# neevparikh/rpt

Hardware: AMD Instinct MI355X
Metric: Msamples/sec (higher is better)
Workload: dtype f32; 1 GPU; C3 lampshade-in-fog path trace 1024x1024x256spp; scene=examples/volumetric_pathtrace_lampshade.rs, parallelism=tile-shard x1, streams=2

## Files before the change

### include/rpt_hip.h

```cpp
#ifndef RPT_HIP_H
#define RPT_HIP_H

#include <stdint.h>

#ifdef __cplusplus
extern "C" {
#endif

#define RPT_OK 0
#define RPT_ERR_INVALID (-1)
#define RPT_ERR_STATE (-2)
#define RPT_ERR_DEVICE (-3)
#define RPT_ERR_UNSUPPORTED (-4)

typedef struct rpt_scene rpt_scene;

enum { RPT_SHAPE_SPHERE = 0, RPT_SHAPE_CUBE = 1, RPT_SHAPE_PLANE = 2, RPT_SHAPE_MESH = 3,
       RPT_SHAPE_GROUP = 4,
       RPT_SHAPE_MONOMIAL = 5  };

typedef struct rpt_shape_desc {
    int32_t kind;
    int32_t has_transform;
    double transform[16];
// ... 105 lines not shown
int rpt_denoise_device(rpt_denoiser*, const rpt_denoise_params*, const void* d_rgb, const void* d_var, const void* d_albedo,
                       const void* d_normal, const void* d_depth, void* d_out, void* d_out_var, void* hip_stream);
int rpt_denoise(rpt_denoiser*, const rpt_denoise_params*, const double* rgb, const double* var, const double* albedo,
                const double* normal, const double* depth, double* out, double* out_var);
int rpt_buffer_mean_device(rpt_buffer*, void* d_rgb, void* d_var, void* hip_stream);
int rpt_buffer_denoised_image(rpt_buffer*, rpt_denoiser*, const rpt_denoise_params*, const void* d_albedo, const void* d_normal,
                              const void* d_depth, uint8_t* out_rgb8);

int rpt_buffer_add_samples_tiles_device(rpt_buffer*, const void* d_rgb, const void* d_tiles, uint32_t n_tiles, void* hip_stream);
int rpt_buffer_tile_batches(rpt_buffer*, uint32_t* out , uint64_t capacity);
typedef struct rpt_adaptive_params {
    uint32_t spp_per_batch, min_batches, max_batches, _pad;
    double threshold;
    double floor;
} rpt_adaptive_params;
int rpt_buffer_tile_errors_device(rpt_buffer*, double floor, void* d_err , void* hip_stream);
int rpt_buffer_refine_tiles(rpt_buffer*, const rpt_adaptive_params*, void* d_tiles_out ,
                            uint32_t* n_out , void* d_err , void* hip_stream);
int rpt_render_adaptive(rpt_scene*, const rpt_camera*, const rpt_render_params*, const rpt_adaptive_params*,
                        uint64_t seed, rpt_buffer*, uint64_t stats[4] );

enum { RPT_PHOTON_MAP = 0, RPT_PHOTON_POINT_BEAM = 1, RPT_PHOTON_BEAM_BEAM = 2 };
int rpt_photon_map_build(rpt_scene*, uint64_t photon_count, int32_t kind, double watts, uint64_t seed);
#define RPT_PHOTON_RECORD_BYTES 48
int rpt_photon_shoot(rpt_scene*, uint64_t photon_count, int32_t kind, double watts, uint64_t seed,
                     uint32_t shard_rank, uint32_t shard_count, uint64_t n_out[2]);
int rpt_photon_records(rpt_scene*, int32_t which , void** d_records, uint64_t* n);
int rpt_photon_map_from_records(rpt_scene*, uint64_t photon_count, int32_t kind, const void* d_surface,
                                uint64_t n_surface, const void* d_volume, uint64_t n_volume);
int rpt_photon_map_stats(rpt_scene*, uint64_t out[8]);
int rpt_photon_map_download(rpt_scene*, int32_t which, float* out, uint64_t capacity_photons);
int rpt_photon_render_sample(rpt_scene*, const rpt_camera*, const rpt_render_params*, uint64_t gather_size,
                             uint64_t gather_size_volume, uint32_t num_samples, uint64_t seed,
                             uint32_t sample_offset, double* out_rgb);
int rpt_photon_render_sample_device(rpt_scene*, const rpt_camera*, const rpt_render_params*, uint64_t gather_size,
                                    uint64_t gather_size_volume, uint32_t num_samples, uint64_t seed,
                                    uint32_t sample_offset, void* d_out_rgb, void* hip_stream);

typedef struct rpt_comm rpt_comm;
#define RPT_COMM_ID_BYTES 128
int rpt_comm_unique_id(void* id_out);
int rpt_comm_create(const void* id, int rank, int n_ranks, int device, rpt_comm** out);
void rpt_comm_destroy(rpt_comm*);
int rpt_comm_rank(const rpt_comm*, int* rank, int* n_ranks);
#define RPT_GATHER_LOOPBACK 1u
int rpt_gather_frame_device(rpt_comm*, uint32_t width, uint32_t height, const void* d_shard, void* d_frame,
                            uint32_t flags, void* hip_stream);
int rpt_allgather_records_device(rpt_comm*, const void* d_local, uint64_t n_local, void* d_out, uint64_t capacity,
                                 uint64_t* n_per_rank, uint64_t* n_total, void* hip_stream);
int rpt_frame_pack_layout(uint32_t width, uint32_t height, uint32_t n_ranks, uint64_t* tile_offsets);
int rpt_frame_pack_device(uint32_t width, uint32_t height, uint32_t rank, uint32_t n_ranks, const void* d_frame,
                          void* d_packed, void* hip_stream);
int rpt_frame_unpack_device(uint32_t width, uint32_t height, uint32_t rank, uint32_t n_ranks, const void* d_packed,
                            void* d_frame, void* hip_stream);

int rpt_debug_epsilon_counters(rpt_scene*, uint64_t out[12]);
int rpt_f64_mesh_tree_info(rpt_scene*, uint64_t out[8]);

int rpt_debug_rng_u32(uint64_t seed, uint32_t pixel, uint32_t sample, uint32_t n, uint32_t* out);
int rpt_debug_material_sample_f(const rpt_material*, uint64_t n, const float* normals, const float* wos,
                                uint64_t seed, float* wi, float* pdf, int32_t* some);
int rpt_debug_material_bsdf(const rpt_material*, uint64_t n, const float* normals, const float* wos,
                            const float* wis, float* out_rgb);
int rpt_debug_radix_sort(uint64_t n, const uint64_t* keys, uint64_t* keys_out, uint32_t* order_out);
int rpt_debug_exclusive_scan2(uint64_t n, const uint32_t* a, const uint32_t* b, uint32_t* out_a, uint32_t* out_b, uint64_t totals[2]);
int rpt_debug_photon_positions64(rpt_scene*, double* out, uint64_t capacity);
int rpt_debug_photon_selections(rpt_scene*, uint32_t* out, uint64_t capacity_words, uint64_t dims[3]);
int rpt_debug_camera_rays(const rpt_camera*, const rpt_render_params*, uint64_t seed, uint32_t sample,
                          float* origins, float* dirs);
int rpt_debug_camera_sample(const rpt_camera*, const rpt_render_params*, uint64_t seed, uint32_t sample,
                            float* origins, float* dirs, uint32_t* next_word);
int rpt_debug_camera_sample_f64(const rpt_camera*, const rpt_render_params*, uint64_t seed, uint32_t sample,
                                double* origins, double* dirs, uint32_t* next_word);
int rpt_debug_light_sample(rpt_scene*, uint32_t light, uint64_t n, const float* positions, uint64_t seed, float* v, float* nrm,
                           float* pdf, float* intensity, float* wi, float* dist, uint32_t* next_word);
int rpt_debug_light_sample_f64(rpt_scene*, uint32_t light, uint64_t n, const double* positions, uint64_t seed, double* v, double* nrm,
                               double* pdf, double* intensity, double* wi, double* dist, uint32_t* next_word);
int rpt_debug_env_color(rpt_scene*, uint64_t n, const float* dirs, float* rgb);
int rpt_debug_env_color_f64(rpt_scene*, uint64_t n, const double* dirs, double* rgb);
int rpt_debug_medium_distance(rpt_scene*, uint64_t n, uint64_t seed, float* dmed, float* t_limit);
int rpt_debug_shadow_test(rpt_scene*, uint32_t light, uint64_t n, const float* origins, const float* dirs, const float* dist,
                          int32_t* out_flag, float* out_t);
int rpt_shadow_scan_info(rpt_scene*, uint32_t light, uint32_t out[4]);
int rpt_debug_distance_pair(float sigma_t, uint32_t k0, uint32_t n, float* out_new, float* out_guarded);
int rpt_debug_draw_forms(uint64_t seed, uint32_t n, uint32_t* out_new, uint32_t* out_ref);

int rpt_debug_bounce(const rpt_material* m, uint32_t max_bounces, uint32_t depth, int32_t in_medium, int32_t medium_event,
                     float albedo_med, const float* medium_color, uint64_t n, const float* normals, const float* rds, uint64_t seed,
                     int32_t* flag, float* wi, float* k, uint32_t* next_word);
int rpt_debug_material_f64(const rpt_material* m, uint64_t n, const double* normals, const double* wos, uint64_t seed, int32_t* some,
                           double* wi, double* pdf, double* f, uint32_t* next_word);
int rpt_debug_material_bsdf_f64(const rpt_material* m, uint64_t n, const double* normals, const double* wos, const double* wis,
                                double* f);
#ifdef __cplusplus
}
#endif
#endif
```

### rpt_amd/_lib.py

```python
import ctypes as C
import os
import sys

_HERE = os.path.dirname(os.path.abspath(__file__))
LIB_PATH = os.environ.get("RPT_LIB", os.path.join(_HERE, "librpt_hip.so"))


class RptError(RuntimeError):
    """Raised for every non-zero return code of the C ABI (message from rpt_last_error)."""


class ShapeDesc(C.Structure):
    pass


ShapeDesc._fields_ = [
    ("kind", C.c_int32),
    ("has_transform", C.c_int32),
    ("transform", C.c_double * 16),
    ("plane_normal", C.c_double * 3),
    ("plane_value", C.c_double),
    ("tris", C.POINTER(C.c_double)),
    ("n_tris", C.c_uint64),
    ("children", C.POINTER(ShapeDesc)),
# ... 86 lines not shown
     [_P, C.POINTER(CameraDesc), C.POINTER(RenderParams), C.c_uint32, C.c_uint64, C.c_uint32, _P, _P, _P, _P]),
    ("rpt_intersect_batch", C.c_int, [_P, C.c_uint64, _P, _P, _P, _P, _P]),
    ("rpt_intersect_batch_f64", C.c_int, [_P, C.c_uint64, _P, _P, _P, _P, _P]),
    ("rpt_intersect_segments", C.c_int, [_P, C.c_uint64, _P, _P, _P, _P, _P]),
    ("rpt_scan_cull_counters", C.c_int, [_P, C.POINTER(C.c_uint64)]),
    ("rpt_scan_cull_groups", C.c_int, [_P, C.POINTER(C.c_float), C.POINTER(C.c_uint64), C.POINTER(C.c_uint32), C.POINTER(C.c_uint32)]),
    ("rpt_scene_stats", C.c_int, [_P, C.POINTER(C.c_uint64)]),
    ("rpt_get_counters", C.c_int, [_P, C.POINTER(C.c_uint64)]),
    ("rpt_debug_section_counters", C.c_int, [_P, C.POINTER(C.c_uint64)]),
    ("rpt_get_timing", C.c_int, [_P, C.POINTER(C.c_double), C.POINTER(C.c_double), C.POINTER(C.c_int32)]),
    ("rpt_get_timing_mean", C.c_int, [_P, C.POINTER(C.c_double), C.POINTER(C.c_double), C.POINTER(C.c_int32)]),
    ("rpt_render_chunking", C.c_int, [C.c_uint32, C.POINTER(C.c_uint32), C.POINTER(C.c_uint32)]),
    ("rpt_scene_render_chunking", C.c_int, [_P, C.c_uint32, C.POINTER(C.c_uint32), C.POINTER(C.c_uint32)]),
    ("rpt_set_option", C.c_int, [C.c_char_p, C.c_int64]),
    ("rpt_scene_set_option", C.c_int, [_P, C.c_char_p, C.c_int64]),
    ("rpt_buffer_create", _P, [C.c_int, C.c_uint32, C.c_uint32, C.c_uint32]),
    ("rpt_buffer_destroy", None, [_P]),
    ("rpt_buffer_add_samples", C.c_int, [_P, _P]),
    ("rpt_buffer_add_samples_device", C.c_int, [_P, _P, _P]),
    ("rpt_buffer_image", C.c_int, [_P, _P]),
    ("rpt_buffer_variance", C.c_int, [_P, C.POINTER(C.c_double)]),
    ("rpt_buffer_batches", C.c_int, [_P, C.POINTER(C.c_uint32)]),
    ("rpt_render_into_buffer", C.c_int,
     [_P, C.POINTER(CameraDesc), C.POINTER(RenderParams), C.c_uint32, C.c_uint64, C.c_uint32, _P]),
    ("rpt_denoiser_create", _P, [C.c_int, C.c_uint32, C.c_uint32]),
    ("rpt_denoiser_destroy", None, [_P]),
    ("rpt_denoise_device", C.c_int, [_P, C.POINTER(DenoiseParams), _P, _P, _P, _P, _P, _P, _P, _P]),
    ("rpt_denoise", C.c_int, [_P, C.POINTER(DenoiseParams), _P, _P, _P, _P, _P, _P, _P]),
    ("rpt_buffer_mean_device", C.c_int, [_P, _P, _P, _P]),
    ("rpt_buffer_denoised_image", C.c_int, [_P, _P, C.POINTER(DenoiseParams), _P, _P, _P, _P]),
    ("rpt_buffer_add_samples_tiles_device", C.c_int, [_P, _P, _P, C.c_uint32, _P]),
    ("rpt_buffer_tile_batches", C.c_int, [_P, _P, C.c_uint64]),
    ("rpt_buffer_tile_errors_device", C.c_int, [_P, C.c_double, _P, _P]),
    ("rpt_buffer_refine_tiles", C.c_int, [_P, C.POINTER(AdaptiveParams), _P, C.POINTER(C.c_uint32), _P, _P]),
    ("rpt_render_adaptive", C.c_int,
     [_P, C.POINTER(CameraDesc), C.POINTER(RenderParams), C.POINTER(AdaptiveParams), C.c_uint64, _P, C.POINTER(C.c_uint64)]),
    ("rpt_photon_map_build", C.c_int, [_P, C.c_uint64, C.c_int32, C.c_double, C.c_uint64]),
    ("rpt_photon_shoot", C.c_int,
     [_P, C.c_uint64, C.c_int32, C.c_double, C.c_uint64, C.c_uint32, C.c_uint32, C.POINTER(C.c_uint64)]),
    ("rpt_photon_records", C.c_int, [_P, C.c_int32, C.POINTER(C.c_void_p), C.POINTER(C.c_uint64)]),
    ("rpt_photon_map_from_records", C.c_int, [_P, C.c_uint64, C.c_int32, _P, C.c_uint64, _P, C.c_uint64]),
    ("rpt_photon_map_stats", C.c_int, [_P, C.POINTER(C.c_uint64)]),
    ("rpt_photon_map_download", C.c_int, [_P, C.c_int32, _P, C.c_uint64]),
    ("rpt_photon_render_sample", C.c_int,
     [_P, C.POINTER(CameraDesc), C.POINTER(RenderParams), C.c_uint64, C.c_uint64, C.c_uint32, C.c_uint64, C.c_uint32, _P]),
    ("rpt_photon_render_sample_device", C.c_int,
     [_P, C.POINTER(CameraDesc), C.POINTER(RenderParams), C.c_uint64, C.c_uint64, C.c_uint32, C.c_uint64, C.c_uint32, _P, _P]),
    ("rpt_comm_unique_id", C.c_int, [_P]),
    ("rpt_comm_create", C.c_int, [_P, C.c_int, C.c_int, C.c_int, C.POINTER(C.c_void_p)]),
    ("rpt_comm_destroy", None, [_P]),
    ("rpt_comm_rank", C.c_int, [_P, C.POINTER(C.c_int), C.POINTER(C.c_int)]),
    ("rpt_gather_frame_device", C.c_int, [_P, C.c_uint32, C.c_uint32, _P, _P, C.c_uint32, _P]),
    ("rpt_allgather_records_device", C.c_int, [_P, _P, C.c_uint64, _P, C.c_uint64, C.POINTER(C.c_uint64), C.POINTER(C.c_uint64), _P]),
    ("rpt_frame_pack_layout", C.c_int, [C.c_uint32, C.c_uint32, C.c_uint32, C.POINTER(C.c_uint64)]),
    ("rpt_frame_pack_device", C.c_int, [C.c_uint32, C.c_uint32, C.c_uint32, C.c_uint32, _P, _P, _P]),
    ("rpt_frame_unpack_device", C.c_int, [C.c_uint32, C.c_uint32, C.c_uint32, C.c_uint32, _P, _P, _P]),
    ("rpt_debug_epsilon_counters", C.c_int, [_P, C.POINTER(C.c_uint64)]),
    ("rpt_f64_mesh_tree_info", C.c_int, [_P, C.POINTER(C.c_uint64)]),
    ("rpt_debug_rng_u32", C.c_int, [C.c_uint64, C.c_uint32, C.c_uint32, C.c_uint32, _P]),
    ("rpt_debug_material_sample_f", C.c_int,
     [C.POINTER(MaterialDesc), C.c_uint64, _P, _P, C.c_uint64, _P, _P, _P]),
    ("rpt_debug_material_bsdf", C.c_int, [C.POINTER(MaterialDesc), C.c_uint64, _P, _P, _P, _P]),
    ("rpt_debug_radix_sort", C.c_int, [C.c_uint64, _P, _P, _P]),
    ("rpt_debug_exclusive_scan2", C.c_int, [C.c_uint64, _P, _P, _P, _P, C.POINTER(C.c_uint64)]),
    ("rpt_debug_photon_positions64", C.c_int, [_P, _P, C.c_uint64]),
    ("rpt_debug_photon_selections", C.c_int, [_P, _P, C.c_uint64, C.POINTER(C.c_uint64)]),
    ("rpt_debug_camera_rays", C.c_int,
     [C.POINTER(CameraDesc), C.POINTER(RenderParams), C.c_uint64, C.c_uint32, _P, _P]),
    ("rpt_debug_light_sample", C.c_int, [_P, C.c_uint32, C.c_uint64, _P, C.c_uint64, _P, _P, _P, _P, _P, _P, _P]),
    ("rpt_debug_light_sample_f64", C.c_int, [_P, C.c_uint32, C.c_uint64, _P, C.c_uint64, _P, _P, _P, _P, _P, _P, _P]),
    ("rpt_debug_env_color", C.c_int, [_P, C.c_uint64, _P, _P]),
    ("rpt_debug_env_color_f64", C.c_int, [_P, C.c_uint64, _P, _P]),
    ("rpt_debug_medium_distance", C.c_int, [_P, C.c_uint64, C.c_uint64, _P, _P]),
    ("rpt_debug_camera_sample", C.c_int,
     [C.POINTER(CameraDesc), C.POINTER(RenderParams), C.c_uint64, C.c_uint32, _P, _P, _P]),
    ("rpt_debug_camera_sample_f64", C.c_int,
     [C.POINTER(CameraDesc), C.POINTER(RenderParams), C.c_uint64, C.c_uint32, _P, _P, _P]),
    ("rpt_debug_bounce", C.c_int, [C.POINTER(MaterialDesc), C.c_uint32, C.c_uint32, C.c_int32, C.c_int32, C.c_float, _P,
                                   C.c_uint64, _P, _P, C.c_uint64, _P, _P, _P, _P]),
    ("rpt_debug_shadow_test", C.c_int, [_P, C.c_uint32, C.c_uint64, _P, _P, _P, _P, _P]),
    ("rpt_debug_distance_pair", C.c_int, [C.c_float, C.c_uint32, C.c_uint32, _P, _P]),
    ("rpt_debug_draw_forms", C.c_int, [C.c_uint64, C.c_uint32, _P, _P]),
    ("rpt_shadow_scan_info", C.c_int, [_P, C.c_uint32, C.POINTER(C.c_uint32)]),
    ("rpt_debug_material_f64", C.c_int, [C.POINTER(MaterialDesc), C.c_uint64, _P, _P, C.c_uint64, _P, _P, _P, _P, _P]),
    ("rpt_debug_material_bsdf_f64", C.c_int, [C.POINTER(MaterialDesc), C.c_uint64, _P, _P, _P, _P]),
]

_lib = None


def vp(a):
    return a.ctypes.data_as(C.c_void_p)


def load():
    global _lib
    if _lib is not None:
        return _lib
    if not os.path.exists(LIB_PATH):
        raise RptError(
            f"{LIB_PATH} is missing: build it with `python -c 'import __graft_entry__ as g; g.build()'` "
            "(hipcc --offload-arch=gfx950).  There is no CPU fallback.")
    if "torch" not in sys.modules and os.environ.get("RPT_IMPORT_TORCH", "0") == "1":
        import torch
    lib = C.CDLL(LIB_PATH, mode=C.RTLD_GLOBAL)
    for name, res, args in SYMBOLS:
        fn = getattr(lib, name)
        fn.restype = res
        fn.argtypes = args
    _lib = lib
    return lib


def check(rc):
    if rc < 0:
        msg = load().rpt_last_error()
        raise RptError(f"rpt error {rc}: {msg.decode() if msg else ''}")
    return rc
```

### rpt_amd/api.py

```python
import ctypes as C
import math
import weakref

import numpy as np

from . import _lib
from ._lib import RptError, vp as _vp

def shard_pixels(width, height, rank, count):
    lib = _lib.load()
    n = _lib.check(lib.rpt_shard_tiles(width, height, rank, count, None, 0))
    tiles = np.zeros(max(n, 1), dtype=np.uint32)
    _lib.check(lib.rpt_shard_tiles(width, height, rank, count, tiles.ctypes.data_as(C.c_void_p), n))
    tiles_x = (width + 31) // 32
    ys, xs = np.mgrid[0:32, 0:32]
    out = []
    for t in tiles[:n]:
        x = (int(t) % tiles_x) * 32 + xs
        y = (int(t) // tiles_x) * 32 + ys
        m = (x < width) & (y < height)
        out.append((y[m] * width + x[m]).astype(np.uint32))
    return np.sort(np.concatenate(out)) if out else np.zeros(0, dtype=np.uint32)


# ... 1133 lines not shown
        return dict(zip(names, [int(v) for v in out]))

    def get_closest_hit(self, origins, dirs):
        lib = _lib.load()
        h = self.scene._commit(self.device_)
        o = np.ascontiguousarray(origins, dtype=np.float32).reshape(-1, 3)
        d = np.ascontiguousarray(dirs, dtype=np.float32).reshape(-1, 3)
        n = o.shape[0]
        t = np.empty(n, dtype=np.float32)
        obj = np.empty(n, dtype=np.int32)
        nrm = np.empty((n, 3), dtype=np.float32)
        _lib.check(lib.rpt_intersect_batch(h, n, o.ctypes.data_as(C.c_void_p), d.ctypes.data_as(C.c_void_p),
                                           t.ctypes.data_as(C.c_void_p), obj.ctypes.data_as(C.c_void_p),
                                           nrm.ctypes.data_as(C.c_void_p)))
        return t, obj, nrm

    def get_closest_hit_f64(self, origins, dirs):
        lib = _lib.load()
        h = self.scene._commit(self.device_)
        o = np.ascontiguousarray(origins, dtype=np.float64).reshape(-1, 3)
        d = np.ascontiguousarray(dirs, dtype=np.float64).reshape(-1, 3)
        n = o.shape[0]
        t = np.empty(n, dtype=np.float64)
        obj = np.empty(n, dtype=np.int32)
        nrm = np.empty((n, 3), dtype=np.float64)
        _lib.check(lib.rpt_intersect_batch_f64(h, n, o.ctypes.data_as(C.c_void_p), d.ctypes.data_as(C.c_void_p),
                                               t.ctypes.data_as(C.c_void_p), obj.ctypes.data_as(C.c_void_p),
                                               nrm.ctypes.data_as(C.c_void_p)))
        return t, obj, nrm

    def f64_mesh_tree_info(self):
        out = (C.c_uint64 * 8)()
        _lib.check(_lib.load().rpt_f64_mesh_tree_info(self.scene._commit(self.device_), out))
        keys = ("meshes", "triangles", "nodes", "depth", "bytes", "render_uses_trees", "photon_uses_trees", "tree_min")
        return {k: int(v) for k, v in zip(keys, out)}

    def debug_light_sample(self, light_index, positions, seed=0, f64=False):
        lib = _lib.load()
        h = self.scene._commit(self.device_)
        ft = np.float64 if f64 else np.float32
        pos = np.ascontiguousarray(positions, dtype=ft).reshape(-1, 3)
        n = pos.shape[0]
        out = {"v": np.empty((n, 3), ft), "nrm": np.empty((n, 3), ft), "p": np.empty(n, ft), "intensity": np.empty((n, 3), ft),
               "wi": np.empty((n, 3), ft), "dist": np.empty(n, ft), "next_word": np.empty(n, np.uint32)}
        fn = lib.rpt_debug_light_sample_f64 if f64 else lib.rpt_debug_light_sample
        _lib.check(fn(h, light_index, n, pos.ctypes.data_as(C.c_void_p), seed,
                      *[out[k].ctypes.data_as(C.c_void_p) for k in ("v", "nrm", "p", "intensity", "wi", "dist", "next_word")]))
        return out

    def debug_env_color(self, dirs, f64=False):
        lib = _lib.load()
        h = self.scene._commit(self.device_)
        d = np.ascontiguousarray(dirs, dtype=np.float64 if f64 else np.float32).reshape(-1, 3)
        out = np.empty_like(d)
        fn = lib.rpt_debug_env_color_f64 if f64 else lib.rpt_debug_env_color
        _lib.check(fn(h, d.shape[0], d.ctypes.data_as(C.c_void_p), out.ctypes.data_as(C.c_void_p)))
        return out

    def debug_medium_distance(self, n, seed=0):
        lib = _lib.load()
        h = self.scene._commit(self.device_)
        dmed, lim = np.empty(n, np.float32), np.empty(n, np.float32)
        _lib.check(lib.rpt_debug_medium_distance(h, n, seed, dmed.ctypes.data_as(C.c_void_p), lim.ctypes.data_as(C.c_void_p)))
        return dmed, lim

    def debug_shadow_test(self, light_index, origins, dirs, dist):
        lib = _lib.load()
        h = self.scene._commit(self.device_)
        o = np.ascontiguousarray(origins, dtype=np.float32).reshape(-1, 3)
        d = np.ascontiguousarray(dirs, dtype=np.float32).reshape(-1, 3)
        ds = np.ascontiguousarray(dist, dtype=np.float32).reshape(-1)
        n = o.shape[0]
        if d.shape[0] != n or ds.shape[0] != n:
            raise ValueError("origins, dirs and dist differ in length")
        flag, t = np.empty(n, np.int32), np.empty(n, np.float32)
        _lib.check(lib.rpt_debug_shadow_test(h, light_index, n, _vp(o), _vp(d), _vp(ds), _vp(flag), _vp(t)))
        return flag, t

    def shadow_scan_info(self, light_index):
        out = (C.c_uint32 * 4)()
        _lib.check(_lib.load().rpt_shadow_scan_info(self.scene._commit(self.device_), light_index, out))
        return {"twin_lo": int(out[0]), "twin_hi": int(out[1]), "shadow_form": int(out[2]), "twin_object": int(np.int32(np.uint32(out[3])))}


def debug_distance_pair(sigma_t, k0, n):
    new, guarded = np.empty(n, np.float32), np.empty(n, np.float32)
    _lib.check(_lib.load().rpt_debug_distance_pair(float(sigma_t), int(k0), int(n), _vp(new), _vp(guarded)))
    return new, guarded


DRAW_FORM_WORDS = 274


def debug_draw_forms(seed, n):
    new, ref = np.empty((DRAW_FORM_WORDS, n), np.uint32), np.empty((DRAW_FORM_WORDS, n), np.uint32)
    _lib.check(_lib.load().rpt_debug_draw_forms(C.c_uint64(int(seed)), int(n), _vp(new), _vp(ref)))
    return new, ref


def debug_bounce(material, normals, rds, max_bounces=3, depth=0, seed=0, in_medium=False, medium_event=False, albedo_med=0.0,
                 medium_color=(0.0, 0.0, 0.0)):
    nrm = np.ascontiguousarray(normals, dtype=np.float32).reshape(-1, 3)
    rd = np.ascontiguousarray(rds, dtype=np.float32).reshape(-1, 3)
    n = nrm.shape[0]
    if rd.shape[0] != n:
        raise ValueError("normals and rds differ in length")
    mcol = np.ascontiguousarray(medium_color, dtype=np.float32).reshape(3)
    out = {"flag": np.empty(n, np.int32), "wi": np.empty((n, 3), np.float32), "k": np.empty((n, 3), np.float32),
           "next_word": np.empty(n, np.uint32)}
    md = material_desc(material, _lib.MaterialDesc)
    _lib.check(_lib.load().rpt_debug_bounce(C.byref(md), max_bounces, depth, int(bool(in_medium)), int(bool(medium_event)),
                                            float(albedo_med), _vp(mcol), n, _vp(nrm), _vp(rd), seed,
                                            *[_vp(out[k]) for k in ("flag", "wi", "k", "next_word")]))
    return out


def debug_material_f64(material, normals, wos, seed=0):
    nrm = np.ascontiguousarray(normals, dtype=np.float64).reshape(-1, 3)
    wo = np.ascontiguousarray(wos, dtype=np.float64).reshape(-1, 3)
    n = nrm.shape[0]
    if wo.shape[0] != n:
        raise ValueError("normals and wos differ in length")
    out = {"some": np.empty(n, np.int32), "wi": np.empty((n, 3)), "pdf": np.empty(n), "f": np.empty((n, 3)),
           "next_word": np.empty(n, np.uint32)}
    md = material_desc(material, _lib.MaterialDesc)
    _lib.check(_lib.load().rpt_debug_material_f64(C.byref(md), n, _vp(nrm), _vp(wo), seed,
                                                  *[_vp(out[k]) for k in ("some", "wi", "pdf", "f", "next_word")]))
    return out


def debug_material_bsdf_f64(material, normals, wos, wis):
    arrs = [np.ascontiguousarray(a, dtype=np.float64).reshape(-1, 3) for a in (normals, wos, wis)]
    n = arrs[0].shape[0]
    if any(a.shape[0] != n for a in arrs):
        raise ValueError("normals, wos and wis differ in length")
    f = np.empty((n, 3))
    md = material_desc(material, _lib.MaterialDesc)
    _lib.check(_lib.load().rpt_debug_material_bsdf_f64(C.byref(md), n, *[_vp(a) for a in arrs], _vp(f)))
    return f


def debug_camera_sample(camera, width, height, sample=0, seed=0, f64=False):
    ft = np.float64 if f64 else np.float32
    n = width * height
    out = {"o": np.empty((n, 3), ft), "d": np.empty((n, 3), ft), "next_word": np.empty(n, np.uint32)}
    prm = _lib.RenderParams(width, height, 0.0, 0, 0, 1)
    lib = _lib.load()
    fn = lib.rpt_debug_camera_sample_f64 if f64 else lib.rpt_debug_camera_sample
    _lib.check(fn(C.byref(camera_desc(camera, _lib.CameraDesc)), C.byref(prm), seed, sample,
                  *[_vp(out[k]) for k in ("o", "d", "next_word")]))
    return out
```

### rpt_amd/csrc/device_core.h

```cpp
#pragma once
#include <hip/hip_runtime.h>
#include <type_traits>
#include "gpu_layout.h"

namespace rptg {

#define RPT_DEV __device__ __forceinline__

static constexpr float kPi = 3.14159265358979323846f;
static constexpr float kInvPi = 0.31830988618379067154f;
static constexpr float kInf = __builtin_huge_valf();

struct V {
    float x, y, z;
};
RPT_DEV V mk(float x, float y, float z) { return V{x, y, z}; }
RPT_DEV V operator+(V a, V b) { return V{a.x + b.x, a.y + b.y, a.z + b.z}; }
RPT_DEV V operator-(V a, V b) { return V{a.x - b.x, a.y - b.y, a.z - b.z}; }
RPT_DEV V operator-(V a) { return V{-a.x, -a.y, -a.z}; }
RPT_DEV V operator*(float s, V a) { return V{s * a.x, s * a.y, s * a.z}; }
RPT_DEV V operator*(V a, float s) { return V{s * a.x, s * a.y, s * a.z}; }
RPT_DEV V operator*(V a, V b) { return V{a.x * b.x, a.y * b.y, a.z * b.z}; }
RPT_DEV float dot(V a, V b) { return fmaf(a.x, b.x, fmaf(a.y, b.y, a.z * b.z)); }
RPT_DEV V cross(V a, V b) {
    return V{a.y * b.z - a.z * b.y, a.z * b.x - a.x * b.z, a.x * b.y - a.y * b.x};
}
RPT_DEV V fma3(float s, V a, V b) { return V{fmaf(s, a.x, b.x), fmaf(s, a.y, b.y), fmaf(s, a.z, b.z)}; }
RPT_DEV V fma3(V s, V a, V b) { return V{fmaf(s.x, a.x, b.x), fmaf(s.y, a.y, b.y), fmaf(s.z, a.z, b.z)}; }
RPT_DEV float rsq(float x) { return __builtin_amdgcn_rsqf(x); }
RPT_DEV float rcp(float x) { return __builtin_amdgcn_rcpf(x); }
RPT_DEV float sqrt1(float x) { return __builtin_amdgcn_sqrtf(x); }
RPT_DEV V normalize(V a) { return rsq(dot(a, a)) * a; }
RPT_DEV V vmin(V a, V b) { return V{fminf(a.x, b.x), fminf(a.y, b.y), fminf(a.z, b.z)}; }
RPT_DEV float max3(float a, float b, float c) { return fmaxf(fmaxf(a, b), c); }
RPT_DEV float min3(float a, float b, float c) { return fminf(fminf(a, b), c); }
RPT_DEV V xyz(const F4& f) { return V{f.x, f.y, f.z}; }
RPT_DEV float dot3w(const F4& r, V p) { return fmaf(r.x, p.x, fmaf(r.y, p.y, fmaf(r.z, p.z, r.w))); }
RPT_DEV float dot3(const F4& r, V p) { return fmaf(r.x, p.x, fmaf(r.y, p.y, r.z * p.z)); }
RPT_DEV bool is_zero(V a) { return a.x == 0.f && a.y == 0.f && a.z == 0.f; }

template <class T>
RPT_DEV T uload(const T* p) {
    static_assert(sizeof(T) % 16 == 0, "scene records are 16-byte multiples");
    typedef uint32_t u4v __attribute__((ext_vector_type(4)));
    typedef const __attribute__((address_space(4))) u4v* CP;
    CP q = (CP)(uintptr_t)p;
    u4v raw[sizeof(T) / 16];
#pragma unroll
    for (unsigned i = 0; i < sizeof(T) / 16; i++) raw[i] = q[i];
    T out;
    __builtin_memcpy(&out, raw, sizeof(T));
    return out;
}

typedef const __attribute__((address_space(4))) SceneView* KernargView;
RPT_DEV KernargView kernarg_scene() {
    KernargView kv = (KernargView)__builtin_amdgcn_kernarg_segment_ptr();
    asm volatile("" : "+s"(kv));
    return kv;
}
template <class T>
RPT_DEV T kernarg_load(const __attribute__((address_space(4))) T* p) {
    static_assert(sizeof(T) % 4 == 0, "kernel-argument structs are dword multiples");
    typedef const __attribute__((address_space(4))) uint32_t* Q;
    Q q = (Q)p;
    uint32_t raw[sizeof(T) / 4];
#pragma unroll
    for (unsigned i = 0; i < sizeof(T) / 4; i++) raw[i] = q[i];
    T out;
    __builtin_memcpy(&out, raw, sizeof(T));
    return out;
}
template <class T>
RPT_DEV const __attribute__((address_space(4))) T* kernarg_args() {
    typedef const __attribute__((address_space(4))) T* P;
    P p = (P)__builtin_amdgcn_kernarg_segment_ptr();
    asm volatile("" : "+s"(p));
    return p;
}

RPT_DEV uint64_t mix64(uint64_t x) {
    x ^= x >> 30;
    x *= 0xBF58476D1CE4E5B9ULL;
    x ^= x >> 27;
    x *= 0x94D049BB133111EBULL;
    x ^= x >> 31;
    return x;
}
// ... 344 lines not shown

template <bool COUNT, bool PRIMS, bool ANY, bool MONO>
RPT_DEV void bvh_traverse(const SceneView& scene_, uint32_t root, V o, V d, float tmin, float& tbest, uint32_t& code,
                          uint32_t& inst, uint32_t* stk, uint32_t stride, uint32_t cap, uint32_t& c_nodes,
                          uint32_t& c_tris, AnyHit any) {
    const auto& sc = *kernarg_scene();
    const BvhNode* nodes = sc.nodes;
    const V inv = mk(rcp(d.x), rcp(d.y), rcp(d.z));
    const uint32_t kDone = 0xFFFFFFFFu;
    uint32_t sp = 0;
    uint32_t cur = root;
    while (cur != kDone) {
        while (!(cur & BVH_LEAF)) {
            const BvhNode nd = nodes[cur];
            if (COUNT) c_nodes++;
            float n0, f0, n1, f1;
            slab2(nd.lo0, nd.hi0, o, inv, n0, f0);
            slab2(nd.lo1, nd.hi1, o, inv, n1, f1);
            const bool h0 = fmaxf(n0, tmin) <= fminf(f0, tbest);
            const bool h1 = fmaxf(n1, tmin) <= fminf(f1, tbest);
            if (h0 && h1) {
                const bool first0 = n0 <= n1;
                if (sp < cap) { stk[sp * stride] = first0 ? nd.e1 : nd.e0; sp++; }
                else if (COUNT && sc.stack_overflows) atomicAdd(sc.stack_overflows, 1ull);
                cur = first0 ? nd.e0 : nd.e1;
            } else if (h0 || h1) {
                cur = h0 ? nd.e0 : nd.e1;
            } else if (sp) {
                sp--;
                cur = stk[sp * stride];
            } else {
                cur = kDone;
            }
        }
        if (cur != kDone) {
            const uint32_t first = cur & BVH_INDEX_MASK;
            const uint32_t count = ((cur >> 26) & 31u) + 1u;
            if (PRIMS && (cur & BVH_PRIMS)) {
                for (uint32_t i = 0; i < count; i++) {
                    if (COUNT) c_tris++;
                    hit_prim<COUNT, MONO>(scene_, sc.pleaf[first + i], o, d, inv, tmin, tbest, code, inst, stk + sp * stride, stride,
                                    cap - sp, c_nodes, c_tris);
                }
            } else {
                for (uint32_t i = 0; i < count; i++) {
                    const TriScan tr = sc.btri[first + i];
                    if (COUNT) c_tris++;
                    float t = hit_tri(tr.pn, tr.A, tr.B, o, d, tmin, tbest);
                    if (t >= 0.f) { tbest = t; code = (K_BVHTRI << 28) | (first + i); }
                }
            }
            if (ANY && code != CODE_MISS && any.blocks(tbest, code)) sp = 0;
            if (sp) {
                sp--;
                cur = stk[sp * stride];
            } else {
                cur = kDone;
            }
        }
    }
}

template <bool SHELL>
RPT_DEV bool interval_meets_box(const SceneView::ScanBox& b, V o, V inv, float tmin, float tbest) {
#pragma clang fp contract(off)
    const float x1 = (b.lo[0] - o.x) * inv.x, x2 = (b.hi[0] - o.x) * inv.x;
    const float y1 = (b.lo[1] - o.y) * inv.y, y2 = (b.hi[1] - o.y) * inv.y;
    const float z1 = (b.lo[2] - o.z) * inv.z, z2 = (b.hi[2] - o.z) * inv.z;
    float start, end;
    if (SHELL) {
        const bool sx = x1 > x2, sy = y1 > y2, sz = z1 > z2;
        start = max3(sx ? x2 : x1, sy ? y2 : y1, sz ? z2 : z1);
        end = min3(sx ? x1 : x2, sy ? y1 : y2, sz ? z1 : z2);
    } else {
        start = max3(fminf(x1, x2), fminf(y1, y2), fminf(z1, z2));
        end = min3(fmaxf(x1, x2), fmaxf(y1, y2), fmaxf(z1, z2));
    }
    return !(fmaxf(start, tmin) > fminf(end, tbest));
}
struct ShadowTwin {
    uint32_t kind, lo, span;
    RPT_DEV bool has(uint32_t i) const { return i - lo <= span; }
};
template <bool MASKED = false, bool MONO = false, bool TAIL = false, bool SHADOW = false>
RPT_DEV void scan_prims(const SceneView& scene, V o, V d, float tmin, float& tbest, uint32_t& code, uint64_t mask = ~0ull,
                        bool* tail_skipped = nullptr, ShadowTwin twin = ShadowTwin{0u, 1u, 0u}, bool* best_is_twin = nullptr) {
    static_assert(!(TAIL && MASKED), "one cull at a time");
    static_assert(!(SHADOW && (MASKED || TAIL)), "the shadow form is a plain scan");
    const auto& sc = *kernarg_scene();
    (void)scene;
    bool flag = false;
    float t_twin = __builtin_nanf("");
    auto acc = [&](bool ok, float t, uint32_t c, auto is_twin) {
        if (ok) tbest = t;
        asm volatile("" : "+v"(tbest));
        if constexpr (!SHADOW) { if (ok) code = c; }
        else if constexpr (std::is_same_v<decltype(is_twin), std::false_type>) flag = flag && !ok;
        else if (ok && is_twin) t_twin = t;
    };
    auto twin_at = [&](auto tw, uint32_t i) {
        if constexpr (decltype(tw)::value) return twin.has(i);
        else return std::false_type{};
    };
    auto kind_loop = [&](uint32_t kind, auto&& loop) {
        if constexpr (SHADOW) {
            if (twin.kind == kind) {
                loop(std::true_type{});
                flag = t_twin == tbest;
                return;
            }
        }
        loop(std::false_type{});
    };
    uint32_t bit = 0;
    auto on = [&](uint32_t i) { return !MASKED || ((mask >> ((bit + i) & 63u)) & 1ull) != 0ull; };
    const uint64_t sph_yrot = MASKED ? 0ull : sc.sph_yrot, cub_yrot = MASKED ? 0ull : sc.cub_yrot;
    kind_loop(K_SPHERE, [&](auto tw) {
        for (uint32_t i = 0; i < sc.n_sph; i++) {
            if (!on(i)) continue;
            const XfScan x = uload(&sc.sph[i]);
            V ol, dl;
            if (!MASKED && ((sph_yrot >> (i & 63u)) & 1ull)) to_local_y(x, o, d, ol, dl);
            else to_local(x, o, d, ol, dl);
            float t;
            acc(sphere_closer(ol, dl, tmin, tbest, t), t, (K_SPHERE << 28) | i, twin_at(tw, i));
        }
    });
    bit += sc.n_sph;
    kind_loop(K_CUBE, [&](auto tw) {
        uint32_t i = 0;
        if (!MASKED)
            for (; i + 1u < sc.n_cub; i += 2u) {
                const XfScan x0 = uload(&sc.cub[i]), x1 = uload(&sc.cub[i + 1u]);
                V ol0, dl0, ol1, dl1;
                float t0, t1;
                if (((cub_yrot >> (i & 63u)) & 3ull) == 3ull) {
                    to_local_y(x0, o, d, ol0, dl0);
                    to_local_y(x1, o, d, ol1, dl1);
                } else {
                    to_local(x0, o, d, ol0, dl0);
                    to_local(x1, o, d, ol1, dl1);
                }
                acc(cube_closer(ol0, dl0, tmin, tbest, t0), t0, (K_CUBE << 28) | i, twin_at(tw, i));
                acc(cube_closer(ol1, dl1, tmin, tbest, t1), t1, (K_CUBE << 28) | (i + 1u), twin_at(tw, i + 1u));
            }
        for (; i < sc.n_cub; i++) {
            if (!on(i)) continue;
            const XfScan x = uload(&sc.cub[i]);
            V ol, dl;
            if (!MASKED && ((cub_yrot >> (i & 63u)) & 1ull)) to_local_y(x, o, d, ol, dl);
            else to_local(x, o, d, ol, dl);
            float t;
            acc(cube_closer(ol, dl, tmin, tbest, t), t, (K_CUBE << 28) | i, twin_at(tw, i));
        }
    });
    bit += sc.n_cub;
    for (uint32_t i = 0; i < sc.n_pln; i++) {
        const F4 nv = uload(&sc.pln[i]).nv;
        float t;
        acc(plane_closer(nv, o, d, tmin, tbest, t), t, (K_PLANE << 28) | i, std::false_type{});
    }
    const uint32_t n_rect = sc.n_rect_x + sc.n_rect_y + sc.n_rect_z;
    if (sc.n_aabb + n_rect + sc.has_shell != 0) {
        const V inv = mk(rcp(d.x), rcp(d.y), rcp(d.z));
        if (sc.has_shell)
            shell_closer(uload(sc.shell), o, inv, tmin, tbest, [&](bool ok, float t, auto code_of) {
                if constexpr (SHADOW) acc(ok, t, 0u, std::false_type{});
                else { if (ok) { tbest = t; code = code_of(); } }
            });
        if constexpr (TAIL) {
            if (sc.scan_cull) {
                const SceneView::ScanBox tb = kernarg_load(&sc.scan_tail);
                if (__ballot(interval_meets_box<false>(tb, o, inv, tmin, tbest)) == 0ull) {
                    if (tail_skipped) *tail_skipped = true;
                    return;
                }
            }
        }
        kind_loop(K_AABB, [&](auto tw) {
            uint32_t i = 0;
            if (!MASKED)
                for (; i + 1u < sc.n_aabb; i += 2u) {
                    const AabbScan b0 = uload(&sc.aabb[i]), b1 = uload(&sc.aabb[i + 1u]);
                    aabb_pair_closer(b0, b1, __float_as_uint(b0.hi.w), o, inv, tmin, tbest, i,
                                     [&](bool ok, float t, uint32_t k) { acc(ok, t, (K_AABB << 28) | k, twin_at(tw, k)); });
                }
            for (; i < sc.n_aabb; i++) {
                if (!on(i)) continue;
                const AabbScan b = uload(&sc.aabb[i]);
                float t;
                acc(aabb_closer(b.lo, b.hi, o, inv, tmin, tbest, t), t, (K_AABB << 28) | i, twin_at(tw, i));
            }
        });
        bit += sc.n_aabb;
        kind_loop(K_RECT, [&](auto tw) {
            uint32_t i = 0;
            for (uint32_t e = sc.n_rect_x; i < e; i++) {
                if (!on(i)) continue;
                const RectScan r = uload(&sc.rect[i]);
                float t;
                acc(rect_closer(r.a, r.b.x, o.x, inv.x, o.y, d.y, o.z, d.z, tmin, tbest, t), t, (K_RECT << 28) | i, twin_at(tw, i));
            }
            for (uint32_t e = sc.n_rect_x + sc.n_rect_y; i < e; i++) {
                if (!on(i)) continue;
                const RectScan r = uload(&sc.rect[i]);
                float t;
                acc(rect_closer(r.a, r.b.x, o.y, inv.y, o.z, d.z, o.x, d.x, tmin, tbest, t), t, (K_RECT << 28) | i, twin_at(tw, i));
            }
            for (uint32_t e = n_rect; i < e; i++) {
                if (!on(i)) continue;
                const RectScan r = uload(&sc.rect[i]);
                float t;
                acc(rect_closer(r.a, r.b.x, o.z, inv.z, o.x, d.x, o.y, d.y, tmin, tbest, t), t, (K_RECT << 28) | i, twin_at(tw, i));
            }
        });
        bit += n_rect;
    } else {
        bit += sc.n_aabb + n_rect;
    }
    kind_loop(K_TRI, [&](auto tw) {
        for (uint32_t i = 0; i < sc.n_tri; i++) {
            if (!on(i)) continue;
            const TriScan tr = uload(&sc.tri[i]);
            float t;
            acc(tri_closer(tr.pn, tr.A, tr.B, o, d, tmin, tbest, t), t, (K_TRI << 28) | i, twin_at(tw, i));
        }
    });
    if constexpr (MONO) {
        static_assert(!MASKED && !TAIL, "scan_mask_for_ball and the tail cull do not cover the monomial surfaces");
        for (uint32_t i = 0; i < sc.n_mono; i++) {
            const MonoScan m = uload(&sc.mono[i]);
            V ol, dl;
            to_local(XfScan{m.r0, m.r1, m.r2}, o, d, ol, dl);
            float t;
            acc(mono_closer(ol, dl, m.h, tmin, tbest, t), t, (K_MONO << 28) | i, std::false_type{});
        }
    }
    if constexpr (SHADOW) *best_is_twin = flag;
}
RPT_DEV uint64_t scan_mask_for_ball(const SceneView& scene_, bool live, V c, float r, bool* touched = nullptr) {
    const auto& sc = *kernarg_scene();
    const uint32_t n = sc.n_sph + sc.n_cub + sc.n_aabb + sc.n_rect_x + sc.n_rect_y + sc.n_rect_z + sc.n_tri;
    if (touched) *touched = n != 0u;
    if (n > 64u) return ~0ull;
    bool mine = false;
    const float r2 = r * r;
    uint64_t mask = 0ull;
    auto reaches = [&](const AabbScan& b) {
        const float dx = fmaxf(fmaxf(b.lo.x - c.x, c.x - b.hi.x), 0.f);
        const float dy = fmaxf(fmaxf(b.lo.y - c.y, c.y - b.hi.y), 0.f);
        const float dz = fmaxf(fmaxf(b.lo.z - c.z, c.z - b.hi.z), 0.f);
        const bool t = live && fmaf(dx, dx, fmaf(dy, dy, dz * dz)) <= r2;
        mine = mine || t;
        return __any(t);
    };
    uint32_t i = 0;
    for (; i + 4u <= n; i += 4u) {
        const AabbScan b0 = uload(&sc.pbox[i]), b1 = uload(&sc.pbox[i + 1u]), b2 = uload(&sc.pbox[i + 2u]), b3 = uload(&sc.pbox[i + 3u]);
        if (reaches(b0)) mask |= 1ull << i;
        if (reaches(b1)) mask |= 2ull << i;
        if (reaches(b2)) mask |= 4ull << i;
        if (reaches(b3)) mask |= 8ull << i;
    }
    for (; i < n; i++)
        if (reaches(uload(&sc.pbox[i]))) mask |= 1ull << i;
    if (touched) *touched = mine;
    return mask;
}
template <bool COUNT>
RPT_DEV void scan_primary(const SceneView& scene, V o, V d, float tmin, float& tbest, uint32_t& code, unsigned long long* cnt) {
    if constexpr (COUNT) {
        const auto& sc = *kernarg_scene();
        const SceneView::ScanBox bound = kernarg_load(&sc.scan_bound);
        const bool first = cnt && uint32_t(__builtin_ctzll(__ballot(true))) == (threadIdx.x & 63u);
        if (!(bound.lo[0] > bound.hi[0])) {
            const V inv = mk(rcp(d.x), rcp(d.y), rcp(d.z));
            const bool need = interval_meets_box<true>(bound, o, inv, tmin, tbest);
            const uint32_t n_need = uint32_t(__popcll(__ballot(need)));
            if (first) atomicAdd(&cnt[n_need == 0u ? 0 : n_need <= 2u ? 1 : n_need <= 4u ? 2 : n_need <= 8u ? 3 : 4], 1ull);
            if (n_need != 0u)
                for (uint32_t g = 0; g < sc.n_scan_groups; g++) {
                    const SceneView::ScanGroup grp = kernarg_load(&sc.scan_groups[g]);
                    const bool reach = need && interval_meets_box<false>(grp.box, o, inv, tmin, tbest);
                    if (__ballot(reach) == 0ull && first) atomicAdd(&cnt[5u + g], 1ull);
                }
        }
        bool skipped = false;
        scan_prims<false, false, true>(scene, o, d, tmin, tbest, code, ~0ull, &skipped);
        if (skipped && first) atomicAdd(&cnt[9], 1ull);
    } else {
        scan_prims<false, false, true>(scene, o, d, tmin, tbest, code);
    }
}

RPT_DEV bool mesh_roots_hit(const SceneView& scene_, V o, V d, float tmin, float tbest) {
    const auto& sc = *kernarg_scene();
    const V inv = mk(rcp(d.x), rcp(d.y), rcp(d.z));
    bool need = false;
    for (uint32_t i = 0; i < sc.n_mesh; i++) {
        const MeshRef m = uload(&sc.meshes[i]);
        const BvhNode nd = uload(&sc.nodes[m.root]);
        float n0, f0, n1, f1;
        slab2(nd.lo0, nd.hi0, o, inv, n0, f0);
        slab2(nd.lo1, nd.hi1, o, inv, n1, f1);
        need = need || fmaxf(n0, tmin) <= fminf(f0, tbest) || fmaxf(n1, tmin) <= fminf(f1, tbest);
    }
    return need;
}
template <bool COUNT, bool ANY>
RPT_DEV void walk_meshes(const SceneView& scene_, V o, V d, float tmin, float& tbest, uint32_t& code, uint32_t& inst,
                         uint32_t* stk, uint32_t stride, uint32_t& c_nodes, uint32_t& c_tris, AnyHit any, uint32_t cap = 32u) {
    const auto& sc = *kernarg_scene();
    for (uint32_t i = 0; i < sc.n_mesh; i++) {
        const MeshRef m = uload(&sc.meshes[i]);
        if (ANY && code != CODE_MISS && any.blocks(tbest, code)) break;
        bvh_traverse<COUNT, false, ANY>(scene_, m.root, o, d, tmin, tbest, code, inst, stk, stride, cap, c_nodes, c_tris, any);
    }
}
static const uint32_t kWalkDone = 0xFFFFFFFFu;
struct WalkState {
    uint32_t cur, sp, mesh;
};
RPT_DEV WalkState walk_begin(const SceneView&) { return WalkState{uload(&kernarg_scene()->meshes[0]).root, 0u, 0u}; }
template <bool COUNT>
RPT_DEV void walk_meshes_resumable(const SceneView& scene_, V o, V d, float tmin, float& tbest, uint32_t& code, uint32_t* stk,
                                   uint32_t stride, WalkState& w, uint32_t min_active, AnyHit any, uint32_t& c_nodes,
                                   uint32_t& c_tris, uint32_t cap = 32u, uint32_t leaf_quarters = 0u, uint32_t* c_wave = nullptr) {
    const auto& sc = *kernarg_scene();
    const BvhNode* nodes = sc.nodes;
    const V inv = mk(rcp(d.x), rcp(d.y), rcp(d.z));
    uint32_t cur = w.cur, sp = w.sp, mesh = w.mesh;
    while (uint32_t(__popcll(__ballot(cur != kWalkDone))) >= min_active) {
        for (;;) {
            const bool inner = !(cur & BVH_LEAF);
            const uint32_t n_inner = uint32_t(__popcll(__ballot(inner)));
            if (n_inner == 0u) break;
            if (leaf_quarters != 0u && 4u * uint32_t(__popcll(__ballot(!inner && cur != kWalkDone))) >= leaf_quarters * n_inner) break;
            if (COUNT && c_wave) c_wave[0]++;
            if (!inner) continue;
            const BvhNode nd = nodes[cur];
            if (COUNT) c_nodes++;
            float n0, f0, n1, f1;
            slab2(nd.lo0, nd.hi0, o, inv, n0, f0);
            slab2(nd.lo1, nd.hi1, o, inv, n1, f1);
            const bool h0 = fmaxf(n0, tmin) <= fminf(f0, tbest);
            const bool h1 = fmaxf(n1, tmin) <= fminf(f1, tbest);
            if (h0 && h1) {
                const bool first0 = n0 <= n1;
                if (sp < cap) { stk[sp * stride] = first0 ? nd.e1 : nd.e0; sp++; }
                else if (COUNT && sc.stack_overflows) atomicAdd(sc.stack_overflows, 1ull);
                cur = first0 ? nd.e0 : nd.e1;
            } else if (h0 || h1) {
                cur = h0 ? nd.e0 : nd.e1;
            } else if (sp) {
                sp--;
                cur = stk[sp * stride];
            } else {
                cur = kWalkDone;
            }
        }
        if (COUNT && c_wave) {
            uint32_t mx = 0;
            for (uint32_t k = 1; k <= 4u; k++)
                if (__ballot((cur & BVH_LEAF) && cur != kWalkDone && ((cur >> 26) & 31u) + 1u >= k) != 0ull) mx = k;
            c_wave[1] += mx;
        }
        if ((cur & BVH_LEAF) && cur != kWalkDone) {
            const uint32_t first = cur & BVH_INDEX_MASK;
            const uint32_t count = ((cur >> 26) & 31u) + 1u;
            TriScan nxt = sc.btri[first];
            for (uint32_t i = 0; i < count; i++) {
                const TriScan tr = nxt;
                if (i + 1u < count) nxt = sc.btri[first + i + 1u];
                if (COUNT) c_tris++;
                float t = hit_tri(tr.pn, tr.A, tr.B, o, d, tmin, tbest);
                if (t >= 0.f) { tbest = t; code = (K_BVHTRI << 28) | (first + i); }
            }
            if (code != CODE_MISS && any.blocks(tbest, code)) { sp = 0; mesh = sc.n_mesh; }
            if (sp) {
                sp--;
                cur = stk[sp * stride];
            } else {
                cur = kWalkDone;
            }
        }
        if (cur == kWalkDone && mesh + 1u < sc.n_mesh) {
            mesh++;
            cur = sc.meshes[mesh].root;
        }
    }
    w.cur = cur;
    w.sp = sp;
    w.mesh = mesh;
}

template <int BVH, bool COUNT, bool ANY = false, bool MONO = false>
RPT_DEV void closest_hit(const SceneView& scene_, V o, V d, float tmin, float& tbest, uint32_t& code, uint32_t& inst,
                         uint32_t* stk, uint32_t stride, uint32_t& c_nodes, uint32_t& c_tris,
                         AnyHit any = AnyHit{-kInf, 1u, 0u}) {
    const auto& sc = *kernarg_scene();
    if (BVH == 2 && sc.scene_bvh) {
        for (uint32_t i = 0; i < sc.n_pln; i++) {
            const F4 nv = uload(&sc.pln[i]).nv;
            float t = hit_plane(nv, o, d, tmin);
            if (t >= 0.f && t < tbest) { tbest = t; code = (K_PLANE << 28) | i; }
        }
        bvh_traverse<COUNT, true, ANY, MONO>(scene_, sc.top_root, o, d, tmin, tbest, code, inst, stk, stride, 32u, c_nodes, c_tris, any);
        if (sc.mesh_deferred) walk_meshes<COUNT, ANY>(scene_, o, d, tmin, tbest, code, inst, stk, stride, c_nodes, c_tris, any);
        return;
    }
    scan_prims<false, MONO>(scene_, o, d, tmin, tbest, code);
    if (BVH) walk_meshes<COUNT, ANY>(scene_, o, d, tmin, tbest, code, inst, stk, stride, c_nodes, c_tris, any);
}

template <int BVH, bool COUNT, bool MONO = false>
RPT_DEV void scan_or_tree(const SceneView& scene_, V o, V d, float tmin, float& tbest, uint32_t& code, uint32_t& inst, uint32_t* stk,
                          uint32_t stride, uint32_t& c_nodes, uint32_t& c_tris) {
    if constexpr (BVH == 3) {
        const auto& sc = *kernarg_scene();
        for (uint32_t i = 0; i < sc.n_pln; i++) {
            const F4 nv = uload(&sc.pln[i]).nv;
            float t = hit_plane(nv, o, d, tmin);
            if (t >= 0.f && t < tbest) { tbest = t; code = (K_PLANE << 28) | i; }
        }
        bvh_traverse<COUNT, true, false, MONO>(scene_, sc.top_root, o, d, tmin, tbest, code, inst, stk, stride, 32u, c_nodes, c_tris);
    } else {
        scan_prims<false, MONO>(scene_, o, d, tmin, tbest, code);
    }
}

RPT_DEV V box_face_normal(V p, V lo, V hi) {
    const float xl = fabsf(p.x - lo.x), xh = fabsf(p.x - hi.x), yl = fabsf(p.y - lo.y), yh = fabsf(p.y - hi.y);
    const float zl = fabsf(p.z - lo.z), zh = fabsf(p.z - hi.z);
    const float ex = fminf(xl, xh), ey = fminf(yl, yh), ez = fminf(zl, zh);
    const bool ax0 = ex <= ey && ex <= ez, ax1 = !ax0 && ey <= ez;
    return mk(ax0 ? (xh < xl ? 1.f : -1.f) : 0.f, ax1 ? (yh < yl ? 1.f : -1.f) : 0.f, (!ax0 && !ax1) ? (zh < zl ? 1.f : -1.f) : 0.f);
}
template <bool MONO = false>
RPT_DEV void finalize_hit(const SceneView& scene_, V o, V d, float tmin, float t, uint32_t code, uint32_t inst, V& n,
                          uint32_t& obj) {
    const auto& sc = *kernarg_scene();
    uint32_t kind = code >> 28, idx = code & 0x0FFFFFFFu;
    if (MONO && kind == K_MONO) {
        const MonoScan m = sc.mono[idx];
        const XfShade s = sc.mono_sh[idx];
        V ol, dl;
        to_local(XfScan{m.r0, m.r1, m.r2}, o, d, ol, dl);
        const V p = fma3(t, dl, ol);
        const float k = m.h.x * 4.f * fmaf(p.x, p.x, p.z * p.z);
        V nl = normalize(mk(k * p.x, -1.f, k * p.z));
        if (dot(nl, dl) > 0.f) nl = -nl;
        n = (s.r1.w != 0.f) ? normalize(mk(dot3(s.r0, nl), dot3(s.r1, nl), dot3(s.r2, nl))) : nl;
        obj = __float_as_uint(s.r0.w);
        return;
    }
    if (kind == K_INSTTRI) {
        const InstRec r = sc.inst[inst];
        const TriShade s = sc.btri_sh[idx];
        V nl;
        if (s.n2.w != 0.f) {
            nl = xyz(s.n1);
        } else {
            const TriScan tr = sc.btri[idx];
            const V ol = mk(dot3w(r.r0, o), dot3w(r.r1, o), dot3w(r.r2, o));
            const V dl = mk(dot3(r.r0, d), dot3(r.r1, d), dot3(r.r2, d));
            V p = fma3(t, dl, ol);
            float v = dot3w(tr.A, p), w = dot3w(tr.B, p);
            float u = 1.f - v - w;
            nl = normalize(u * xyz(s.n1) + v * xyz(s.n2) + w * xyz(s.n3));
        }
        n = normalize(mk(dot3(r.n0, nl), dot3(r.n1, nl), dot3(r.n2, nl)));
        obj = __float_as_uint(r.n0.w);
        return;
    }
    if (kind == K_SPHERE) {
        const XfScan x = sc.sph[idx];
        const XfShade s = sc.sph_sh[idx];
        V ol, dl;
        to_local(x, o, d, ol, dl);
        V nl = normalize(fma3(t, dl, ol));
        n = (s.r1.w != 0.f) ? normalize(mk(dot3(s.r0, nl), dot3(s.r1, nl), dot3(s.r2, nl))) : nl;
        obj = __float_as_uint(s.r0.w);
    } else if (kind == K_CUBE) {
        const XfScan x = sc.cub[idx];
        const XfShade s = sc.cub_sh[idx];
        V ol, dl;
        to_local(x, o, d, ol, dl);
        const V nl = box_face_normal(fma3(t, dl, ol), mk(-0.5f, -0.5f, -0.5f), mk(0.5f, 0.5f, 0.5f));
        n = (s.r1.w != 0.f) ? normalize(mk(dot3(s.r0, nl), dot3(s.r1, nl), dot3(s.r2, nl))) : nl;
        obj = __float_as_uint(s.r0.w);
    } else if (kind == K_AABB) {
        const AabbScan b = sc.aabb[idx];
        n = box_face_normal(fma3(t, d, o), xyz(b.lo), xyz(b.hi));
        obj = __float_as_uint(b.lo.w);
// ... 298 lines not shown
```

### rpt_amd/csrc/gpu_layout.h

```cpp
#pragma once
#include <stdint.h>

namespace rptg {

struct alignas(16) F4 {
    float x, y, z, w;
};

enum : uint32_t { K_SPHERE = 0, K_CUBE = 1, K_PLANE = 2, K_TRI = 3, K_BVHTRI = 4, K_AABB = 5, K_RECT = 6,
                  K_INST = 7,
                  K_INSTTRI = 8,
                  K_MONO = 9 };
static const uint32_t CODE_MISS = 0xFFFFFFFFu;

struct alignas(16) XfScan {
    F4 r0, r1, r2;
};
struct alignas(16) XfShade {
    F4 r0, r1, r2;
};
struct alignas(16) PlaneScan {
    F4 nv;
};
struct alignas(16) MonoScan {
    F4 r0, r1, r2;
    F4 h;
};
struct alignas(16) PlaneShade {
    F4 unit_n_obj;
};
struct alignas(16) TriScan {
    F4 pn, A, B;
};
struct alignas(16) TriShade {
    F4 n1, n2, n3;
};
struct alignas(16) AabbScan {
    F4 lo, hi;
};
struct alignas(16) RectScan {
    F4 a;
    F4 b;
};
struct alignas(16) ShellScan {
    F4 lo, hi;
    uint32_t face[8];
};
struct alignas(16) RectShade {
    F4 n_obj;
};
struct alignas(16) BvhNode {
    float lo0[3];
    uint32_t e0;
    float hi0[3];
    uint32_t pad0;
    float lo1[3];
    uint32_t e1;
    float hi1[3];
    uint32_t pad1;
};
static const uint32_t BVH_LEAF = 0x80000000u;
static const uint32_t BVH_PRIMS = 0x02000000u;
static const uint32_t BVH_INDEX_MASK = 0x01FFFFFFu;
enum : uint32_t { M_LAMBERTIAN = 0, M_PHONG = 1, M_MIRROR = 2, M_TRANSMISSIVE = 3 };
struct alignas(16) Material {
    F4 albedo_emit;
    F4 params;
};
enum : uint32_t { L_POINT = 0, L_AMBIENT = 1, L_DIRECTIONAL = 2, L_OBJECT = 3 };
enum : uint32_t { LS_SPHERE = 0, LS_CUBE = 1, LS_GROUP = 2, LS_MESH = 3 };
struct alignas(16) Light {
    uint32_t kind;
    uint32_t shape;
    int32_t twin_object;
    uint32_t first;
    uint32_t count;
    uint32_t xf;
    uint32_t twin_lo, twin_hi;
    F4 color;
    F4 albedo;
};
struct alignas(16) LightPart {
    uint32_t shape;
    uint32_t first;
// ... 72 lines not shown
```

### rpt_amd/csrc/host_internal.h

```cpp
#pragma once
#include <hip/hip_runtime_api.h>

#include <functional>
#include <string>
#include <utility>

#include "../../include/rpt_hip.h"
#include "kernels.h"

namespace rpt64 { struct Args; struct Camera; }

namespace rpti {
class DevMem {
  public:
    DevMem() = default;
    DevMem(DevMem&& o) noexcept : p_(std::exchange(o.p_, nullptr)), cap_(std::exchange(o.cap_, 0)) {}
    DevMem& operator=(DevMem&& o) noexcept {
        if (this != &o) {
            reset();
            p_ = std::exchange(o.p_, nullptr);
            cap_ = std::exchange(o.cap_, 0);
        }
        return *this;
    }
    ~DevMem() { reset(); }
    hipError_t reserve(size_t bytes) {
        if (bytes <= cap_) return hipSuccess;
        hipError_t e = p_ ? hipFree(p_) : hipSuccess;
        p_ = nullptr;
        cap_ = 0;
        if (e == hipSuccess) e = hipMalloc(&p_, bytes);
        if (e != hipSuccess) { p_ = nullptr; return e; }
        cap_ = bytes;
        return hipSuccess;
    }
    void reset() {
        if (p_) (void)hipFree(p_);
        p_ = nullptr;
        cap_ = 0;
    }
    template <class T = void>
    T* get() const { return static_cast<T*>(p_); }
    size_t capacity() const { return cap_; }
    explicit operator bool() const { return p_ != nullptr; }

  private:
    void* p_ = nullptr;
    size_t cap_ = 0;
};
class Event {
  public:
    Event() = default;
    Event(Event&& o) noexcept : e_(std::exchange(o.e_, nullptr)) {}
    Event& operator=(Event&& o) noexcept {
        if (this != &o) {
            reset();
            e_ = std::exchange(o.e_, nullptr);
        }
        return *this;
    }
    ~Event() { reset(); }
    hipError_t create(unsigned flags = hipEventDefault) {
        reset();
        hipError_t e = hipEventCreateWithFlags(&e_, flags);
        if (e != hipSuccess) e_ = nullptr;
        return e;
    }
    void reset() {
        if (e_) (void)hipEventDestroy(e_);
        e_ = nullptr;
    }
    hipEvent_t get() const { return e_; }

  private:
    hipEvent_t e_ = nullptr;
};
inline float elapsed_ms(const Event& a, const Event& b) {
    float ms = 0.f;
    (void)hipEventElapsedTime(&ms, a.get(), b.get());
    return ms;
}

int fail(int code, const std::string& msg);
uint64_t seed_mix(uint64_t seed);
struct SceneDev {
    bool committed;
    int device, n_cus;
    rptg::SceneView view;
    int first_object_light;
    bool epsilon64;
    bool has_monomial;
};
SceneDev scene_dev(rpt_scene* s);
void fill_camera64(const rpt_camera* cam, rpt64::Camera& q);
int light_kind(rpt_scene* s, uint32_t light);
void*& photon_slot(rpt_scene* s);
void photon_release(void* p);
int prepare_render(rpt_scene* s, hipStream_t st, const rpt_camera* cam, const rpt_render_params* prm, uint32_t iterations, uint64_t seed,
                   uint32_t sample_offset, rptg::RenderArgs& a, uint32_t min_chunk = 0, uint32_t fixed_chunk = 0,
                   uint32_t slab_item_bytes = 16,
                   bool launch_set = true);
int run_persistent(rpt_scene* s, const rpt_render_params* prm, const rptg::RenderArgs& a, double* d_out, hipStream_t st,
                   int blocks_per_cu, const std::function<hipError_t(const rptg::RenderArgs&, int, hipStream_t)>& launch,
                   bool indexed_start = false, bool wave_items = false,
                   const std::function<hipError_t(double, double*, hipStream_t)>& resolve = nullptr,
                   bool clear_sharded = true);
int serialize_with_other_streams(rpt_scene* s, hipStream_t st);
int fetch_counters(rpt_scene* s, const rptg::RenderArgs& a);
void fill_args64(rpt_scene* s, const rpt_camera* cam, const rpt_render_params* prm, const rptg::RenderArgs* a, rpt64::Args& q);
double* scratch_out(rpt_scene* s, size_t bytes);
int64_t option_photon_skip(rpt_scene* s);
int64_t option_max_blocks(rpt_scene* s);
int64_t option_f64_photon_slice(rpt_scene* s);
int64_t option_photon_parts(rpt_scene* s);
int64_t option_photon_coop_gather(rpt_scene* s);
int64_t option_photon_split(rpt_scene* s);
int64_t option_photon_block_lists(rpt_scene* s);
}

#define RPTI_HIP_TRY(expr)                                                                          \
    do {                                                                                            \
        hipError_t e__ = (expr);                                                                    \
        if (e__ != hipSuccess)                                                                      \
            return rpti::fail(RPT_ERR_DEVICE, std::string(#expr) + ": " + hipGetErrorString(e__));  \
    } while (0)
```

### rpt_amd/csrc/kernels.h

```cpp
#pragma once
#include <hip/hip_runtime_api.h>
#include <stddef.h>
#include <stdint.h>
#include "gpu_layout.h"

namespace rptg {

struct RenderArgs {
    SceneView sc;
    CameraG cam;
    uint32_t width, height;
    float inv_dim;
    uint32_t max_bounces;
    uint32_t iterations;
    uint32_t sample_offset;
    uint32_t chunk_spp;
    uint32_t n_chunks;
    uint64_t seed_mixed;
    const uint32_t* tiles;
    uint32_t n_tiles, tiles_x;
    uint32_t n_owned;
    uint32_t n_items;
    float* slab;
    float* slab2;
    unsigned long long* queue;
    unsigned long long* counters;
    uint32_t lds_stack;
    uint32_t defer_lanes;
    uint32_t defer_stop;
    uint32_t walk_leaf_quarters;
    uint32_t detach;
    uint32_t pull_batch;
    uint32_t detach_trigger;
    uint32_t stream_backlog;
    uint32_t stream_contexts;
    uint32_t n_twin_lights;
    uint32_t* stream_scratch;
};

static_assert(offsetof(RenderArgs, sc) == 0, "RenderArgs must begin with the SceneView");

struct KernelInfo {
    int vgprs, sgprs, lds, max_blocks_per_cu;
};

hipError_t launch_render(const RenderArgs& a, int n_blocks, hipStream_t stream);
hipError_t render_occupancy(bool medium, int bvh, int* blocks_per_cu, int detach = 0);
size_t stream_scratch_bytes_per_block();
int bvh_mode(const SceneView& sc);
hipError_t launch_buffer_add(uint32_t n_pixels, const double* d_batch, double* d_sum, double* d_sumsq, hipStream_t st);
hipError_t launch_buffer_image(uint32_t w, uint32_t h, uint32_t radius, uint32_t n_batches, const double* d_sum, uint8_t* d_out,
                               hipStream_t st);
hipError_t launch_buffer_variance(uint32_t n_pixels, uint32_t n_batches, const double* d_sum, const double* d_sumsq, double* d_out,
                                  hipStream_t st);
hipError_t launch_resolve(const RenderArgs& a, double scale, double* d_out, hipStream_t stream);
hipError_t launch_frame_pack(const double* d_frame, double* d_packed, const uint32_t* d_tiles, uint32_t n_tiles, uint32_t tiles_x,
                             uint32_t width, uint32_t height, hipStream_t st);
hipError_t launch_frame_unpack(const double* d_packed, double* d_frame, const uint32_t* d_tiles, uint32_t n_tiles, uint32_t tiles_x,
                               uint32_t width, uint32_t height, hipStream_t st);
__attribute__((weak)) hipError_t launch_intersect_segments(const SceneView& sc, uint64_t n, const float* d_o, const float* d_d, const float* d_tmax,
                                                           float* d_t, uint32_t* d_code, hipStream_t stream);
hipError_t launch_intersect(const SceneView& sc, uint64_t n, const float* d_o, const float* d_d, float* d_t,
                            int32_t* d_obj, float* d_n, bool bvh, hipStream_t stream);
struct FeatureArgs {
    RenderArgs r;
    double* slab;
    uint32_t* ids;
};
static_assert(offsetof(FeatureArgs, r) == 0, "FeatureArgs must begin with the SceneView");
struct FeatureResolveArgs {
    const uint32_t* tiles;
    uint32_t tiles_x, n_owned, n_chunks, n_items;
    uint32_t width, height, iterations, pad_;
    const double* slab;
    const uint32_t* ids;
    double *albedo, *normal, *depth;
};
__attribute__((weak)) hipError_t launch_features(const FeatureArgs& a, hipStream_t stream);
__attribute__((weak)) hipError_t launch_feature_resolve(const FeatureResolveArgs& a, hipStream_t stream);
struct DenoisePrepareArgs {
    uint32_t n_pixels, flags;
    const double *rgb, *var, *albedo, *normal, *depth;
    double* rec;
    double* ids;
};
struct DenoisePassArgs {
    uint32_t width, height, step, flags;
    uint32_t terms, pad_;
    double sigma_color2, a_n, a_z;
    const double* rec_in;
    const double* ids;
    const double* albedo;
    double* rec_out;
    double *out, *out_var;
};
__attribute__((weak)) hipError_t launch_denoise_prepare(const DenoisePrepareArgs& a, hipStream_t stream);
__attribute__((weak)) hipError_t launch_denoise_pass(const DenoisePassArgs& a, bool staged , hipStream_t stream);
static constexpr uint32_t kDenoiseMaxStagedStep = 2;
__attribute__((weak)) hipError_t launch_buffer_mean(uint32_t n_pixels, uint32_t n_batches, const double* d_sum, const double* d_sumsq,
                                                    double* d_rgb, double* d_var , hipStream_t st);
__attribute__((weak)) hipError_t launch_color_bytes(uint64_t n_values, const double* d_rgb, uint8_t* d_out, hipStream_t st);
struct TileBufferView {
    uint32_t width, height, tiles_x, tiles_y;
    uint32_t n_batches, pad_;
    const uint32_t* extra;
};
__attribute__((weak)) hipError_t launch_buffer_add_tiles(const TileBufferView& b, const double* d_batch, double* d_sum, double* d_sumsq,
                                                         uint32_t* d_extra, const uint32_t* d_tiles, uint32_t n_tiles, hipStream_t st);
__attribute__((weak)) hipError_t launch_buffer_image_tiles(const TileBufferView& b, uint32_t radius, const double* d_sum, uint8_t* d_out,
                                                           hipStream_t st);
__attribute__((weak)) hipError_t launch_buffer_variance_tiles(const TileBufferView& b, const double* d_sum, const double* d_sumsq, double* d_out,
                                                              hipStream_t st);
__attribute__((weak)) hipError_t launch_buffer_mean_tiles(const TileBufferView& b, const double* d_sum, const double* d_sumsq, double* d_rgb,
                                                          double* d_var , hipStream_t st);
__attribute__((weak)) hipError_t launch_tile_errors(const TileBufferView& b, double floor, const double* d_sum, const double* d_sumsq,
                                                    double* d_err, hipStream_t st);
__attribute__((weak)) hipError_t launch_tile_select(const TileBufferView& b, double threshold2, uint32_t max_batches, const double* d_err,
                                                    uint32_t* d_tiles_out, uint32_t* d_n_out, hipStream_t st);
hipError_t launch_debug_rng(uint64_t seed_mixed, uint32_t pixel, uint32_t sample, uint32_t n, uint32_t* d_out,
                            hipStream_t stream);
hipError_t launch_debug_sample_f(const Material& m, uint64_t n, const float* d_n, const float* d_wo,
                                 uint64_t seed_mixed, float* d_wi, float* d_pdf, int32_t* d_some, hipStream_t s);
hipError_t launch_debug_bsdf(const Material& m, uint64_t n, const float* d_n, const float* d_wo, const float* d_wi,
                             float* d_out, hipStream_t s);
__attribute__((weak)) hipError_t launch_debug_camera_sample(const CameraG& cam, uint32_t w, uint32_t h, float inv_dim, uint64_t seed_mixed,
                                                            uint32_t sample, float* d_o, float* d_d, uint32_t* d_next_word ,
                                                            hipStream_t s);
struct LightSampleArgs {
    uint32_t light;
    uint32_t pad_;
    uint64_t n;
    uint64_t seed_mixed;
    const float* pos;
    float *v, *nrm, *pdf;
    float *intensity, *wi, *dist;
    uint32_t* next_word;
};
__attribute__((weak)) hipError_t launch_debug_light_sample(const SceneView& sc, const LightSampleArgs& q, hipStream_t s);
__attribute__((weak)) hipError_t launch_debug_env_color(const SceneView& sc, uint64_t n, const float* d_dirs, float* d_rgb, hipStream_t s);
__attribute__((weak)) hipError_t launch_debug_medium_distance(const SceneView& sc, uint64_t n, uint64_t seed_mixed, float* d_dmed,
                                                              float* d_limit, hipStream_t s);
struct ShadowTestArgs {
    uint32_t light;
    uint32_t pad_;
    uint64_t n;
    const float *o, *d;
    const float* dist;
    int32_t* flag;
    float* t;
};
__attribute__((weak)) hipError_t launch_debug_shadow_test(const SceneView& sc, const ShadowTestArgs& q, hipStream_t s);
__attribute__((weak)) hipError_t launch_debug_distance_pair(float sigma_t, uint32_t k0, uint32_t n, float* d_new, float* d_guarded, hipStream_t s);
static constexpr uint32_t kDrawFormWords = 274;
__attribute__((weak)) hipError_t launch_debug_draw_forms(uint64_t seed_mixed, uint32_t n, const float inv[3], uint32_t* d_new, uint32_t* d_ref,
                                                         hipStream_t s);
struct BounceArgs {
    Material m;
    uint32_t max_bounces, depth;
    uint32_t in_medium;
    uint32_t medium_event;
    float albedo_med;
    float mcol[3];
    uint64_t n;
    uint64_t seed_mixed;
    const float *nrm, *rd;
    int32_t* flag;
    float *wi, *k;
    uint32_t* next_word;
};
__attribute__((weak)) hipError_t launch_debug_bounce(const BounceArgs& q, hipStream_t s);

}
namespace rpt64 { struct Args; struct ShootArgs64; struct SurfArgs64; struct FeatureArgs64; }
namespace rptg {
hipError_t launch_render_f64(const rpt64::Args& a, int n_blocks, hipStream_t stream);
hipError_t launch_resolve_f64(const rpt64::Args& a, double scale, double* d_out, hipStream_t stream);
hipError_t render_f64_occupancy(bool medium, int* blocks_per_cu);
hipError_t launch_photon_shoot_f64(const rpt64::ShootArgs64& a, int n_blocks, hipStream_t stream);
hipError_t launch_photon_surface_f64(const rpt64::SurfArgs64& a, int n_blocks, hipStream_t stream);
hipError_t launch_resolve_photon_f64(const rpt64::Args& a, const void* slab32, uint32_t n_chunks32, double scale_over_total, bool accumulate,
                                     double* d_out, hipStream_t stream);
__attribute__((weak)) hipError_t launch_features_f64(const rpt64::FeatureArgs64& a, hipStream_t stream);
}
```

### rpt_amd/csrc/kernels.hip

```cpp
#include "device_core.h"
#include "kernels.h"

namespace rptg {

RPT_DEV uint32_t mbcnt64(uint64_t m) {
    return __builtin_amdgcn_mbcnt_hi(uint32_t(m >> 32), __builtin_amdgcn_mbcnt_lo(uint32_t(m), 0u));
}
template <bool MONO = false>
RPT_DEV uint32_t code_object(const SceneView& sc, uint32_t code, uint32_t inst) {
    uint32_t kind = code >> 28, idx = code & 0x0FFFFFFFu;
    float w;
    if (MONO && kind == K_MONO) w = sc.mono_sh[idx].r0.w;
    else if (kind == K_INSTTRI) w = sc.inst[inst].n0.w;
    else if (kind == K_SPHERE) w = sc.sph_sh[idx].r0.w;
    else if (kind == K_CUBE) w = sc.cub_sh[idx].r0.w;
    else if (kind == K_PLANE) w = sc.pln_sh[idx].unit_n_obj.w;
    else if (kind == K_TRI) w = sc.tri_sh[idx].n1.w;
    else if (kind == K_AABB) w = sc.aabb[idx].lo.w;
    else if (kind == K_RECT) w = sc.rect_sh[idx].n_obj.w;
    else w = sc.btri_sh[idx].n1.w;
    return __float_as_uint(w);
}
RPT_DEV float ray_tmin(V o) { return 2e-5f * (1.f + max3(fabsf(o.x), fabsf(o.y), fabsf(o.z))); }

// ... 67 lines not shown
        RPT_MARK(k);                                                                             \
        if (COUNT) {                                                                             \
            const uint64_t m_ = __ballot(true);                                                  \
            if (mbcnt64(m_) == 0) {                                                              \
                atomicAdd(&a.counters[8 + 2 * (k)], 1ull);                                       \
                atomicAdd(&a.counters[9 + 2 * (k)], (unsigned long long)__popcll(m_));           \
            }                                                                                    \
        }                                                                                        \
    } while (0)
#endif
#ifdef RPT_SECT_CLOCKS
#define SECTK(k)                                                                                 \
    do {                                                                                         \
        if (COUNT) {                                                                             \
            const uint64_t now_ = __builtin_amdgcn_s_memtime();                                  \
            if (mbcnt64(__ballot(true)) == 0) {                                                  \
                sect_lds_[threadIdx.x >> 6][2 * (k)] += 1ull;                                    \
                sect_lds_[threadIdx.x >> 6][2 * sect_prev_ + 1] += now_ - sect_clk_;             \
            }                                                                                    \
            sect_prev_ = (k);                                                                    \
            sect_clk_ = now_;                                                                    \
        }                                                                                        \
    } while (0)
#else
#define SECTK(k) SECT(k)
#endif
RPT_DEV float medium_distance_guarded(float xi, float inv_sigma_t) { return -__logf(xi) * inv_sigma_t; }
RPT_DEV float medium_distance(float xi, float inv_sigma_t) {
#pragma clang fp contract(off)
    const float ln2_hi = 0x1.62e42ep-1f, ln2_lo = 0x1.efa39ep-25f;
    const float y = __builtin_amdgcn_logf(xi);
    const float r = y * ln2_hi;
    const float e = __builtin_fmaf(y, ln2_hi, -r);
    const float lo = __builtin_fmaf(y, ln2_lo, e);
    const float ln = __builtin_fmaf(ln2_hi, y, lo);
    return -ln * inv_sigma_t;
}
template <bool MEDIUM>
RPT_DEV void stage_distance(Rng& rng, float inv_sigma_t, float& dmed, float& t) {
    dmed = kInf;
    if (MEDIUM) {
        float xi = rng.range(0.f, 1.f);
        dmed = medium_distance(xi, inv_sigma_t);
    }
    t = (MEDIUM && dmed < 400.f) ? dmed * (1.f + 1e-6f) : kInf;
}
template <bool COUNT, bool MONO = false>
RPT_DEV void stage_event(const RenderArgs& a, const LdsTables& tab, V ro, V rd, uint32_t depth, bool medium, float dmed, float t,
                         uint32_t code, uint32_t inst, V& x, V& n, V& mcol, Mat& mat, V& E) {
    const SceneView& sc = a.sc;
    if (medium) {
        SECT(5);
        x = fma3(dmed, rd, ro);
        bool hi = sc.medium_kind == 1u && x.y > 250.f;
        mcol = hi ? mk(sc.medium_color_hi[0], sc.medium_color_hi[1], sc.medium_color_hi[2])
                  : mk(sc.medium_color[0], sc.medium_color[1], sc.medium_color[2]);
        E = (depth == 0) ? sc.medium_emission * mcol : mk(0, 0, 0);
    } else {
        uint32_t obj;
        SECT(6);
        finalize_hit<MONO>(sc, ro, rd, ray_tmin(ro), t, code, inst, n, obj);
        mat = load_mat(sc, obj, tab);
        x = fma3(t, rd, ro);
        E = (depth == 0) ? mat_emit(mat) * mat_color(mat) : mk(0, 0, 0);
    }
}
template <bool PIN_RD = false>
RPT_DEV void stage_light_add(const SceneView& sc, float albedo_med, V rd, bool medium, V I, V wi, V n, V mcol, const Mat& mat, V& E) {
    if (medium) {
        E = fma3(albedo_med * sc.medium_phase, I * mcol, E);
    } else {
        if constexpr (PIN_RD) asm volatile("" : "+v"(rd.x), "+v"(rd.y), "+v"(rd.z));
        V f = bsdf(mat, n, -normalize(rd), wi);
        E = fma3(dot(wi, n), f * I, E);
    }
}
template <bool MONO = false>
RPT_DEV void stage_light_term(const SceneView& sc, const Light& L, float albedo_med, V rd, bool medium, float ts, uint32_t cs,
                              uint32_t is, float dist, V I, V wi, V n, V mcol, const Mat& mat, V& E) {
    const bool twin = (L.twin_lo <= L.twin_hi) ? (cs >= L.twin_lo && cs <= L.twin_hi)
                                               : (cs != CODE_MISS && code_object<MONO>(sc, cs, is) == uint32_t(L.twin_object));
    if (cs != CODE_MISS && ts >= dist * (1.f - 1e-3f) && twin) stage_light_add(sc, albedo_med, rd, medium, I, wi, n, mcol, mat, E);
}
template <bool MONO = false>
RPT_DEV bool scan_light_visible(const SceneView& sc, const Light& L, V x, V wi, float dist, float& ts) {
    ts = dist * (1.f + 1e-3f);
    uint32_t cs = CODE_MISS;
    if (__float_as_uint(L.color.w) != 0u) {
        bool twin = false;
        scan_prims<false, MONO, false, true>(sc, x, wi, ray_tmin(x), ts, cs, ~0ull, nullptr,
                                             ShadowTwin{L.twin_lo >> 28, L.twin_lo & 0x0FFFFFFFu, L.twin_hi - L.twin_lo}, &twin);
        return twin && ts >= dist * (1.f - 1e-3f);
    }
    scan_prims<false, MONO>(sc, x, wi, ray_tmin(x), ts, cs);
    const bool twin = (L.twin_lo <= L.twin_hi) ? (cs >= L.twin_lo && cs <= L.twin_hi)
                                               : (cs != CODE_MISS && code_object<MONO>(sc, cs, 0u) == uint32_t(L.twin_object));
    return cs != CODE_MISS && ts >= dist * (1.f - 1e-3f) && twin;
}
template <bool MEDIUM, bool COUNT>
RPT_DEV bool stage_bounce(const RenderArgs& a, float albedo_med, V rd, uint32_t depth, bool medium, V n, V mcol, const Mat& mat,
                          Rng& rng, V& wi, V& k) {
    bool bounce;
    SECT(10);
    if (medium) {
        SECT(11);
        bounce = rng.below<kRoulette08>(0.8f);
        if (bounce) {
            float ax = rng.range(-1.f, 1.f), ay = rng.range(-1.f, 1.f), az = rng.range(-1.f, 1.f);
            wi = normalize(mk(ax, ay, az));
            k = (albedo_med * 1.25f) * mcol;
        }
    } else {
        SECT(12);
        bounce = MEDIUM ? rng.below<kRoulette08>(0.8f) : (depth < a.max_bounces);
        if (bounce) {
            float pdf;
            SECT(13);
            const V wo = -normalize(rd);
            bounce = sample_f(mat, n, wo, rng, wi, pdf);
            if (bounce) {
                V f = bsdf(mat, n, wo, wi);
                float wgt = fabsf(dot(wi, n)) * rcp(MEDIUM ? pdf * 0.8f : pdf);
                k = wgt * f;
            }
        }
    }
    return bounce && !is_zero(k);
}

template <bool MEDIUM, int BVH, bool COUNT, bool GROUPS = false, int DETACH = 0, bool MONO = false>
__global__ __launch_bounds__(256, BVH == 0 ? ((GROUPS || COUNT || MONO) ? RPT_MIN_WAVES_SCAN_GROUPS : RPT_MIN_WAVES_SCAN) : BVH == 3 ? RPT_MIN_WAVES_SCENE_MESH : BVH == 1 ? (DETACH == 2 ? RPT_MIN_WAVES_STREAM : RPT_MIN_WAVES_MESH) : RPT_MIN_WAVES)
void render_kernel(const RenderArgs a) {
#ifdef RPT_SECT_CLOCKS
    __shared__ unsigned long long sect_lds_[4][56];
    if ((threadIdx.x & 63u) < 56u) sect_lds_[threadIdx.x >> 6][threadIdx.x & 63u] = 0ull;
    uint64_t sect_clk_ = __builtin_amdgcn_s_memtime();
    uint32_t sect_prev_ = 27u;
#endif
    static_assert(DETACH == 0 || (MEDIUM && BVH == 1 && !GROUPS), "detached tree walks: per-mesh-tree kernels in a medium only");
    static_assert(DETACH == 0 || !MONO, "no detached tree walks in scenes with monomial surfaces");
    extern __shared__ uint32_t dyn_lds[];
    const SceneView& sc = a.sc;
    uint32_t* stk = BVH ? (dyn_lds + threadIdx.x) : nullptr;
    const uint32_t stride = 256;

    const float sigma_t = sc.sigma_a + sc.sigma_s;
    const float inv_sigma_t = MEDIUM ? 1.f / sigma_t : 0.f;
    const float albedo_med = MEDIUM ? sc.sigma_s / sigma_t : 0.f;

    Rng rng;
    rng.s0 = rng.s1 = rng.s2 = rng.s3 = 0;
    V ro = mk(0, 0, 0), rd = mk(0, 0, 1);
    V P = mk(0, 0, 0), Q = mk(1, 1, 1), Rc = mk(kInf, kInf, kInf);
    constexpr uint32_t kStackRows = BVH == 1 ? (DETACH ? kDetachStackRows : 21u) : 32u;
    constexpr uint32_t kStateBase = BVH ? kStackRows * 256u : 0u;
    uint32_t* const ls = dyn_lds + kStateBase + threadIdx.x;
    enum { S_SLAB = 0, S_END = 1, S_PIX = 2, S_XN = 3, S_YN = 4, S_S = 5, S_ACC = 6, S_P = 9, S_Q = 12, S_RC = 15, S_ROWS = 18 };
    static_assert(S_RC + 3 == S_ROWS, "the staged tables begin right behind the state rows");
    constexpr uint32_t kTabBase = kStateBase + (BVH == 0 ? uint32_t(S_ROWS) : 5u) * 256u;
    LdsTables tab;
    {
        const F4* const t4 = reinterpret_cast<const F4*>(dyn_lds + kTabBase);
        F4* const w4 = reinterpret_cast<F4*>(dyn_lds + kTabBase);
        const uint32_t nm = sc.n_obj <= kLdsMats ? sc.n_obj : 0u, nl = sc.n_ltris <= kLdsLtris ? sc.n_ltris : 0u;
        for (uint32_t i = threadIdx.x; i < 2u * nm; i += 256u) w4[i] = reinterpret_cast<const F4*>(sc.mats)[i];
        for (uint32_t i = threadIdx.x; i < 6u * nl; i += 256u) w4[2u * kLdsMats + i] = reinterpret_cast<const F4*>(sc.ltris)[i];
        __syncthreads();
        tab.mats = t4; tab.n_mats = nm;
        tab.ltris = t4 + 2u * kLdsMats; tab.n_ltris = nl;
    }
    auto in_lds = [](int k) { return BVH == 0 || k <= S_YN; };
    V acc_r = mk(0, 0, 0);
    uint32_t slab_idx_r = 0, s_r = 0, s_end_r = 0, pix_r = 0;
    float xn_r = 0.f, yn_r = 0.f;
    auto ldu = [&](int k, uint32_t reg) { return in_lds(k) ? ls[k * 256] : reg; };
    auto ldf = [&](int k, float reg) { return in_lds(k) ? __uint_as_float(ls[k * 256]) : reg; };
    auto stu = [&](int k, uint32_t& reg, uint32_t v) { if (in_lds(k)) ls[k * 256] = v; else reg = v; };
    auto stf = [&](int k, float& reg, float v) { if (in_lds(k)) ls[k * 256] = __float_as_uint(v); else reg = v; };
    volatile uint32_t* const ls_pend = dyn_lds + (DETACH ? kDetachPendBase : 0u);
    unsigned long long* const acc64 = reinterpret_cast<unsigned long long*>(dyn_lds + (DETACH ? kDetachAccBase : 0u));
    volatile uint32_t* const wq = dyn_lds + (DETACH ? kDetachQBase + (threadIdx.x >> 6) * kQWaveDwords : 0u);
    auto acc_add = [&](V v) {
        if constexpr (DETACH) {
            atomicAdd(&acc64[threadIdx.x], to_fixed(v.x));
            atomicAdd(&acc64[256u + threadIdx.x], to_fixed(v.y));
            atomicAdd(&acc64[512u + threadIdx.x], to_fixed(v.z));
        } else {
            stf(S_ACC + 0, acc_r.x, ldf(S_ACC + 0, acc_r.x) + v.x);
            stf(S_ACC + 1, acc_r.y, ldf(S_ACC + 1, acc_r.y) + v.y);
            stf(S_ACC + 2, acc_r.z, ldf(S_ACC + 2, acc_r.z) + v.z);
        }
    };
    if constexpr (DETACH) {
        if ((threadIdx.x & 63u) < 16u) wq[threadIdx.x & 63u] = 0u;
        ls_pend[threadIdx.x] = 0u;
    }
    auto ldv = [&](int k, V reg) { return BVH == 0 ? mk(__uint_as_float(ls[k * 256]), __uint_as_float(ls[(k + 1) * 256]), __uint_as_float(ls[(k + 2) * 256])) : reg; };
    auto stv = [&](int k, V& reg, V v) {
        if (BVH == 0) { ls[k * 256] = __float_as_uint(v.x); ls[(k + 1) * 256] = __float_as_uint(v.y); ls[(k + 2) * 256] = __float_as_uint(v.z); }
        else reg = v;
    };
    uint32_t depth = 0;
    bool alive = true, have_item = false, need_path = true;
    bool item_done = true;
    bool drained = false;
    bool first_batch = true;
    uint32_t pool_next = 0, pool_end = 0;
    uint32_t pool_chunk = 0, pool_x0 = 0, pool_y0 = 0;

    uint32_t c_samples = 0, c_rays = 0, c_vertices = 0, c_trips = 0, c_nodes = 0, c_btris = 0;
    uint32_t c_nodes_primary = 0;
    uint32_t c_wave[2] = {0, 0}, w_tot[2] = {0, 0};

    enum : uint32_t { PH_NEW = 0, PH_HAVEP = 1, PH_LIGHT = 2, PH_HAVES = 3, PH_WAITP = 4, PH_WAITS = 5 };
    uint32_t phase = PH_NEW, q_code = CODE_MISS, q_inst = 0, v_li = 0;
    float q_t = kInf, v_dmed = kInf, v_dist = 0.f;
    V v_x = mk(0, 0, 0), v_n = mk(0, 1, 0), v_mcol = mk(0, 0, 0), v_E = mk(0, 0, 0), v_I = mk(0, 0, 0), v_wi = mk(0, 0, 1);
    Mat v_mat = Mat{mk(0, 0, 0), 0.f, 0u, 0.f, 0.f};
    bool v_medium = false;
    WalkState walk{kWalkDone, 0u, 0u};
    uint32_t fuse = 0u;
    constexpr uint32_t kNoEntry = 0xFFFFFFFFu;
    uint32_t h_e = kNoEntry;
// ... 709 lines not shown
                        if (L.twin_object >= 0) {
                            SECTK(8);
                            const float tm = ray_tmin(v_x);
                            q_t = v_dist * (1.f + 1e-3f);
                            q_code = CODE_MISS;
                            q_inst = 0;
                            scan_or_tree<BVH, COUNT, MONO>(sc, v_x, v_wi, tm, q_t, q_code, q_inst, stk, stride, c_nodes, c_btris);
                            if (COUNT) c_rays++;
                            const AnyHit any{L.twin_lo <= L.twin_hi ? v_dist * (1.f - 1e-3f) : -kInf, L.twin_lo, L.twin_hi};
                            const bool blocked = q_code != CODE_MISS && any.blocks(q_t, q_code);
                            phase = (!blocked && mesh_roots_hit(sc, v_x, v_wi, tm, q_t)) ? PH_WAITS : PH_HAVES;
                            walk = walk_begin(sc);
                            next = false;
                        }
                    }
                    if (next) v_li = l + 1u;
                }
                if (alive && phase == PH_HAVES && v_li == l) {
                    SECTK(9);
                    stage_light_term<MONO>(sc, L, albedo_med, rd, v_medium, q_t, q_code, q_inst, v_dist, v_I, v_wi, v_n, v_mcol, v_mat, v_E);
                    v_li = l + 1u;
                    phase = PH_LIGHT;
                }
            }
            if (alive && phase == PH_LIGHT && v_li >= sc.n_lights) {
                V wi = mk(0, 0, 1), k = mk(0, 0, 0);
                const bool cont = stage_bounce<MEDIUM, COUNT>(a, albedo_med, rd, depth, v_medium, v_n, v_mcol, v_mat, rng, wi, k);
                SECTK(14);
                P = fma3(Q, v_E, P);
                if (cont) {
                    if (!MEDIUM) Rc = vmin(Rc, fma3(100.f, Q, P));
                    Q = Q * k;
                    ro = v_x;
                    rd = wi;
                    depth++;
                } else {
                    acc_add(vmin(P, Rc));
                    need_path = true;
                }
                phase = PH_NEW;
            }
            const bool waiting = alive && phase >= PH_WAITP;
            const uint64_t wm = __ballot(waiting);
            const bool idle = __ballot(alive && !waiting && !(need_path && item_done)) == 0;
            if (wm != 0 && (uint32_t(__popcll(wm)) >= a.defer_lanes || idle)) {
                if (COUNT) c_wave[0] = c_wave[1] = 0;
                if (waiting) {
                    SECTK(15);
                    const bool shadow = phase == PH_WAITS;
                    const V qo = shadow ? v_x : ro, qd = shadow ? v_wi : rd;
                    AnyHit any{-kInf, 1u, 0u};
                    if (shadow) {
                        const uint32_t lo = sc.lights[v_li].twin_lo, hi = sc.lights[v_li].twin_hi;
                        any = AnyHit{lo <= hi ? v_dist * (1.f - 1e-3f) : -kInf, lo, hi};
                    }
                    walk_meshes_resumable<COUNT>(sc, qo, qd, ray_tmin(qo), q_t, q_code, stk, stride, walk,
                                                 idle ? 1u : a.defer_stop, any, c_nodes, c_btris, kStackRows, a.walk_leaf_quarters, c_wave);
                    if (walk.cur == kWalkDone) {
                        phase = shadow ? PH_HAVES : PH_HAVEP;
                        SECTK(16);
                        if ((q_code >> 28) == K_BVHTRI) { SECTK(17); }
                        if (shadow) { SECTK(18); }
                    }
                }
                if (COUNT) {
                    for (int k = 0; k < 2; k++) {
                        uint32_t v = c_wave[k];
                        for (int off = 32; off; off >>= 1) v = max(v, uint32_t(__shfl_xor(int(v), off)));
                        w_tot[k] += v;
                    }
                }
            }
            continue;
        }
        if (!alive || need_path) continue;

        if (COUNT) c_vertices++;
        SECTK(2);
        float dmed, t;
        stage_distance<MEDIUM>(rng, inv_sigma_t, dmed, t);
        const float tmin = ray_tmin(ro);
        uint32_t code = CODE_MISS, inst = 0;
        if constexpr (MEDIUM && BVH == 0 && !MONO)
            scan_primary<COUNT>(sc, ro, rd, tmin, t, code, COUNT ? a.counters + kCullCounters : nullptr);
        else
            closest_hit<BVH, COUNT, false, MONO>(sc, ro, rd, tmin, t, code, inst, stk, stride, c_nodes, c_btris);
        if (COUNT) c_rays++;
        SECTK(3);
        const bool hit = code != CODE_MISS;

        const bool ev_medium = MEDIUM && (dmed < (hit ? t : 400.f));
        const bool ev_surface = !ev_medium && hit;
        if (!ev_medium && !ev_surface) {
            SECTK(4);
            if constexpr (BVH == 0) {
                const V v = fma3(ldv(S_Q, Q), env_color(sc, rd), ldv(S_P, P));
                acc_add(MEDIUM ? v : vmin(v, ldv(S_RC, Rc)));
            } else {
                acc_add(vmin(fma3(Q, env_color(sc, rd), P), Rc));
            }
            need_path = true;
            continue;
        }

        V x, n = mk(0, 1, 0), mcol = mk(0, 0, 0), E;
        Mat mat = Mat{mk(0, 0, 0), 0.f, 0u, 0.f, 0.f};
        stage_event<COUNT, MONO>(a, tab, ro, rd, depth, ev_medium, dmed, t, code, inst, x, n, mcol, mat, E);

        for (uint32_t li = 0; li < sc.n_lights; li++) {
            const Light L = uload(&sc.lights[li]);
            if (L.kind == L_AMBIENT) {
                E = fma3(xyz(L.color), ev_medium ? mcol : mat_color(mat), E);
            } else if (L.kind == L_OBJECT) {
                V I, wi;
                float dist;
                SECTK(7);
                illuminate_object<GROUPS>(sc, L, x, rng, I, wi, dist, tab);
                if (L.twin_object >= 0) {
                    SECTK(8);
                    if constexpr (BVH == 0) {
                        float ts;
                        const bool visible = scan_light_visible<MONO>(sc, L, x, wi, dist, ts);
                        if (COUNT) c_rays++;
                        SECTK(9);
                        if (visible) stage_light_add<true>(sc, albedo_med, rd, ev_medium, I, wi, n, mcol, mat, E);
                    } else {
                        float ts = dist * (1.f + 1e-3f);
                        uint32_t cs = CODE_MISS, is = 0;
                        const bool range = L.twin_lo <= L.twin_hi;
                        closest_hit<BVH, COUNT, true, MONO>(sc, x, wi, ray_tmin(x), ts, cs, is, stk, stride, c_nodes, c_btris,
                                                            AnyHit{range ? dist * (1.f - 1e-3f) : -kInf, L.twin_lo, L.twin_hi});
                        if (COUNT) c_rays++;
                        SECTK(9);
                        stage_light_term<MONO>(sc, L, albedo_med, rd, ev_medium, ts, cs, is, dist, I, wi, n, mcol, mat, E);
                    }
                }
            }
        }

        V wi = mk(0, 0, 1), k = mk(0, 0, 0);
        const bool cont = stage_bounce<MEDIUM, COUNT>(a, albedo_med, rd, depth, ev_medium, n, mcol, mat, rng, wi, k);
        SECTK(14);
        if constexpr (BVH == 0) {
            const V q = ldv(S_Q, Q);
            const V pn = fma3(q, E, ldv(S_P, P));
            if (cont) {
                stv(S_P, P, pn);
                if (!MEDIUM) stv(S_RC, Rc, vmin(ldv(S_RC, Rc), fma3(100.f, q, pn)));
                stv(S_Q, Q, q * k);
                ro = x;
                rd = wi;
                depth++;
            } else {
                acc_add(MEDIUM ? pn : vmin(pn, ldv(S_RC, Rc)));
                need_path = true;
            }
        } else {
            P = fma3(Q, E, P);
            if (cont) {
                if (!MEDIUM) Rc = vmin(Rc, fma3(100.f, Q, P));
                Q = Q * k;
                ro = x;
                rd = wi;
                depth++;
            } else {
                acc_add(vmin(P, Rc));
                need_path = true;
            }
        }
    }

    if (COUNT) {
#ifdef RPT_SECT_CLOCKS
        if ((threadIdx.x & 63u) < 56u) atomicAdd(&a.counters[8 + (threadIdx.x & 63u)], sect_lds_[threadIdx.x >> 6][threadIdx.x & 63u]);
#endif
        atomicAdd(&a.counters[0], (unsigned long long)c_samples);
        atomicAdd(&a.counters[1], (unsigned long long)c_rays);
        atomicAdd(&a.counters[2], (unsigned long long)c_vertices);
        if ((threadIdx.x & 63u) == 0) atomicAdd(&a.counters[3], (unsigned long long)c_trips);
        if ((threadIdx.x & 63u) == 0) { atomicAdd(&a.counters[46], (unsigned long long)w_tot[0]); atomicAdd(&a.counters[47], (unsigned long long)w_tot[1]); }
        atomicAdd(&a.counters[5], (unsigned long long)c_nodes);
        if (c_nodes_primary) atomicAdd(&a.counters[61], (unsigned long long)c_nodes_primary);
        atomicAdd(&a.counters[6], (unsigned long long)c_btris);
    }
}

__global__ __launch_bounds__(256) void resolve_kernel(const RenderArgs a, double scale, double* __restrict__ out) {
    uint32_t p = blockIdx.x * 256u + threadIdx.x;
    if (p >= a.n_owned) return;
    uint32_t x, y;
    item_pixel(a, p, x, y);
    if (x >= a.width || y >= a.height) return;
    double r = 0.0, g = 0.0, b = 0.0;
    const float4* slab = reinterpret_cast<const float4*>(a.slab);
    for (uint32_t c = 0; c < a.n_chunks; c++) {
        float4 v = slab[size_t(c) * a.n_owned + p];
        r += double(v.x);
        g += double(v.y);
        b += double(v.z);
        if (a.slab2) {
            const float4 w = reinterpret_cast<const float4*>(a.slab2)[size_t(c) * a.n_owned + p];
            r += double(w.x);
            g += double(w.y);
            b += double(w.z);
        }
    }
    size_t o = (size_t(y) * a.width + x) * 3;
    double inv = scale / double(a.iterations);
    out[o] = r * inv;
    out[o + 1] = g * inv;
    out[o + 2] = b * inv;
}

__global__ __launch_bounds__(256) void buffer_add_kernel(uint32_t n_pixels, const double* __restrict__ batch,
                                                         double* __restrict__ sum, double* __restrict__ sumsq) {
    uint32_t p = blockIdx.x * 256u + threadIdx.x;
    if (p >= n_pixels) return;
    double r = batch[3 * size_t(p)], g = batch[3 * size_t(p) + 1], b = batch[3 * size_t(p) + 2];
    sum[3 * size_t(p)] += r;
    sum[3 * size_t(p) + 1] += g;
    sum[3 * size_t(p) + 2] += b;
    sumsq[p] += r * r + g * g + b * b;
}
__global__ __launch_bounds__(256) void buffer_image_kernel(uint32_t width, uint32_t height, uint32_t radius, uint32_t n_batches,
                                                           const double* __restrict__ sum, uint8_t* __restrict__ out) {
    uint32_t p = blockIdx.x * 256u + threadIdx.x;
    if (p >= width * height) return;
    uint32_t x = p % width, y = p / width;
    double r = 0.0, g = 0.0, b = 0.0;
    uint64_t count = 0;
    uint32_t x0 = x >= radius ? x - radius : 0u, y0 = y >= radius ? y - radius : 0u;
    for (uint32_t i = x0; i <= x + radius; i++)
        for (uint32_t j = y0; j <= y + radius; j++)
            if (i < width && j < height) {
                size_t q = size_t(j) * width + i;
                r += sum[3 * q];
                g += sum[3 * q + 1];
                b += sum[3 * q + 2];
                count += n_batches;
            }
    double c[3] = {r / double(count), g / double(count), b / double(count)};
    for (int k = 0; k < 3; k++) {
        double v = fmin(fmax(c[k], 0.0), 1.0);
        out[3 * size_t(p) + k] = uint8_t(pow(v, 1.0 / 2.2) * 255.0);
    }
}
__global__ __launch_bounds__(256) void buffer_variance_kernel(uint32_t n_pixels, uint32_t n_batches, const double* __restrict__ sum,
                                                              const double* __restrict__ sumsq, double* __restrict__ out) {
    uint32_t p = blockIdx.x * 256u + threadIdx.x;
    if (p >= n_pixels) return;
    double n = double(n_batches);
    double mr = sum[3 * size_t(p)] / n, mg = sum[3 * size_t(p) + 1] / n, mb = sum[3 * size_t(p) + 2] / n;
    double ss = sumsq[p] - n * (mr * mr + mg * mg + mb * mb);
    out[p] = fmax(ss, 0.0) / (n - 1.0);
}

template <bool PACK>
__global__ __launch_bounds__(256) void frame_tiles_kernel(const double* __restrict__ src, double* __restrict__ dst,
                                                          const uint32_t* __restrict__ tiles, uint32_t n_tiles, uint32_t tiles_x,
                                                          uint32_t width, uint32_t height) {
    const uint64_t e = uint64_t(blockIdx.x) * 256u + threadIdx.x;
    if (e >= uint64_t(n_tiles) * 3072u) return;
    const uint32_t t = uint32_t(e / 3072u), r = uint32_t(e % 3072u), p = r / 3u, c = r - 3u * p;
    const uint32_t tile = tiles[t], ty = tile / tiles_x, tx = tile - ty * tiles_x;
    const uint32_t x = tx * 32u + (p & 31u), y = ty * 32u + (p >> 5);
    const bool inside = x < width && y < height;
    const size_t f = (size_t(y) * width + x) * 3u + c;
    if (PACK) dst[e] = inside ? src[f] : 0.0;
    else if (inside) dst[f] = src[e];
// ... 244 lines not shown
        for (uint32_t j = 0; j < 32u; j++) bits |= uint32_t(REF ? r.below_ref(0.8f) : r.template below<kRoulette08>(0.8f)) << j;
        put(256u + h, bits);
    }
    r = start;
    for (uint32_t j = 0; j < 8u; j++) {
        uint32_t ku, kv;
        if (REF) triangle_pair_ref(r, ku, kv);
        else triangle_pair(r, ku, kv);
        put(258u + 2u * j, ku);
        put(259u + 2u * j, kv);
    }
}
__global__ __launch_bounds__(256) void debug_draw_forms_kernel(uint64_t seed_mixed, uint32_t n, float inv0, float inv1, float inv2,
                                                               uint32_t* __restrict__ out_new, uint32_t* __restrict__ out_ref) {
    const uint32_t i = blockIdx.x * 256u + threadIdx.x;
    if (i >= n) return;
    RngT<RPT_RNG_ALL> r;
    r.seed(seed_mixed, i, 0);
    draw_forms<false>(r, i, n, inv0, inv1, inv2, out_new);
    draw_forms<true>(r, i, n, inv0, inv1, inv2, out_ref);
}
template <bool MEDIUM>
__global__ __launch_bounds__(256) void debug_bounce_kernel(const RenderArgs a, const BounceArgs q) {
    const uint64_t i = uint64_t(blockIdx.x) * 256u + threadIdx.x;
    if (i >= q.n) return;
    Rng r;
    r.seed(q.seed_mixed, uint32_t(i), 0);
    V wi = mk(0.f, 0.f, 0.f), k = mk(0.f, 0.f, 0.f);
    const bool go = stage_bounce<MEDIUM, false>(a, q.albedo_med, mk(q.rd[3 * i], q.rd[3 * i + 1], q.rd[3 * i + 2]), q.depth,
                                                MEDIUM && q.medium_event != 0u, mk(q.nrm[3 * i], q.nrm[3 * i + 1], q.nrm[3 * i + 2]),
                                                mk(q.mcol[0], q.mcol[1], q.mcol[2]), mat_from(q.m), r, wi, k);
    q.flag[i] = go ? 1 : 0;
    q.wi[3 * i] = wi.x; q.wi[3 * i + 1] = wi.y; q.wi[3 * i + 2] = wi.z;
    q.k[3 * i] = k.x; q.k[3 * i + 1] = k.y; q.k[3 * i + 2] = k.z;
    q.next_word[i] = r.next();
}

static constexpr size_t kStackBytes = 32u * 256u * sizeof(uint32_t);
static constexpr size_t kTabBytes = (2u * 32u + 6u * 8u) * 16u;
static constexpr size_t kStateBytes = 18u * 256u * sizeof(uint32_t) + kTabBytes;
static constexpr size_t kStateBytesBvh = 5u * 256u * sizeof(uint32_t) + kTabBytes;
static constexpr size_t kMeshTreeBytes = (21u + 5u) * 256u * sizeof(uint32_t) + kTabBytes;
static constexpr size_t kDetachBytes = kDetachDwords * sizeof(uint32_t);
static_assert(kTabBytes == kTabDwords * 4u, "one table layout");

template <bool M, int B, bool C>
static hipError_t launch_render_t(const RenderArgs& a, int n_blocks, hipStream_t stream) {
    const size_t lds = B == 1 ? kMeshTreeBytes : B ? kStackBytes + kStateBytesBvh : kStateBytes;
    if (a.sc.n_mono) {
        if (a.sc.n_lparts) hipLaunchKernelGGL((render_kernel<M, B, false, true, 0, true>), dim3(n_blocks), dim3(256), lds, stream, a);
        else hipLaunchKernelGGL((render_kernel<M, B, false, false, 0, true>), dim3(n_blocks), dim3(256), lds, stream, a);
        return hipGetLastError();
    }
    if constexpr (M && B == 1) {
#ifdef RPT_EXPERIMENTS
        if (a.detach == 2 && !a.sc.n_lparts) {
            hipLaunchKernelGGL((render_kernel<true, 1, C, false, 2>), dim3(n_blocks), dim3(256), kDetachBytes, stream, a);
            return hipGetLastError();
        }
#endif
        if (a.detach && !a.sc.n_lparts) {
            hipLaunchKernelGGL((render_kernel<true, 1, C, false, 1>), dim3(n_blocks), dim3(256), kDetachBytes, stream, a);
            return hipGetLastError();
        }
    }
    if (a.sc.n_lparts) hipLaunchKernelGGL((render_kernel<M, B, false, true>), dim3(n_blocks), dim3(256), lds, stream, a);
    else hipLaunchKernelGGL((render_kernel<M, B, C>), dim3(n_blocks), dim3(256), lds, stream, a);
    return hipGetLastError();
}
template <bool M, bool C>
static hipError_t launch_render_b(const RenderArgs& a, int bvh, int n_blocks, hipStream_t stream) {
    if (bvh == 3) return launch_render_t<M, 3, C>(a, n_blocks, stream);
    if (bvh == 2) return launch_render_t<M, 2, C>(a, n_blocks, stream);
    if (bvh == 1) return launch_render_t<M, 1, C>(a, n_blocks, stream);
    return launch_render_t<M, 0, C>(a, n_blocks, stream);
}
int bvh_mode(const SceneView& sc) { return sc.scene_bvh ? ((sc.mesh_deferred && sc.n_mesh) ? 3 : 2) : (sc.n_nodes ? 1 : 0); }
hipError_t launch_render(const RenderArgs& a, int n_blocks, hipStream_t stream) {
    const bool m = a.sc.has_medium != 0, c = a.counters != nullptr;
    const int b = bvh_mode(a.sc);
    if (m) return c ? launch_render_b<true, true>(a, b, n_blocks, stream) : launch_render_b<true, false>(a, b, n_blocks, stream);
    return c ? launch_render_b<false, true>(a, b, n_blocks, stream) : launch_render_b<false, false>(a, b, n_blocks, stream);
}
size_t stream_scratch_bytes_per_block() { return size_t(kWaveScratchDwords) * 4u * 4u; }
hipError_t render_occupancy(bool medium, int bvh, int* blocks_per_cu, int detach) {
#ifdef RPT_EXPERIMENTS
    if (detach == 2 && medium && bvh == 1)
        return hipOccupancyMaxActiveBlocksPerMultiprocessor(blocks_per_cu, (const void*)render_kernel<true, 1, false, false, 2>, 256, kDetachBytes);
#endif
    if (detach && medium && bvh == 1)
        return hipOccupancyMaxActiveBlocksPerMultiprocessor(blocks_per_cu, (const void*)render_kernel<true, 1, false, false, 1>, 256, kDetachBytes);
    const void* f;
    if (bvh == 3) return hipOccupancyMaxActiveBlocksPerMultiprocessor(blocks_per_cu, medium ? (const void*)render_kernel<true, 3, false> : (const void*)render_kernel<false, 3, false>,
                                                                      256, kStackBytes + kStateBytesBvh);
    if (medium) f = bvh == 2 ? (const void*)render_kernel<true, 2, false> : bvh == 1 ? (const void*)render_kernel<true, 1, false> : (const void*)render_kernel<true, 0, false>;
    else f = bvh == 2 ? (const void*)render_kernel<false, 2, false> : bvh == 1 ? (const void*)render_kernel<false, 1, false> : (const void*)render_kernel<false, 0, false>;
    return hipOccupancyMaxActiveBlocksPerMultiprocessor(blocks_per_cu, f, 256, bvh == 1 ? kMeshTreeBytes : bvh ? kStackBytes + kStateBytesBvh : kStateBytes);
}
hipError_t launch_resolve(const RenderArgs& a, double scale, double* d_out, hipStream_t stream) {
    uint32_t blocks = (a.n_owned + 255u) / 256u;
    hipLaunchKernelGGL(resolve_kernel, dim3(blocks), dim3(256), 0, stream, a, scale, d_out);
    return hipGetLastError();
}
hipError_t launch_buffer_add(uint32_t n_pixels, const double* d_batch, double* d_sum, double* d_sumsq, hipStream_t st) {
    hipLaunchKernelGGL(buffer_add_kernel, dim3((n_pixels + 255) / 256), dim3(256), 0, st, n_pixels, d_batch, d_sum, d_sumsq);
    return hipGetLastError();
}
hipError_t launch_buffer_image(uint32_t w, uint32_t h, uint32_t radius, uint32_t n_batches, const double* d_sum, uint8_t* d_out,
                               hipStream_t st) {
    hipLaunchKernelGGL(buffer_image_kernel, dim3((w * h + 255) / 256), dim3(256), 0, st, w, h, radius, n_batches, d_sum, d_out);
    return hipGetLastError();
}
hipError_t launch_buffer_variance(uint32_t n_pixels, uint32_t n_batches, const double* d_sum, const double* d_sumsq, double* d_out,
                                  hipStream_t st) {
    hipLaunchKernelGGL(buffer_variance_kernel, dim3((n_pixels + 255) / 256), dim3(256), 0, st, n_pixels, n_batches, d_sum, d_sumsq,
                       d_out);
    return hipGetLastError();
}
hipError_t launch_frame_pack(const double* d_frame, double* d_packed, const uint32_t* d_tiles, uint32_t n_tiles, uint32_t tiles_x,
                             uint32_t width, uint32_t height, hipStream_t st) {
    if (!n_tiles) return hipSuccess;
    hipLaunchKernelGGL(frame_tiles_kernel<true>, dim3(n_tiles * 12u), dim3(256), 0, st, d_frame, d_packed, d_tiles, n_tiles, tiles_x, width, height);
    return hipGetLastError();
}
hipError_t launch_frame_unpack(const double* d_packed, double* d_frame, const uint32_t* d_tiles, uint32_t n_tiles, uint32_t tiles_x,
                               uint32_t width, uint32_t height, hipStream_t st) {
    if (!n_tiles) return hipSuccess;
    hipLaunchKernelGGL(frame_tiles_kernel<false>, dim3(n_tiles * 12u), dim3(256), 0, st, d_packed, d_frame, d_tiles, n_tiles, tiles_x, width, height);
    return hipGetLastError();
}
hipError_t launch_intersect(const SceneView& sc, uint64_t n, const float* d_o, const float* d_d, float* d_t,
                            int32_t* d_obj, float* d_n, bool bvh, hipStream_t stream) {
    uint32_t blocks = uint32_t((n + 255) / 256);
    if (sc.n_mono) {
        if (bvh) hipLaunchKernelGGL((intersect_kernel<2, true>), dim3(blocks), dim3(256), kStackBytes, stream, sc, n, d_o, d_d, d_t, d_obj, d_n);
        else hipLaunchKernelGGL((intersect_kernel<0, true>), dim3(blocks), dim3(256), 0, stream, sc, n, d_o, d_d, d_t, d_obj, d_n);
        return hipGetLastError();
    }
    if (bvh) hipLaunchKernelGGL(intersect_kernel<2>, dim3(blocks), dim3(256), kStackBytes, stream, sc, n, d_o, d_d, d_t, d_obj, d_n);
    else hipLaunchKernelGGL(intersect_kernel<0>, dim3(blocks), dim3(256), 0, stream, sc, n, d_o, d_d, d_t, d_obj, d_n);
    return hipGetLastError();
}
hipError_t launch_features(const FeatureArgs& a, hipStream_t stream) {
    if (!a.r.n_items) return hipSuccess;
    const dim3 grid((a.r.n_items + 255u) / 256u);
    const bool bvh = a.r.sc.n_nodes != 0;
    if (a.r.sc.n_mono) {
        if (bvh) hipLaunchKernelGGL((features_kernel<2, true>), grid, dim3(256), kStackBytes, stream, a);
        else hipLaunchKernelGGL((features_kernel<0, true>), grid, dim3(256), 0, stream, a);
        return hipGetLastError();
    }
    if (bvh) hipLaunchKernelGGL(features_kernel<2>, grid, dim3(256), kStackBytes, stream, a);
    else hipLaunchKernelGGL(features_kernel<0>, grid, dim3(256), 0, stream, a);
    return hipGetLastError();
}
hipError_t launch_feature_resolve(const FeatureResolveArgs& a, hipStream_t stream) {
    if (!a.n_owned) return hipSuccess;
    hipLaunchKernelGGL(feature_resolve_kernel, dim3((a.n_owned + 255u) / 256u), dim3(256), 0, stream, a);
    return hipGetLastError();
}
hipError_t launch_intersect_segments(const SceneView& sc, uint64_t n, const float* d_o, const float* d_d, const float* d_tmax, float* d_t,
                                     uint32_t* d_code, hipStream_t stream) {
    hipLaunchKernelGGL(intersect_segments_kernel, dim3(uint32_t((n + 255) / 256)), dim3(256), 0, stream, sc, n, d_o, d_d, d_tmax, d_t, d_code);
    return hipGetLastError();
}
hipError_t launch_debug_rng(uint64_t seed_mixed, uint32_t pixel, uint32_t sample, uint32_t n, uint32_t* d_out,
                            hipStream_t stream) {
    hipLaunchKernelGGL(debug_rng_kernel, dim3(1), dim3(64), 0, stream, seed_mixed, pixel, sample, n, d_out);
    return hipGetLastError();
}
hipError_t launch_debug_sample_f(const Material& m, uint64_t n, const float* d_n, const float* d_wo,
                                 uint64_t seed_mixed, float* d_wi, float* d_pdf, int32_t* d_some, hipStream_t s) {
    hipLaunchKernelGGL(debug_sample_f_kernel, dim3(uint32_t((n + 255) / 256)), dim3(256), 0, s, m, n, d_n, d_wo, seed_mixed,
                       d_wi, d_pdf, d_some);
    return hipGetLastError();
}
hipError_t launch_debug_bsdf(const Material& m, uint64_t n, const float* d_n, const float* d_wo, const float* d_wi,
                             float* d_out, hipStream_t s) {
    hipLaunchKernelGGL(debug_bsdf_kernel, dim3(uint32_t((n + 255) / 256)), dim3(256), 0, s, m, n, d_n, d_wo, d_wi, d_out);
    return hipGetLastError();
}
hipError_t launch_debug_camera_sample(const CameraG& cam, uint32_t w, uint32_t h, float inv_dim, uint64_t seed_mixed, uint32_t sample,
                                      float* d_o, float* d_d, uint32_t* d_next_word, hipStream_t s) {
    hipLaunchKernelGGL(debug_camera_kernel, dim3((w * h + 255) / 256), dim3(256), 0, s, cam, w, h, inv_dim, seed_mixed, sample, d_o, d_d,
                       d_next_word);
    return hipGetLastError();
}
hipError_t launch_debug_light_sample(const SceneView& sc, const LightSampleArgs& q, hipStream_t s) {
    const dim3 grid(uint32_t((q.n + 255) / 256));
    if (sc.n_lparts) hipLaunchKernelGGL(debug_light_sample_kernel<true>, grid, dim3(256), 0, s, sc, q);
    else hipLaunchKernelGGL(debug_light_sample_kernel<false>, grid, dim3(256), 0, s, sc, q);
    return hipGetLastError();
}
hipError_t launch_debug_env_color(const SceneView& sc, uint64_t n, const float* d_dirs, float* d_rgb, hipStream_t s) {
    hipLaunchKernelGGL(debug_env_color_kernel, dim3(uint32_t((n + 255) / 256)), dim3(256), 0, s, sc, n, d_dirs, d_rgb);
    return hipGetLastError();
}
hipError_t launch_debug_medium_distance(const SceneView& sc, uint64_t n, uint64_t seed_mixed, float* d_dmed, float* d_limit,
                                        hipStream_t s) {
    hipLaunchKernelGGL(debug_medium_distance_kernel, dim3(uint32_t((n + 255) / 256)), dim3(256), 0, s, sc, n, seed_mixed, d_dmed, d_limit);
    return hipGetLastError();
}
hipError_t launch_debug_shadow_test(const SceneView& sc, const ShadowTestArgs& q, hipStream_t s) {
    const dim3 grid(uint32_t((q.n + 255) / 256));
    if (sc.n_mono) hipLaunchKernelGGL(debug_shadow_test_kernel<true>, grid, dim3(256), 0, s, sc, q);
    else hipLaunchKernelGGL(debug_shadow_test_kernel<false>, grid, dim3(256), 0, s, sc, q);
    return hipGetLastError();
}
hipError_t launch_debug_distance_pair(float sigma_t, uint32_t k0, uint32_t n, float* d_new, float* d_guarded, hipStream_t s) {
    hipLaunchKernelGGL(debug_distance_pair_kernel, dim3((n + 255u) / 256u), dim3(256), 0, s, sigma_t, k0, n, d_new, d_guarded);
    return hipGetLastError();
}
hipError_t launch_debug_draw_forms(uint64_t seed_mixed, uint32_t n, const float inv[3], uint32_t* d_new, uint32_t* d_ref, hipStream_t s) {
    hipLaunchKernelGGL(debug_draw_forms_kernel, dim3((n + 255u) / 256u), dim3(256), 0, s, seed_mixed, n, inv[0], inv[1], inv[2], d_new, d_ref);
    return hipGetLastError();
}
hipError_t launch_debug_bounce(const BounceArgs& q, hipStream_t s) {
    RenderArgs a{};
    a.max_bounces = q.max_bounces;
    const dim3 grid(uint32_t((q.n + 255) / 256));
    if (q.in_medium) hipLaunchKernelGGL(debug_bounce_kernel<true>, grid, dim3(256), 0, s, a, q);
    else hipLaunchKernelGGL(debug_bounce_kernel<false>, grid, dim3(256), 0, s, a, q);
    return hipGetLastError();
}

}
```

### rpt_amd/csrc/rpt_capi.cpp

```cpp
#include <hip/hip_runtime_api.h>

#include <algorithm>
#include <cfloat>
#include <cmath>
#include <cstdio>
#include <cstring>
#include <functional>
#include <limits>
#include <memory>
#include <mutex>
#include <string>
#include <unordered_map>
#include <vector>

#include "../../include/rpt_hip.h"
#include "host_internal.h"
#include "kernels.h"
#include "f64_layout.h"

using namespace rptg;

static thread_local std::string g_err;
namespace rpti {
int fail(int code, const std::string& msg) {
    g_err = msg;
    return code;
}
}
using rpti::fail;
namespace rpti {
uint64_t seed_mix(uint64_t seed) {
    uint64_t x = seed + 0x9E3779B97F4A7C15ULL;
    x ^= x >> 30;
    x *= 0xBF58476D1CE4E5B9ULL;
    x ^= x >> 27;
    x *= 0x94D049BB133111EBULL;
    x ^= x >> 31;
    return x;
}
}
#define HIP_TRY(expr)                                                                              \
    do {                                                                                           \
        hipError_t e__ = (expr);                                                                   \
        if (e__ != hipSuccess)                                                                     \
            return fail(RPT_ERR_DEVICE, std::string(#expr) + ": " + hipGetErrorString(e__));       \
    } while (0)

struct rpt_options {
    int64_t counters = 0;
    int64_t chunk_spp = 0;
    int64_t blocks_per_cu = 0;
    int64_t max_blocks = 0;
    int64_t timing = 0;
    int64_t room_shell = 1;
    int64_t scan_specialise = 1;
    int64_t scan_cull = 1;
    int64_t shadow_scan = 1;
    int64_t photon_skip = 0;
    int64_t photon_block_lists = 1;
    int64_t photon_coop_gather = 1;
    int64_t photon_split = 0;
    int64_t photon_parts = 4;
    int64_t instancing = 1;
    int64_t bvh_leaf_max = 4;
    int64_t bvh_max_depth = 20;
    int64_t bvh_sweep_below = 4096;
    int64_t defer_stop = 16;
    int64_t walk_leaf_quarters = 6;
    int64_t defer_lanes = 32;
    int64_t detach_shadows = 1;
    int64_t stream_backlog = 48;
    int64_t stream_contexts = 1;
    int64_t detach_lanes = 44;
    int64_t pull_batch = 2;
    int64_t detach_trigger = 28;
    int64_t scene_bvh_min = 64;
    int64_t scene_tree_meshes = 0;
    int64_t f64_cull = 1;
    int64_t f64_mesh_tree_min = 64;
    int64_t f64_photon_slice = 0;
    int64_t f64_surf_batch = 8;
    int64_t denoise_stage = -1;
    int64_t epsilon_policy = 0;
};
static rpt_options g_defaults;
static std::mutex g_defaults_mutex;
static int set_option_in(rpt_options& o, const char* name, int64_t value) {
    if (!name) return fail(RPT_ERR_INVALID, "null option name");
    const std::string s(name);
    if (s == "counters") o.counters = value;
    else if (s == "chunk_spp") { if (value < 0) return fail(RPT_ERR_INVALID, "chunk_spp must be >= 0 (0 = auto)"); o.chunk_spp = value; }
    else if (s == "blocks_per_cu") o.blocks_per_cu = value;
    else if (s == "max_blocks") { if (value < 0 || value > (1 << 20)) return fail(RPT_ERR_INVALID, "max_blocks must be 0..2^20 (0 = no cap)"); o.max_blocks = value; }
    else if (s == "timing") o.timing = value;
    else if (s == "room_shell") o.room_shell = value;
    else if (s == "scan_specialise") o.scan_specialise = value;
    else if (s == "scan_cull") o.scan_cull = value;
    else if (s == "shadow_scan") o.shadow_scan = value;
    else if (s == "photon_skip") o.photon_skip = value;
    else if (s == "photon_block_lists") o.photon_block_lists = value;
    else if (s == "photon_parts") o.photon_parts = value;
    else if (s == "photon_split") {
#ifndef RPT_EXPERIMENTS
        if (value != 0) return fail(RPT_ERR_UNSUPPORTED, "photon_split: a rejected prototype, built with -DRPT_EXPERIMENTS only");
#endif
        o.photon_split = value;
    }
    else if (s == "photon_coop_gather") o.photon_coop_gather = value;
    else if (s == "instancing") o.instancing = value;
    else if (s == "defer_lanes") { if (value < 1 || value > 64) return fail(RPT_ERR_INVALID, "defer_lanes must be 1..64"); o.defer_lanes = value; }
    else if (s == "bvh_leaf_max") { if (value < 1 || value > 16) return fail(RPT_ERR_INVALID, "bvh_leaf_max must be 1..16"); o.bvh_leaf_max = value; }
    else if (s == "bvh_sweep_below") { if (value < 0) return fail(RPT_ERR_INVALID, "bvh_sweep_below must be >= 0"); o.bvh_sweep_below = value; }
    else if (s == "bvh_max_depth") { if (value < 1 || value > 20) return fail(RPT_ERR_INVALID, "bvh_max_depth must be 1..20"); o.bvh_max_depth = value; }
    else if (s == "walk_leaf_quarters") { if (value < 0 || value > 256) return fail(RPT_ERR_INVALID, "walk_leaf_quarters must be 0..256"); o.walk_leaf_quarters = value; }
    else if (s == "detach_shadows") {
        if (value < 0 || value > 2) return fail(RPT_ERR_INVALID, "detach_shadows must be 0, 1 or 2");
#ifndef RPT_EXPERIMENTS
        if (value == 2) return fail(RPT_ERR_UNSUPPORTED, "detach_shadows = 2 (streamed walks): a rejected prototype, built with -DRPT_EXPERIMENTS only");
#endif
        o.detach_shadows = value;
    }
    else if (s == "stream_contexts") { if (value < 1 || value > 6) return fail(RPT_ERR_INVALID, "stream_contexts must be 1..6"); o.stream_contexts = value; }
    else if (s == "stream_backlog") { if (value < 1 || value > 256) return fail(RPT_ERR_INVALID, "stream_backlog must be 1..256"); o.stream_backlog = value; }
    else if (s == "detach_lanes") { if (value < 1 || value > 96) return fail(RPT_ERR_INVALID, "detach_lanes must be 1..96"); o.detach_lanes = value; }
    else if (s == "pull_batch") { if (value < 1 || value > 64) return fail(RPT_ERR_INVALID, "pull_batch must be 1..64"); o.pull_batch = value; }
    else if (s == "detach_trigger") { if (value < 1 || value > 32) return fail(RPT_ERR_INVALID, "detach_trigger must be 1..32"); o.detach_trigger = value; }
    else if (s == "defer_stop") { if (value < 1 || value > 64) return fail(RPT_ERR_INVALID, "defer_stop must be 1..64"); o.defer_stop = value; }
    else if (s == "f64_cull") { if (value < 0 || value > 2) return fail(RPT_ERR_INVALID, "f64_cull must be 0, 1 or 2"); o.f64_cull = value; }
    else if (s == "f64_mesh_tree_min") { if (value < 0 || value > (int64_t(1) << 32)) return fail(RPT_ERR_INVALID, "f64_mesh_tree_min must be 0..2^32"); o.f64_mesh_tree_min = value; }
    else if (s == "f64_photon_slice") { if (value < 0 || value > (1 << 20)) return fail(RPT_ERR_INVALID, "f64_photon_slice must be 0..2^20"); o.f64_photon_slice = value; }
    else if (s == "f64_surf_batch") { if (value < 1 || value > 64) return fail(RPT_ERR_INVALID, "f64_surf_batch must be 1..64"); o.f64_surf_batch = value; }
    else if (s == "epsilon_policy") { if (value < 0 || value > 1) return fail(RPT_ERR_INVALID, "epsilon_policy must be 0 or 1"); o.epsilon_policy = value; }
    else if (s == "denoise_stage") {
        if (value < -1 || value > int64_t(rptg::kDenoiseMaxStagedStep)) return fail(RPT_ERR_INVALID, "denoise_stage must be -1 (default), 0, 1 or 2");
        o.denoise_stage = value;
    }
    else if (s == "scene_tree_meshes") o.scene_tree_meshes = value;
    else if (s == "scene_bvh_min") { if (value < 0) return fail(RPT_ERR_INVALID, "scene_bvh_min must be >= 0"); o.scene_bvh_min = value; }
    else return fail(RPT_ERR_INVALID, "unknown option: " + s);
    return RPT_OK;
}

namespace {
struct D3 {
    double x, y, z;
};
inline D3 operator+(D3 a, D3 b) { return {a.x + b.x, a.y + b.y, a.z + b.z}; }
inline D3 operator-(D3 a, D3 b) { return {a.x - b.x, a.y - b.y, a.z - b.z}; }
inline D3 operator*(double s, D3 a) { return {s * a.x, s * a.y, s * a.z}; }
inline double dot(D3 a, D3 b) { return a.x * b.x + a.y * b.y + a.z * b.z; }
inline D3 cross(D3 a, D3 b) { return {a.y * b.z - a.z * b.y, a.z * b.x - a.x * b.z, a.x * b.y - a.y * b.x}; }
inline D3 normalize(D3 a) {
    double l = std::sqrt(dot(a, a));
    return {a.x / l, a.y / l, a.z / l};
}
inline D3 d3(const double* p) { return {p[0], p[1], p[2]}; }
inline double comp(const D3& v, int a) { return a == 0 ? v.x : (a == 1 ? v.y : v.z); }
inline F4 f4(D3 v, double w) { return F4{float(v.x), float(v.y), float(v.z), float(w)}; }
inline float bits_f(uint32_t u) {
    float f;
    std::memcpy(&f, &u, 4);
    return f;
}
inline uint32_t bits_u(float f) {
    uint32_t u;
    std::memcpy(&u, &f, 4);
    return u;
}

struct Xf {
    bool has = false;
    double M[4][4], Minv[4][4], L[3][3], N[3][3], det = 1.0;
    D3 point(D3 p) const { return {M[0][0] * p.x + M[0][1] * p.y + M[0][2] * p.z + M[0][3], M[1][0] * p.x + M[1][1] * p.y + M[1][2] * p.z + M[1][3], M[2][0] * p.x + M[2][1] * p.y + M[2][2] * p.z + M[2][3]}; }
    D3 normal(D3 n) const { return {N[0][0] * n.x + N[0][1] * n.y + N[0][2] * n.z, N[1][0] * n.x + N[1][1] * n.y + N[1][2] * n.z, N[2][0] * n.x + N[2][1] * n.y + N[2][2] * n.z}; }
};
bool invert4(const double a[4][4], double out[4][4]) {
    double w[4][8];
    for (int i = 0; i < 4; i++)
        for (int j = 0; j < 4; j++) {
            w[i][j] = a[i][j];
            w[i][4 + j] = i == j ? 1.0 : 0.0;
// ... 256 lines not shown
            for (int a = 1; a < 3; a++)
                if (chi[a] - clo[a] > chi[axis] - clo[axis]) axis = a;
            mid = first + count / 2;
            std::nth_element(t.begin() + first, t.begin() + mid, t.begin() + first + count,
                             [axis](const BTri& p, const BTri& q) { return p.c[axis] < q.c[axis]; });
        } else if (best_axis < 0 || depth >= kMaxDepth) {
            if (count <= 16 && leaf_ok) return make_leaf();
            mid = first + count / 2;
        } else {
            float parent_cost = area(lo, hi) * float(count);
            if (best_cost >= parent_cost && count <= 8 && leaf_ok) return make_leaf();
            float ext = chi[best_axis] - clo[best_axis];
            float scale = float(kBins) / ext;
            auto it = std::partition(t.begin() + first, t.begin() + first + count, [&](const BTri& x) {
                int b = std::min(kBins - 1, int((x.c[best_axis] - clo[best_axis]) * scale));
                return b <= best_bin;
            });
            mid = uint32_t(it - t.begin());
            if (mid == first || mid == first + count) mid = first + count / 2;
        }
        uint32_t left = uint32_t(nodes.size());
        nodes.push_back(TmpNode{});
        nodes.push_back(TmpNode{});
        nodes[node].left_or_first = left;
        nodes[node].count = 0;
        build(left, first, mid - first, depth + 1);
        build(left + 1, mid, first + count - mid, depth + 1);
    }
};

template <class T>
struct DevBuf {
    T* p = nullptr;
    size_t n = 0;
};

}

struct rpt_scene {
    std::vector<HObject> objects;
    std::vector<HLight> lights;
    std::vector<HMedium> media;
    double env[3] = {0, 0, 0};
    uint32_t hdri_w = 0, hdri_h = 0;
    std::vector<float> hdri;
    std::vector<double> hdri64;
    bool committed = false;
    rpt_options opt;
    int device = 0;
    int n_cus = 256;
    SceneView view{};
    struct LaunchSet {
        rpti::DevMem d_slab;
        rpti::DevMem d_queue;
        rpti::DevMem d_stream;
        rpti::Event done;
        rpti::Event launched;
        hipStream_t stream = nullptr;
        bool used = false;
    };
    struct Device {
        rpti::DevMem arena;
        rpti::DevMem arena64;
        rpti::DevMem d_tiles;
        LaunchSet sets[2];
        rpti::DevMem d_counters;
        rpti::DevMem d_out;
        rpti::DevMem d_feat_slab, d_feat_out;
        rpti::Event feat_done;
        bool feat_used = false;
        std::vector<rpti::Event> evs;
    } dev;
    int cur_set = 0;
    uint64_t last_counters[64] = {0};
    uint64_t last_cull[12] = {0};
    static constexpr size_t kTimedLaunches = 1024;
    size_t ev_count = 0;
    int last_blocks = 0;
    uint64_t prims_per_ray = 0;
    uint32_t n_twin_lights = 0;
    std::vector<Light> light_records;
    bool twins_scanned = false;
    uint64_t stats[16] = {0};
    void* photon = nullptr;
    rpt64::Scene view64{};
    double medium_color64[3] = {0, 0, 0}, medium_color_hi64[3] = {0, 0, 0};
    const rpt64::MeshNode* mnodes64 = nullptr;
    const uint32_t* mleaf64 = nullptr;
    const uint32_t* mroot64 = nullptr;
    uint64_t mesh_tree_info64[8] = {0};
    uint64_t last_counters64[64] = {0};
    std::unordered_map<uint64_t, std::vector<std::shared_ptr<const std::vector<double>>>> mesh_pool;
    uint32_t tk_w = 0, tk_h = 0, tk_rank = 0, tk_count = 0, n_tiles = 0, tiles_x = 0;
};

using MeshCallCache = std::unordered_map<const double*, std::pair<uint64_t, std::shared_ptr<const std::vector<double>>>>;
static std::shared_ptr<const std::vector<double>> intern_mesh(rpt_scene* s, const double* p, uint64_t n_tris,
                                                              MeshCallCache& seen) {
    auto it = seen.find(p);
    if (it != seen.end() && it->second.first == n_tris) return it->second.second;
    const size_t n = size_t(n_tris) * 18;
    uint64_t h = 0xCBF29CE484222325ULL ^ n;
    for (size_t i = 0; i < n; i++) {
        uint64_t w;
        std::memcpy(&w, p + i, 8);
        h = (h ^ w) * 0x100000001B3ULL;
        h ^= h >> 29;
    }
    auto& bucket = s->mesh_pool[h];
    for (auto& c : bucket)
        if (c->size() == n && std::memcmp(c->data(), p, n * 8) == 0) { seen[p] = {n_tris, c}; return c; }
    auto m = std::make_shared<const std::vector<double>>(p, p + n);
    bucket.push_back(m);
    seen[p] = {n_tris, m};
    return m;
}
static bool copy_shape(rpt_scene* s, MeshCallCache& seen, const rpt_shape_desc* d, HShape& out, std::string& why,
                       int depth = 0) {
    if (!d) { why = "null shape"; return false; }
    if (d->kind < 0 || d->kind > RPT_SHAPE_MONOMIAL) { why = "unknown shape kind"; return false; }
    if (d->kind == RPT_SHAPE_MONOMIAL && !std::isfinite(d->plane_normal[0])) { why = "MonomialSurface height must be finite"; return false; }
    out.d = *d;
    out.mesh.reset();
    out.children.clear();
    if (d->kind == RPT_SHAPE_MESH) {
        if (d->n_tris == 0 || !d->tris) { why = "mesh without triangles"; return false; }
        out.mesh = intern_mesh(s, d->tris, d->n_tris, seen);
    }
    if (d->kind == RPT_SHAPE_GROUP) {
        if (d->n_children == 0 || !d->children) { why = "group without children"; return false; }
        if (depth >= 16) { why = "groups nested too deeply"; return false; }
        out.children.resize(d->n_children);
        for (uint64_t i = 0; i < d->n_children; i++) {
            if (d->children[i].kind == RPT_SHAPE_PLANE) { why = "Plane is not Bounded and cannot be a KdTree child (src/kdtree.rs:12)"; return false; }
            if (!copy_shape(s, seen, d->children + i, out.children[i], why, depth + 1)) return false;
        }
    }
    out.d.tris = nullptr;
    out.d.children = nullptr;
    Xf x;
    if (!make_xf(*d, x)) { why = "singular transform"; return false; }
    return true;
}
static bool holds_monomial(const HShape& h) {
    if (h.d.kind == RPT_SHAPE_MONOMIAL) return true;
    for (const HShape& c : h.children)
        if (holds_monomial(c)) return true;
    return false;
}
static bool check_material(const rpt_material* m, std::string& why) {
    if (!m) { why = "null material"; return false; }
    if (m->kind < 0 || m->kind > RPT_MAT_TRANSMISSIVE) { why = "unknown material kind"; return false; }
    return true;
}

extern "C" {

const char* rpt_last_error(void) { return g_err.c_str(); }

int rpt_device_count(void) {
    int n = 0;
    if (hipGetDeviceCount(&n) != hipSuccess) return 0;
    return n;
}

int rpt_set_option(const char* name, int64_t value) {
    std::lock_guard<std::mutex> lock(g_defaults_mutex);
    return set_option_in(g_defaults, name, value);
}
int rpt_scene_set_option(rpt_scene* s, const char* name, int64_t value) {
    if (!s) return fail(RPT_ERR_INVALID, "null scene");
    return set_option_in(s->opt, name, value);
}

rpt_scene* rpt_scene_create(void) {
    rpt_scene* s = new rpt_scene();
    std::lock_guard<std::mutex> lock(g_defaults_mutex);
    s->opt = g_defaults;
    return s;
}

static void release_device(rpt_scene* s) {
    if (!s->committed && !s->dev.arena && !s->dev.arena64) return;
    (void)hipSetDevice(s->device);
    s->dev = rpt_scene::Device{};
    if (s->photon) rpti::photon_release(s->photon);
    s->photon = nullptr;
    s->committed = false;
}

void rpt_scene_destroy(rpt_scene* s) {
    if (!s) return;
    release_device(s);
    delete s;
}

int rpt_scene_add_object(rpt_scene* s, const rpt_shape_desc* d, const rpt_material* m) {
    if (!s) return fail(RPT_ERR_INVALID, "null scene");
    if (s->committed) return fail(RPT_ERR_STATE, "scene is immutable after rpt_scene_commit");
    std::string why;
    HObject o;
    MeshCallCache seen;
    if (!copy_shape(s, seen, d, o.shape, why) || !check_material(m, why)) return fail(RPT_ERR_INVALID, why);
    o.mat = *m;
    s->objects.push_back(std::move(o));
    return int(s->objects.size()) - 1;
}
static int add_simple_light(rpt_scene* s, int kind, const double* color, const double* vec) {
    if (!s || !color) return fail(RPT_ERR_INVALID, "null argument");
    if (s->committed) return fail(RPT_ERR_STATE, "scene is immutable after rpt_scene_commit");
    HLight l{};
    l.kind = kind;
    std::memcpy(l.color, color, 24);
    if (vec) std::memcpy(l.vec, vec, 24);
    s->lights.push_back(std::move(l));
    return RPT_OK;
}
int rpt_scene_add_light_point(rpt_scene* s, const double color[3], const double location[3]) {
    if (!location) return fail(RPT_ERR_INVALID, "null location");
    return add_simple_light(s, L_POINT, color, location);
}
int rpt_scene_add_light_ambient(rpt_scene* s, const double color[3]) { return add_simple_light(s, L_AMBIENT, color, nullptr); }
int rpt_scene_add_light_directional(rpt_scene* s, const double color[3], const double direction[3]) {
    if (!direction) return fail(RPT_ERR_INVALID, "null direction");
    return add_simple_light(s, L_DIRECTIONAL, color, direction);
}
int rpt_scene_add_light_object(rpt_scene* s, const rpt_shape_desc* d, const rpt_material* m) {
    if (!s) return fail(RPT_ERR_INVALID, "null scene");
    if (s->committed) return fail(RPT_ERR_STATE, "scene is immutable after rpt_scene_commit");
    std::string why;
    HLight l{};
    l.kind = L_OBJECT;
    MeshCallCache seen;
    if (!copy_shape(s, seen, d, l.obj.shape, why) || !check_material(m, why)) return fail(RPT_ERR_INVALID, why);
    if (d->kind == RPT_SHAPE_PLANE)
        return fail(RPT_ERR_INVALID, "a plane cannot be a Light::Object (Plane::sample is unimplemented in rpt)");
    if (holds_monomial(l.obj.shape))
        return fail(RPT_ERR_UNSUPPORTED, "a MonomialSurface (alone or in a KdTree group) cannot be a Light::Object: MonomialSurface::sample "
                                         "is not built (src/shape/monomial_surface.rs:109-123)");
    l.obj.mat = *m;
    s->lights.push_back(std::move(l));
    return RPT_OK;
}
int rpt_scene_add_medium(rpt_scene* s, int32_t kind, double absorption, double scattering) {
    if (!s) return fail(RPT_ERR_INVALID, "null scene");
    if (s->committed) return fail(RPT_ERR_STATE, "scene is immutable after rpt_scene_commit");
    if (kind != RPT_MEDIUM_HOMOGENEOUS_ISOTROPIC && kind != RPT_MEDIUM_COLORED_GLOWING_FOG)
        return fail(RPT_ERR_INVALID, "unknown medium kind");
    if (!(absorption + scattering > 0.0)) return fail(RPT_ERR_INVALID, "medium extinction must be > 0");
    s->media.push_back(HMedium{kind, absorption, scattering});
    return RPT_OK;
}
int rpt_scene_set_environment_color(rpt_scene* s, const double rgb[3]) {
    if (!s || !rgb) return fail(RPT_ERR_INVALID, "null argument");
    if (s->committed) return fail(RPT_ERR_STATE, "scene is immutable after rpt_scene_commit");
    std::memcpy(s->env, rgb, 24);
    s->hdri_w = s->hdri_h = 0;
    s->hdri.clear();
    s->hdri64.clear();
    return RPT_OK;
}
int rpt_scene_set_environment_hdri(rpt_scene* s, uint32_t width, uint32_t height, const double* rgb) {
    if (!s || !rgb) return fail(RPT_ERR_INVALID, "null argument");
    if (s->committed) return fail(RPT_ERR_STATE, "scene is immutable after rpt_scene_commit");
    if (width == 0 || height == 0) return fail(RPT_ERR_INVALID, "Hdri::new asserts width > 0 && height > 0");
    s->hdri_w = width;
    s->hdri_h = height;
    s->hdri.resize(size_t(width) * height * 4);
    s->hdri64.assign(rgb, rgb + size_t(width) * height * 3);
    for (size_t i = 0; i < size_t(width) * height; i++) {
        s->hdri[4 * i] = float(rgb[3 * i]); s->hdri[4 * i + 1] = float(rgb[3 * i + 1]); s->hdri[4 * i + 2] = float(rgb[3 * i + 2]);
// ... 1660 lines not shown
    a.n_owned = a.n_tiles * 1024u;
    uint64_t n_items = uint64_t(a.n_owned) * a.n_chunks;
    if (n_items >= (1ull << 32) - (1ull << 24)) return fail(RPT_ERR_INVALID, "too many work items; raise chunk_spp");
    a.n_items = uint32_t(n_items);
    if (!launch_set) return RPT_OK;
    size_t slab_bytes = std::max<size_t>(size_t(n_items) * slab_item_bytes, 16);
    if (s->dev.sets[s->cur_set].used && s->dev.sets[s->cur_set].stream != st) s->cur_set ^= 1;
    rpt_scene::LaunchSet& ls = s->dev.sets[s->cur_set];
    if (ls.used && ls.stream != st) HIP_TRY(hipStreamWaitEvent(st, ls.done.get(), 0));
    HIP_TRY(ls.d_slab.reserve(slab_bytes));
    ls.stream = st;
    ls.used = true;
    a.slab = ls.d_slab.get<float>();
    a.queue = ls.d_queue.get<unsigned long long>();
    a.counters = s->opt.counters ? s->dev.d_counters.get<unsigned long long>() : nullptr;
    a.lds_stack = s->view.n_nodes ? 1u : 0u;
    a.defer_lanes = uint32_t(s->opt.defer_lanes);
    a.defer_stop = uint32_t(std::min(s->opt.defer_stop, s->opt.defer_lanes));
    a.walk_leaf_quarters = uint32_t(s->opt.walk_leaf_quarters);
    a.detach = 0;
    if (s->opt.detach_shadows && s->view.has_medium && bvh_mode(s->view) == 1 && s->view.n_lparts == 0 && s->twins_scanned)
        a.detach = (s->opt.detach_shadows == 2 && s->n_twin_lights <= 3) ? 2u : 1u;
    a.stream_backlog = uint32_t(s->opt.stream_backlog);
    a.stream_contexts = uint32_t(s->opt.stream_contexts);
    a.n_twin_lights = s->n_twin_lights;
    a.stream_scratch = nullptr;
    a.pull_batch = uint32_t(s->opt.pull_batch);
    a.detach_trigger = uint32_t(s->opt.detach_trigger);
    if (a.detach) {
        a.defer_lanes = uint32_t(s->opt.detach_lanes);
        a.defer_stop = uint32_t(std::min<int64_t>(s->opt.defer_stop, std::min(s->opt.detach_lanes, s->opt.detach_trigger)));
    }
    return RPT_OK;
}

extern "C++" int rpti::serialize_with_other_streams(rpt_scene* s, hipStream_t st) {
    for (auto& ls : s->dev.sets)
        if (ls.used && ls.stream != st) HIP_TRY(hipStreamWaitEvent(st, ls.done.get(), 0));
    return RPT_OK;
}

extern "C++" int rpti::run_persistent(rpt_scene* s, const rpt_render_params* prm, const RenderArgs& a, double* d_out, hipStream_t st,
                         int blocks_per_cu, const std::function<hipError_t(const RenderArgs&, int, hipStream_t)>& launch,
                         bool indexed_start, bool wave_items, const std::function<hipError_t(double, double*, hipStream_t)>& resolve,
                         bool clear_sharded) {
    const int k = s->dev.sets[0].d_queue.get() == a.queue ? 0 : 1;
    rpt_scene::LaunchSet& mine = s->dev.sets[k];
    rpt_scene::LaunchSet& other = s->dev.sets[k ^ 1];
    if (other.used && other.stream != st) HIP_TRY(hipStreamWaitEvent(st, other.launched.get(), 0));
    HIP_TRY(hipMemsetAsync(a.queue, 0, 8, st));
    if (a.counters) HIP_TRY(hipMemsetAsync(a.counters, 0, 640, st));
    uint32_t shard_count = prm->shard_count == 0 ? 1 : prm->shard_count;
    if (shard_count > 1 && clear_sharded) HIP_TRY(hipMemsetAsync(d_out, 0, size_t(prm->width) * prm->height * 24, st));
    if (a.n_items) {
        uint64_t want = wave_items ? (uint64_t(a.n_items) + 3) / 4 : (uint64_t(a.n_items) + 255) / 256;
        int n_blocks = int(std::min<uint64_t>(uint64_t(s->n_cus) * std::max(blocks_per_cu, 1), want));
        if (s->opt.max_blocks > 0) n_blocks = int(std::min<int64_t>(n_blocks, s->opt.max_blocks));
        s->last_blocks = n_blocks;
        if (indexed_start) HIP_TRY(hipMemsetD32Async((hipDeviceptr_t)a.queue, int(uint32_t(n_blocks) * 4u * 64u), 1, st));
        const rpti::Event* ev = nullptr;
        if (s->opt.timing) {
            const size_t slot = s->ev_count % rpt_scene::kTimedLaunches;
            while (s->dev.evs.size() < 3 * (slot + 1)) {
                rpti::Event e;
                HIP_TRY(e.create());
                s->dev.evs.push_back(std::move(e));
            }
            ev = &s->dev.evs[3 * slot];
            HIP_TRY(hipEventRecord(ev[0].get(), st));
        }
        HIP_TRY(hipEventRecord(mine.launched.get(), st));
        HIP_TRY(launch(a, n_blocks, st));
        if (ev) HIP_TRY(hipEventRecord(ev[1].get(), st));
        if (resolve) HIP_TRY(resolve(std::pow(2.0, prm->exposure_value), d_out, st));
        else HIP_TRY(launch_resolve(a, std::pow(2.0, prm->exposure_value), d_out, st));
        if (ev) {
            HIP_TRY(hipEventRecord(ev[2].get(), st));
            s->ev_count++;
        }
    }
    HIP_TRY(hipEventRecord(mine.done.get(), st));
    return RPT_OK;
}
static int run_render(rpt_scene* s, const rpt_render_params* prm, const RenderArgs& a_in, double* d_out, hipStream_t st) {
    RenderArgs a = a_in;
    int bpc = int(s->opt.blocks_per_cu);
    if (bpc <= 0) {
        HIP_TRY(render_occupancy(a.sc.has_medium != 0, bvh_mode(a.sc), &bpc, int(a.detach)));
        if (bpc < 1) bpc = 1;
    }
    if (a.detach == 2) {
        rpt_scene::LaunchSet& ls = s->dev.sets[s->dev.sets[0].d_queue.get() == a.queue ? 0 : 1];
        HIP_TRY(ls.d_stream.reserve(size_t(s->n_cus) * size_t(bpc) * stream_scratch_bytes_per_block()));
        a.stream_scratch = ls.d_stream.get<uint32_t>();
    }
    return rpti::run_persistent(s, prm, a, d_out, st, bpc,
                                [](const RenderArgs& ra, int nb, hipStream_t stream) { return launch_render(ra, nb, stream); }, true);
}
extern "C++" rpti::SceneDev rpti::scene_dev(rpt_scene* s) {
    int first = -1;
    for (size_t i = 0; i < s->lights.size(); i++)
        if (s->lights[i].kind == L_OBJECT) { first = int(i); break; }
    bool mono = false;
    for (const auto& o : s->objects) mono = mono || holds_monomial(o.shape);
    return SceneDev{s->committed, s->device, s->n_cus, s->view, first, bool(s->dev.arena64), mono};
}
extern "C++" void*& rpti::photon_slot(rpt_scene* s) { return s->photon; }
extern "C++" int64_t rpti::option_photon_skip(rpt_scene* s) { return s->opt.photon_skip; }
extern "C++" int64_t rpti::option_max_blocks(rpt_scene* s) { return s->opt.max_blocks; }
extern "C++" int64_t rpti::option_f64_photon_slice(rpt_scene* s) { return s->opt.f64_photon_slice; }
extern "C++" int64_t rpti::option_photon_block_lists(rpt_scene* s) { return s->opt.photon_block_lists; }
extern "C++" int64_t rpti::option_photon_parts(rpt_scene* s) { return s->opt.photon_parts; }
extern "C++" int64_t rpti::option_photon_split(rpt_scene* s) { return s->opt.photon_split; }
extern "C++" int64_t rpti::option_photon_coop_gather(rpt_scene* s) { return s->opt.photon_coop_gather; }
extern "C++" double* rpti::scratch_out(rpt_scene* s, size_t bytes) {
    return s->dev.d_out.reserve(bytes) == hipSuccess ? s->dev.d_out.get<double>() : nullptr;
}
extern "C++" int rpti::fetch_counters(rpt_scene* s, const RenderArgs& a) {
    std::memset(s->last_counters, 0, sizeof(s->last_counters));
    std::memset(s->last_cull, 0, sizeof(s->last_cull));
    if (a.counters) {
        HIP_TRY(hipMemcpy(s->last_counters, a.counters, 512, hipMemcpyDeviceToHost));
        HIP_TRY(hipMemcpy(s->last_cull, a.counters + 64, sizeof(s->last_cull), hipMemcpyDeviceToHost));
        s->last_counters[4] = s->last_counters[1] * s->prims_per_ray;
    }
    return RPT_OK;
}

int rpt_render_sample_device(rpt_scene* s, const rpt_camera* cam, const rpt_render_params* prm, uint32_t iterations,
                             uint64_t seed, uint32_t sample_offset, void* d_out_rgb, void* hip_stream) {
    if (!d_out_rgb) return fail(RPT_ERR_INVALID, "null output");
    if (s && s->dev.arena64) return run_render64(s, cam, prm, iterations, seed, sample_offset, static_cast<double*>(d_out_rgb), static_cast<hipStream_t>(hip_stream));
    RenderArgs a{};
    int rc = rpti::prepare_render(s, static_cast<hipStream_t>(hip_stream), cam, prm, iterations, seed, sample_offset, a);
    if (rc) return rc;
    rc = run_render(s, prm, a, static_cast<double*>(d_out_rgb), static_cast<hipStream_t>(hip_stream));
    if (rc) return rc;
    if (a.counters) {
        HIP_TRY(hipStreamSynchronize(static_cast<hipStream_t>(hip_stream)));
        return rpti::fetch_counters(s, a);
    }
    return RPT_OK;
}

int rpt_render_sample(rpt_scene* s, const rpt_camera* cam, const rpt_render_params* prm, uint32_t iterations,
                      uint64_t seed, uint32_t sample_offset, double* out_rgb) {
    if (!out_rgb) return fail(RPT_ERR_INVALID, "null output");
    RenderArgs a{};
    int rc = rpti::prepare_render(s, nullptr, cam, prm, iterations, seed, sample_offset, a);
    if (rc) return rc;
    size_t bytes = size_t(prm->width) * prm->height * 24;
    double* d_out = rpti::scratch_out(s, bytes);
    if (!d_out) return fail(RPT_ERR_DEVICE, "out of device memory");
    if (s->dev.arena64) {
        rc = run_render64(s, cam, prm, iterations, seed, sample_offset, d_out, nullptr);
        if (rc) return rc;
        HIP_TRY(hipMemcpy(out_rgb, d_out, bytes, hipMemcpyDeviceToHost));
        return RPT_OK;
    }
    rc = run_render(s, prm, a, d_out, nullptr);
    if (rc) return rc;
    HIP_TRY(hipMemcpy(out_rgb, d_out, bytes, hipMemcpyDeviceToHost));
    return rpti::fetch_counters(s, a);
}
static int use_tile_list(RenderArgs& a, const uint32_t* d_tiles, uint32_t n_tiles) {
    if (n_tiles > a.n_tiles) return fail(RPT_ERR_INVALID, "more tiles listed than the frame has");
    a.tiles = d_tiles;
    a.n_tiles = n_tiles;
    a.n_owned = n_tiles * 1024u;
    const uint64_t n_items = uint64_t(a.n_owned) * a.n_chunks;
    if (n_items >= (1ull << 32) - (1ull << 24)) return fail(RPT_ERR_INVALID, "too many work items; raise chunk_spp");
    a.n_items = uint32_t(n_items);
    return RPT_OK;
}
static int check_sample_tiles(const rpt_scene* s, const rpt_camera* cam, const rpt_render_params* prm, uint32_t iterations, const void* tiles,
                              uint32_t n_tiles, const void* out) {
    if (!s || !cam || !prm) return fail(RPT_ERR_INVALID, "null argument");
    if (!out) return fail(RPT_ERR_INVALID, "null output");
    if (n_tiles && !tiles) return fail(RPT_ERR_INVALID, "null tile list");
    if (prm->width == 0 || prm->height == 0 || iterations == 0) return fail(RPT_ERR_INVALID, "empty render");
// ... 733 lines not shown
    HIP_TRY(launch_debug_light_sample(s->view, q, nullptr));
    HIP_TRY(hipMemcpy(v, q.v, n * 12, hipMemcpyDeviceToHost));
    HIP_TRY(hipMemcpy(nrm, q.nrm, n * 12, hipMemcpyDeviceToHost));
    HIP_TRY(hipMemcpy(intensity, q.intensity, n * 12, hipMemcpyDeviceToHost));
    HIP_TRY(hipMemcpy(wi, q.wi, n * 12, hipMemcpyDeviceToHost));
    HIP_TRY(hipMemcpy(pdf, q.pdf, n * 4, hipMemcpyDeviceToHost));
    HIP_TRY(hipMemcpy(dist, q.dist, n * 4, hipMemcpyDeviceToHost));
    HIP_TRY(hipMemcpy(next_word, q.next_word, n * 4, hipMemcpyDeviceToHost));
    return RPT_OK;
}
int rpt_debug_env_color(rpt_scene* s, uint64_t n, const float* dirs, float* rgb) {
    if (!s || !dirs || !rgb) return fail(RPT_ERR_INVALID, "null argument");
    if (!s->committed) return fail(RPT_ERR_STATE, "rpt_scene_commit must be called first");
    if (s->dev.arena64) return fail(RPT_ERR_STATE, "rpt_debug_env_color: the scene was committed with epsilon_policy = 1 (rpt_debug_env_color_f64)");
    if (!launch_debug_env_color) return fail(RPT_ERR_UNSUPPORTED, "rpt_debug_env_color: built without the kernels");
    if (n == 0) return RPT_OK;
    HIP_TRY(hipSetDevice(s->device));
    rpti::DevMem d_d, d_c;
    HIP_TRY(hook_scratch(d_d, n * 12));
    HIP_TRY(hook_scratch(d_c, n * 12));
    HIP_TRY(hipMemcpy(d_d.get(), dirs, n * 12, hipMemcpyHostToDevice));
    HIP_TRY(launch_debug_env_color(s->view, n, d_d.get<float>(), d_c.get<float>(), nullptr));
    HIP_TRY(hipMemcpy(rgb, d_c.get(), n * 12, hipMemcpyDeviceToHost));
    return RPT_OK;
}
int rpt_debug_medium_distance(rpt_scene* s, uint64_t n, uint64_t seed, float* dmed, float* t_limit) {
    if (!s || !dmed || !t_limit) return fail(RPT_ERR_INVALID, "null argument");
    if (s->media.empty()) return fail(RPT_ERR_INVALID, "rpt_debug_medium_distance: the scene has no medium");
    if (!s->committed) return fail(RPT_ERR_STATE, "rpt_scene_commit must be called first");
    if (s->dev.arena64) return fail(RPT_ERR_STATE, "rpt_debug_medium_distance: the scene was committed with epsilon_policy = 1");
    if (!launch_debug_medium_distance) return fail(RPT_ERR_UNSUPPORTED, "rpt_debug_medium_distance: built without the kernels");
    if (n == 0) return RPT_OK;
    if (n > 0xFFFFFFFFull) return fail(RPT_ERR_INVALID, "rpt_debug_medium_distance: the case number keys a 32-bit stream field");
    HIP_TRY(hipSetDevice(s->device));
    rpti::DevMem d_m, d_t;
    HIP_TRY(hook_scratch(d_m, n * 4));
    HIP_TRY(hook_scratch(d_t, n * 4));
    HIP_TRY(launch_debug_medium_distance(s->view, n, seed_mix(seed), d_m.get<float>(), d_t.get<float>(), nullptr));
    HIP_TRY(hipMemcpy(dmed, d_m.get(), n * 4, hipMemcpyDeviceToHost));
    HIP_TRY(hipMemcpy(t_limit, d_t.get(), n * 4, hipMemcpyDeviceToHost));
    return RPT_OK;
}
int rpt_debug_shadow_test(rpt_scene* s, uint32_t light, uint64_t n, const float* origins, const float* dirs, const float* dist,
                          int32_t* out_flag, float* out_t) {
    if (!s || !origins || !dirs || !dist || !out_flag || !out_t) return fail(RPT_ERR_INVALID, "null argument");
    if (rpti::light_kind(s, light) != int(L_OBJECT)) return fail(RPT_ERR_INVALID, "rpt_debug_shadow_test: not a Light::Object");
    if (!s->committed) return fail(RPT_ERR_STATE, "rpt_scene_commit must be called first");
    if (s->dev.arena64) return fail(RPT_ERR_STATE, "rpt_debug_shadow_test: the scene was committed with epsilon_policy = 1");
    if (s->view.n_nodes != 0 || s->view.scene_bvh || s->view.n_inst)
        return fail(RPT_ERR_UNSUPPORTED, "rpt_debug_shadow_test: the scene has a tree (the query is the linear scan's)");
    if (!launch_debug_shadow_test) return fail(RPT_ERR_UNSUPPORTED, "rpt_debug_shadow_test: built without the kernels");
    if (n == 0) return RPT_OK;
    HIP_TRY(hipSetDevice(s->device));
    rpti::DevMem d_in, d_out;
    HIP_TRY(hook_scratch(d_in, n * 28));
    HIP_TRY(hook_scratch(d_out, n * 8));
    float* const in = d_in.get<float>();
    HIP_TRY(hipMemcpy(in, origins, n * 12, hipMemcpyHostToDevice));
    HIP_TRY(hipMemcpy(in + 3 * n, dirs, n * 12, hipMemcpyHostToDevice));
    HIP_TRY(hipMemcpy(in + 6 * n, dist, n * 4, hipMemcpyHostToDevice));
    ShadowTestArgs q{};
    q.light = light;
    q.n = n;
    q.o = in; q.d = in + 3 * n; q.dist = in + 6 * n;
    q.flag = d_out.get<int32_t>();
    q.t = d_out.get<float>() + n;
    HIP_TRY(launch_debug_shadow_test(s->view, q, nullptr));
    HIP_TRY(hipMemcpy(out_flag, q.flag, n * 4, hipMemcpyDeviceToHost));
    HIP_TRY(hipMemcpy(out_t, q.t, n * 4, hipMemcpyDeviceToHost));
    return RPT_OK;
}
int rpt_shadow_scan_info(rpt_scene* s, uint32_t light, uint32_t out[4]) {
    if (!s || !out) return fail(RPT_ERR_INVALID, "null argument");
    if (rpti::light_kind(s, light) != int(L_OBJECT)) return fail(RPT_ERR_INVALID, "rpt_shadow_scan_info: not a Light::Object");
    if (!s->committed) return fail(RPT_ERR_STATE, "rpt_scene_commit must be called first");
    if (s->dev.arena64) return fail(RPT_ERR_STATE, "rpt_shadow_scan_info: the scene was committed with epsilon_policy = 1");
    if (light >= s->light_records.size()) return fail(RPT_ERR_STATE, "rpt_shadow_scan_info: the light was added after the commit");
    const Light& L = s->light_records[light];
    out[0] = L.twin_lo;
    out[1] = L.twin_hi;
    out[2] = (bits_u(L.color.w) != 0u && bvh_mode(s->view) == 0) ? 1u : 0u;
    out[3] = uint32_t(L.twin_object);
    return RPT_OK;
}
int rpt_debug_distance_pair(float sigma_t, uint32_t k0, uint32_t n, float* out_new, float* out_guarded) {
    if (!out_new || !out_guarded) return fail(RPT_ERR_INVALID, "null argument");
    if (!(sigma_t > 0.f) || !(sigma_t < INFINITY)) return fail(RPT_ERR_INVALID, "rpt_debug_distance_pair: sigma_t must be positive and finite");
    if (k0 >= (1u << 23) || n > (1u << 23) - k0) return fail(RPT_ERR_INVALID, "rpt_debug_distance_pair: a draw has 23 bits (k0 + n <= 2^23)");
    if (!launch_debug_distance_pair) return fail(RPT_ERR_UNSUPPORTED, "rpt_debug_distance_pair: built without the kernels");
    if (n == 0) return RPT_OK;
    rpti::DevMem d_out;
    HIP_TRY(hook_scratch(d_out, size_t(n) * 8));
    HIP_TRY(launch_debug_distance_pair(sigma_t, k0, n, d_out.get<float>(), d_out.get<float>() + n, nullptr));
    HIP_TRY(hipMemcpy(out_new, d_out.get<float>(), size_t(n) * 4, hipMemcpyDeviceToHost));
    HIP_TRY(hipMemcpy(out_guarded, d_out.get<float>() + n, size_t(n) * 4, hipMemcpyDeviceToHost));
    return RPT_OK;
}

int rpt_debug_draw_forms(uint64_t seed, uint32_t n, uint32_t* out_new, uint32_t* out_ref) {
    if (!out_new || !out_ref) return fail(RPT_ERR_INVALID, "null argument");
    if (n > (1u << 20)) return fail(RPT_ERR_INVALID, "rpt_debug_draw_forms: at most 2^20 lanes");
    if (!launch_debug_draw_forms) return fail(RPT_ERR_UNSUPPORTED, "rpt_debug_draw_forms: built without the kernels");
    if (n == 0) return RPT_OK;
    const size_t bytes = size_t(n) * kDrawFormWords * 4;
    const float inv[3] = {1.f / 64.f, 1.f / 1024.f, 1.f / 3000.f};
    rpti::DevMem d_new, d_ref;
    HIP_TRY(hook_scratch(d_new, bytes));
    HIP_TRY(hook_scratch(d_ref, bytes));
    HIP_TRY(launch_debug_draw_forms(seed_mix(seed), n, inv, d_new.get<uint32_t>(), d_ref.get<uint32_t>(), nullptr));
    HIP_TRY(hipMemcpy(out_new, d_new.get(), bytes, hipMemcpyDeviceToHost));
    HIP_TRY(hipMemcpy(out_ref, d_ref.get(), bytes, hipMemcpyDeviceToHost));
    return RPT_OK;
}

int rpt_debug_bounce(const rpt_material* m, uint32_t max_bounces, uint32_t depth, int32_t in_medium, int32_t medium_event,
                     float albedo_med, const float* medium_color, uint64_t n, const float* normals, const float* rds, uint64_t seed,
                     int32_t* flag, float* wi, float* k, uint32_t* next_word) {
    std::string why;
    if (!check_material(m, why)) return fail(RPT_ERR_INVALID, why);
    if (!medium_color || !normals || !rds || !flag || !wi || !k || !next_word) return fail(RPT_ERR_INVALID, "null argument");
    if (medium_event && !in_medium) return fail(RPT_ERR_INVALID, "rpt_debug_bounce: a medium event needs in_medium");
    if (n > 0xFFFFFFFFull) return fail(RPT_ERR_INVALID, "rpt_debug_bounce: the case number keys a 32-bit stream field");
    if (!launch_debug_bounce) return fail(RPT_ERR_UNSUPPORTED, "rpt_debug_bounce: built without the kernels");
    if (n == 0) return RPT_OK;
    rpti::DevMem d_in, d_out;
    HIP_TRY(hook_scratch(d_in, n * 24));
    HIP_TRY(hook_scratch(d_out, n * 32));
    float* const in = d_in.get<float>();
    float* const o = d_out.get<float>();
    HIP_TRY(hipMemcpy(in, normals, n * 12, hipMemcpyHostToDevice));
    HIP_TRY(hipMemcpy(in + 3 * n, rds, n * 12, hipMemcpyHostToDevice));
    BounceArgs q{};
    q.m = to_gpu_material(m);
    q.max_bounces = max_bounces;
    q.depth = depth;
    q.in_medium = in_medium ? 1u : 0u;
    q.medium_event = medium_event ? 1u : 0u;
    q.albedo_med = albedo_med;
    for (int i = 0; i < 3; i++) q.mcol[i] = medium_color[i];
    q.n = n;
    q.seed_mixed = seed_mix(seed);
    q.nrm = in; q.rd = in + 3 * n;
    q.wi = o; q.k = o + 3 * n;
    q.flag = reinterpret_cast<int32_t*>(o + 6 * n);
    q.next_word = reinterpret_cast<uint32_t*>(o + 7 * n);
    HIP_TRY(launch_debug_bounce(q, nullptr));
    HIP_TRY(hipMemcpy(wi, q.wi, n * 12, hipMemcpyDeviceToHost));
    HIP_TRY(hipMemcpy(k, q.k, n * 12, hipMemcpyDeviceToHost));
    HIP_TRY(hipMemcpy(flag, q.flag, n * 4, hipMemcpyDeviceToHost));
    HIP_TRY(hipMemcpy(next_word, q.next_word, n * 4, hipMemcpyDeviceToHost));
    return RPT_OK;
}

}
```

Measured before the change: 15150 Msamples/s.

## JIT-specialize the primitive scan kernel on scene shape constants via hiprtc

Adds a runtime path that compiles the render kernel with hiprtc, with the scene's primitive counts, shell, cull and rotation masks baked in as compile-time constants. The scan loops can then be unrolled and dead branches dropped. The compiled code object is cached in memory and on disk, and is only used if its VGPR count does not exceed the ahead-of-time kernel's. The cost is compile time on a cache miss, a default threshold of 2^27 camera samples before compiling, and more build and load complexity with fallbacks.

```diff
diff --git a/include/rpt_hip.h b/include/rpt_hip.h
--- a/include/rpt_hip.h
+++ b/include/rpt_hip.h
@@ -211,6 +211,17 @@
 int rpt_debug_shadow_test(rpt_scene*, uint32_t light, uint64_t n, const float* origins, const float* dirs, const float* dist,
                           int32_t* out_flag, float* out_t);
 int rpt_shadow_scan_info(rpt_scene*, uint32_t light, uint32_t out[4]);
+#define RPT_SCAN_JIT_OFF 0
+#define RPT_SCAN_JIT_IDLE 1
+#define RPT_SCAN_JIT_ACTIVE 2
+#define RPT_SCAN_JIT_FALLBACK 3
+#define RPT_SCAN_JIT_OUT_OF_SCOPE 4
+#define RPT_SCAN_JIT_CACHE_NONE 0
+#define RPT_SCAN_JIT_CACHE_MEMORY 1
+#define RPT_SCAN_JIT_CACHE_DISK 2
+#define RPT_SCAN_JIT_CACHE_MISS 3
+int rpt_scan_jit_info(rpt_scene*, int64_t out[8], char* text, uint64_t text_capacity);
+int rpt_scan_jit_forget(void);
 int rpt_debug_distance_pair(float sigma_t, uint32_t k0, uint32_t n, float* out_new, float* out_guarded);
 int rpt_debug_draw_forms(uint64_t seed, uint32_t n, uint32_t* out_new, uint32_t* out_ref);
 
diff --git a/rpt_amd/_lib.py b/rpt_amd/_lib.py
--- a/rpt_amd/_lib.py
+++ b/rpt_amd/_lib.py
@@ -192,6 +192,8 @@
     ("rpt_debug_distance_pair", C.c_int, [C.c_float, C.c_uint32, C.c_uint32, _P, _P]),
     ("rpt_debug_draw_forms", C.c_int, [C.c_uint64, C.c_uint32, _P, _P]),
     ("rpt_shadow_scan_info", C.c_int, [_P, C.c_uint32, C.POINTER(C.c_uint32)]),
+    ("rpt_scan_jit_info", C.c_int, [_P, C.POINTER(C.c_int64), _P, C.c_uint64]),
+    ("rpt_scan_jit_forget", C.c_int, []),
     ("rpt_debug_material_f64", C.c_int, [C.POINTER(MaterialDesc), C.c_uint64, _P, _P, C.c_uint64, _P, _P, _P, _P, _P]),
     ("rpt_debug_material_bsdf_f64", C.c_int, [C.POINTER(MaterialDesc), C.c_uint64, _P, _P, _P, _P]),
 ]
diff --git a/rpt_amd/api.py b/rpt_amd/api.py
--- a/rpt_amd/api.py
+++ b/rpt_amd/api.py
@@ -1239,6 +1239,15 @@
         _lib.check(_lib.load().rpt_shadow_scan_info(self.scene._commit(self.device_), light_index, out))
         return {"twin_lo": int(out[0]), "twin_hi": int(out[1]), "shadow_form": int(out[2]), "twin_object": int(np.int32(np.uint32(out[3])))}
 
+    def scan_jit_info(self):
+        out = (C.c_int64 * 8)()
+        text = C.create_string_buffer(2048)
+        _lib.check(_lib.load().rpt_scan_jit_info(self.scene._commit(self.device_), out, C.cast(text, C.c_void_p), len(text)))
+        shape, _, reason = text.value.decode(errors="replace").partition("\n")
+        return {"state": ("off", "idle", "active", "fallback", "out_of_scope")[int(out[0])], "cache": ("none", "memory", "disk", "miss")[int(out[1])],
+                "compile_ms": out[2] / 1000.0, "vgprs": int(out[3]), "scratch": int(out[4]), "launches": int(out[5]), "compiles": int(out[6]),
+                "aot_vgprs": int(out[7]), "shape": shape, "reason": reason}
+
 
 def debug_distance_pair(sigma_t, k0, n):
     new, guarded = np.empty(n, np.float32), np.empty(n, np.float32)
diff --git a/rpt_amd/csrc/device_core.h b/rpt_amd/csrc/device_core.h
--- a/rpt_amd/csrc/device_core.h
+++ b/rpt_amd/csrc/device_core.h
@@ -1,9 +1,26 @@
 #pragma once
+#ifndef __HIPCC_RTC__
 #include <hip/hip_runtime.h>
 #include <type_traits>
+#endif
 #include "gpu_layout.h"
 
 namespace rptg {
+
+#ifndef __HIPCC_RTC__
+namespace tt = std;
+#else
+namespace tt {
+template <bool B> struct bool_constant { static constexpr bool value = B; };
+typedef bool_constant<true> true_type;
+typedef bool_constant<false> false_type;
+template <class A, class B> inline constexpr bool is_same_v = false;
+template <class A> inline constexpr bool is_same_v<A, A> = true;
+template <bool C, class A, class B> struct conditional { typedef A type; };
+template <class A, class B> struct conditional<false, A, B> { typedef B type; };
+template <bool C, class A, class B> using conditional_t = typename conditional<C, A, B>::type;
+}
+#endif
 
 #define RPT_DEV __device__ __forceinline__
 
@@ -514,41 +531,77 @@
     uint32_t kind, lo, span;
     RPT_DEV bool has(uint32_t i) const { return i - lo <= span; }
 };
-template <bool MASKED = false, bool MONO = false, bool TAIL = false, bool SHADOW = false>
+struct ScanShapeRt {
+    KernargView sc;
+    RPT_DEV uint32_t n_sph() const { return sc->n_sph; }
+    RPT_DEV uint32_t n_cub() const { return sc->n_cub; }
+    RPT_DEV uint32_t n_pln() const { return sc->n_pln; }
+    RPT_DEV uint32_t n_aabb() const { return sc->n_aabb; }
+    RPT_DEV uint32_t n_rect_x() const { return sc->n_rect_x; }
+    RPT_DEV uint32_t n_rect_y() const { return sc->n_rect_y; }
+    RPT_DEV uint32_t n_rect_z() const { return sc->n_rect_z; }
+    RPT_DEV uint32_t n_tri() const { return sc->n_tri; }
+    RPT_DEV uint32_t has_shell() const { return sc->has_shell; }
+    RPT_DEV uint32_t scan_cull() const { return sc->scan_cull; }
+    RPT_DEV uint64_t sph_yrot() const { return sc->sph_yrot; }
+    RPT_DEV uint64_t cub_yrot() const { return sc->cub_yrot; }
+};
+#ifdef RPT_SCAN_SHAPE
+struct ScanShapeK {
+    KernargView sc;
+    static constexpr uint64_t k[12] = {RPT_SCAN_SHAPE};
+    RPT_DEV constexpr uint32_t n_sph() const { return uint32_t(k[0]); }
+    RPT_DEV constexpr uint32_t n_cub() const { return uint32_t(k[1]); }
+    RPT_DEV constexpr uint32_t n_pln() const { return uint32_t(k[2]); }
+    RPT_DEV constexpr uint32_t n_aabb() const { return uint32_t(k[3]); }
+    RPT_DEV constexpr uint32_t n_rect_x() const { return uint32_t(k[4]); }
+    RPT_DEV constexpr uint32_t n_rect_y() const { return uint32_t(k[5]); }
+    RPT_DEV constexpr uint32_t n_rect_z() const { return uint32_t(k[6]); }
+    RPT_DEV constexpr uint32_t n_tri() const { return uint32_t(k[7]); }
+    RPT_DEV constexpr uint32_t has_shell() const { return uint32_t(k[8]); }
+    RPT_DEV constexpr uint32_t scan_cull() const { return uint32_t(k[9]); }
+    RPT_DEV constexpr uint64_t sph_yrot() const { return k[10]; }
+    RPT_DEV constexpr uint64_t cub_yrot() const { return k[11]; }
+};
+#else
+typedef ScanShapeRt ScanShapeK;
+#endif
+template <bool MASKED = false, bool MONO = false, bool TAIL = false, bool SHADOW = false, class SHAPE = ScanShapeRt>
 RPT_DEV void scan_prims(const SceneView& scene, V o, V d, float tmin, float& tbest, uint32_t& code, uint64_t mask = ~0ull,
                         bool* tail_skipped = nullptr, ShadowTwin twin = ShadowTwin{0u, 1u, 0u}, bool* best_is_twin = nullptr) {
     static_assert(!(TAIL && MASKED), "one cull at a time");
     static_assert(!(SHADOW && (MASKED || TAIL)), "the shadow form is a plain scan");
     const auto& sc = *kernarg_scene();
     (void)scene;
+    const SHAPE sh{&sc};
     bool flag = false;
     float t_twin = __builtin_nanf("");
     auto acc = [&](bool ok, float t, uint32_t c, auto is_twin) {
         if (ok) tbest = t;
         asm volatile("" : "+v"(tbest));
         if constexpr (!SHADOW) { if (ok) code = c; }
-        else if constexpr (std::is_same_v<decltype(is_twin), std::false_type>) flag = flag && !ok;
+        else if constexpr (tt::is_same_v<decltype(is_twin), tt::false_type>) flag = flag && !ok;
         else if (ok && is_twin) t_twin = t;
     };
     auto twin_at = [&](auto tw, uint32_t i) {
         if constexpr (decltype(tw)::value) return twin.has(i);
-        else return std::false_type{};
+        else return tt::false_type{};
     };
     auto kind_loop = [&](uint32_t kind, auto&& loop) {
         if constexpr (SHADOW) {
             if (twin.kind == kind) {
-                loop(std::true_type{});
+                loop(tt::true_type{});
                 flag = t_twin == tbest;
                 return;
             }
         }
-        loop(std::false_type{});
+        loop(tt::false_type{});
     };
     uint32_t bit = 0;
     auto on = [&](uint32_t i) { return !MASKED || ((mask >> ((bit + i) & 63u)) & 1ull) != 0ull; };
-    const uint64_t sph_yrot = MASKED ? 0ull : sc.sph_yrot, cub_yrot = MASKED ? 0ull : sc.cub_yrot;
+    const uint64_t sph_yrot = MASKED ? 0ull : sh.sph_yrot(), cub_yrot = MASKED ? 0ull : sh.cub_yrot();
     kind_loop(K_SPHERE, [&](auto tw) {
-        for (uint32_t i = 0; i < sc.n_sph; i++) {
+        for (uint32_t i = 0; i < sh.n_sph(); i++) {
             if (!on(i)) continue;
             const XfScan x = uload(&sc.sph[i]);
             V ol, dl;
@@ -558,11 +611,11 @@
             acc(sphere_closer(ol, dl, tmin, tbest, t), t, (K_SPHERE << 28) | i, twin_at(tw, i));
         }
     });
-    bit += sc.n_sph;
+    bit += sh.n_sph();
     kind_loop(K_CUBE, [&](auto tw) {
         uint32_t i = 0;
         if (!MASKED)
-            for (; i + 1u < sc.n_cub; i += 2u) {
+            for (; i + 1u < sh.n_cub(); i += 2u) {
                 const XfScan x0 = uload(&sc.cub[i]), x1 = uload(&sc.cub[i + 1u]);
                 V ol0, dl0, ol1, dl1;
                 float t0, t1;
@@ -576,7 +629,7 @@
                 acc(cube_closer(ol0, dl0, tmin, tbest, t0), t0, (K_CUBE << 28) | i, twin_at(tw, i));
                 acc(cube_closer(ol1, dl1, tmin, tbest, t1), t1, (K_CUBE << 28) | (i + 1u), twin_at(tw, i + 1u));
             }
-        for (; i < sc.n_cub; i++) {
+        for (; i < sh.n_cub(); i++) {
             if (!on(i)) continue;
             const XfScan x = uload(&sc.cub[i]);
             V ol, dl;
@@ -586,22 +639,22 @@
             acc(cube_closer(ol, dl, tmin, tbest, t), t, (K_CUBE << 28) | i, twin_at(tw, i));
         }
     });
-    bit += sc.n_cub;
-    for (uint32_t i = 0; i < sc.n_pln; i++) {
+    bit += sh.n_cub();
+    for (uint32_t i = 0; i < sh.n_pln(); i++) {
         const F4 nv = uload(&sc.pln[i]).nv;
         float t;
-        acc(plane_closer(nv, o, d, tmin, tbest, t), t, (K_PLANE << 28) | i, std::false_type{});
-    }
-    const uint32_t n_rect = sc.n_rect_x + sc.n_rect_y + sc.n_rect_z;
-    if (sc.n_aabb + n_rect + sc.has_shell != 0) {
+        acc(plane_closer(nv, o, d, tmin, tbest, t), t, (K_PLANE << 28) | i, tt::false_type{});
+    }
+    const uint32_t n_rect = sh.n_rect_x() + sh.n_rect_y() + sh.n_rect_z();
+    if (sh.n_aabb() + n_rect + sh.has_shell() != 0) {
         const V inv = mk(rcp(d.x), rcp(d.y), rcp(d.z));
-        if (sc.has_shell)
+        if (sh.has_shell())
             shell_closer(uload(sc.shell), o, inv, tmin, tbest, [&](bool ok, float t, auto code_of) {
-                if constexpr (SHADOW) acc(ok, t, 0u, std::false_type{});
+                if constexpr (SHADOW) acc(ok, t, 0u, tt::false_type{});
                 else { if (ok) { tbest = t; code = code_of(); } }
             });
         if constexpr (TAIL) {
-            if (sc.scan_cull) {
+            if (sh.scan_cull()) {
                 const SceneView::ScanBox tb = kernarg_load(&sc.scan_tail);
                 if (__ballot(interval_meets_box<false>(tb, o, inv, tmin, tbest)) == 0ull) {
                     if (tail_skipped) *tail_skipped = true;
@@ -612,28 +665,28 @@
         kind_loop(K_AABB, [&](auto tw) {
             uint32_t i = 0;
             if (!MASKED)
-                for (; i + 1u < sc.n_aabb; i += 2u) {
+                for (; i + 1u < sh.n_aabb(); i += 2u) {
                     const AabbScan b0 = uload(&sc.aabb[i]), b1 = uload(&sc.aabb[i + 1u]);
                     aabb_pair_closer(b0, b1, __float_as_uint(b0.hi.w), o, inv, tmin, tbest, i,
                                      [&](bool ok, float t, uint32_t k) { acc(ok, t, (K_AABB << 28) | k, twin_at(tw, k)); });
                 }
-            for (; i < sc.n_aabb; i++) {
+            for (; i < sh.n_aabb(); i++) {
                 if (!on(i)) continue;
                 const AabbScan b = uload(&sc.aabb[i]);
                 float t;
                 acc(aabb_closer(b.lo, b.hi, o, inv, tmin, tbest, t), t, (K_AABB << 28) | i, twin_at(tw, i));
             }
         });
-        bit += sc.n_aabb;
+        bit += sh.n_aabb();
         kind_loop(K_RECT, [&](auto tw) {
             uint32_t i = 0;
-            for (uint32_t e = sc.n_rect_x; i < e; i++) {
+            for (uint32_t e = sh.n_rect_x(); i < e; i++) {
                 if (!on(i)) continue;
                 const RectScan r = uload(&sc.rect[i]);
                 float t;
                 acc(rect_closer(r.a, r.b.x, o.x, inv.x, o.y, d.y, o.z, d.z, tmin, tbest, t), t, (K_RECT << 28) | i, twin_at(tw, i));
             }
-            for (uint32_t e = sc.n_rect_x + sc.n_rect_y; i < e; i++) {
+            for (uint32_t e = sh.n_rect_x() + sh.n_rect_y(); i < e; i++) {
                 if (!on(i)) continue;
                 const RectScan r = uload(&sc.rect[i]);
                 float t;
@@ -648,10 +701,10 @@
         });
         bit += n_rect;
     } else {
-        bit += sc.n_aabb + n_rect;
+        bit += sh.n_aabb() + n_rect;
     }
     kind_loop(K_TRI, [&](auto tw) {
-        for (uint32_t i = 0; i < sc.n_tri; i++) {
+        for (uint32_t i = 0; i < sh.n_tri(); i++) {
             if (!on(i)) continue;
             const TriScan tr = uload(&sc.tri[i]);
             float t;
@@ -665,7 +718,7 @@
             V ol, dl;
             to_local(XfScan{m.r0, m.r1, m.r2}, o, d, ol, dl);
             float t;
-            acc(mono_closer(ol, dl, m.h, tmin, tbest, t), t, (K_MONO << 28) | i, std::false_type{});
+            acc(mono_closer(ol, dl, m.h, tmin, tbest, t), t, (K_MONO << 28) | i, tt::false_type{});
         }
     }
     if constexpr (SHADOW) *best_is_twin = flag;
@@ -699,7 +752,7 @@
     if (touched) *touched = mine;
     return mask;
 }
-template <bool COUNT>
+template <bool COUNT, class SHAPE = ScanShapeRt>
 RPT_DEV void scan_primary(const SceneView& scene, V o, V d, float tmin, float& tbest, uint32_t& code, unsigned long long* cnt) {
     if constexpr (COUNT) {
         const auto& sc = *kernarg_scene();
@@ -718,10 +771,10 @@
                 }
         }
         bool skipped = false;
-        scan_prims<false, false, true>(scene, o, d, tmin, tbest, code, ~0ull, &skipped);
+        scan_prims<false, false, true, false, SHAPE>(scene, o, d, tmin, tbest, code, ~0ull, &skipped);
         if (skipped && first) atomicAdd(&cnt[9], 1ull);
     } else {
-        scan_prims<false, false, true>(scene, o, d, tmin, tbest, code);
+        scan_prims<false, false, true, false, SHAPE>(scene, o, d, tmin, tbest, code);
     }
 }
 
@@ -826,7 +879,7 @@
     w.mesh = mesh;
 }
 
-template <int BVH, bool COUNT, bool ANY = false, bool MONO = false>
+template <int BVH, bool COUNT, bool ANY = false, bool MONO = false, class SHAPE = ScanShapeRt>
 RPT_DEV void closest_hit(const SceneView& scene_, V o, V d, float tmin, float& tbest, uint32_t& code, uint32_t& inst,
                          uint32_t* stk, uint32_t stride, uint32_t& c_nodes, uint32_t& c_tris,
                          AnyHit any = AnyHit{-kInf, 1u, 0u}) {
@@ -841,7 +894,7 @@
         if (sc.mesh_deferred) walk_meshes<COUNT, ANY>(scene_, o, d, tmin, tbest, code, inst, stk, stride, c_nodes, c_tris, any);
         return;
     }
-    scan_prims<false, MONO>(scene_, o, d, tmin, tbest, code);
+    scan_prims<false, MONO, false, false, SHAPE>(scene_, o, d, tmin, tbest, code);
     if (BVH) walk_meshes<COUNT, ANY>(scene_, o, d, tmin, tbest, code, inst, stk, stride, c_nodes, c_tris, any);
 }
 
diff --git a/rpt_amd/csrc/gpu_layout.h b/rpt_amd/csrc/gpu_layout.h
--- a/rpt_amd/csrc/gpu_layout.h
+++ b/rpt_amd/csrc/gpu_layout.h
@@ -1,5 +1,17 @@
 #pragma once
+#ifndef __HIPCC_RTC__
 #include <stdint.h>
+#else
+typedef __INT8_TYPE__ int8_t;
+typedef __UINT8_TYPE__ uint8_t;
+typedef __INT16_TYPE__ int16_t;
+typedef __UINT16_TYPE__ uint16_t;
+typedef __INT32_TYPE__ int32_t;
+typedef __UINT32_TYPE__ uint32_t;
+typedef __INT64_TYPE__ int64_t;
+typedef __UINT64_TYPE__ uint64_t;
+typedef __UINTPTR_TYPE__ uintptr_t;
+#endif
 
 namespace rptg {
 
diff --git a/rpt_amd/csrc/host_internal.h b/rpt_amd/csrc/host_internal.h
--- a/rpt_amd/csrc/host_internal.h
+++ b/rpt_amd/csrc/host_internal.h
@@ -4,6 +4,7 @@
 #include <functional>
 #include <string>
 #include <utility>
+#include <vector>
 
 #include "../../include/rpt_hip.h"
 #include "kernels.h"
@@ -82,6 +83,35 @@
 }
 
 int fail(int code, const std::string& msg);
+struct ScanShape {
+    uint32_t n_sph, n_cub, n_pln, n_aabb, n_rect_x, n_rect_y, n_rect_z, n_tri, has_shell, scan_cull, medium;
+    uint64_t sph_yrot, cub_yrot;
+};
+bool scan_shape_of(const rptg::SceneView& v, ScanShape* out, std::string* why);
+std::string scan_shape_string(const ScanShape& h);
+std::string scan_jit_program(const ScanShape& h);
+std::string scan_jit_kernel_name(const ScanShape& h);
+const std::vector<std::string>& scan_jit_options();
+bool scan_jit_sources(const std::string& dir, std::vector<std::pair<std::string, std::string>>* out, std::string* why);
+std::string scan_jit_key(const std::string& program, const std::vector<std::pair<std::string, std::string>>& sources,
+                         const std::vector<std::string>& options, int rtc_major, int rtc_minor);
+bool scan_jit_compile(const ScanShape& shape, const std::vector<std::pair<std::string, std::string>>& sources, std::vector<char>* code,
+                      std::string* lowered, double* ms, std::string* why);
+bool scan_jit_resources(const std::vector<char>& code, int* vgprs, int* scratch);
+bool scan_jit_cache_read(const std::string& path, std::vector<char>* code, std::string* lowered, std::string* why);
+bool scan_jit_cache_write(const std::string& dir, const std::string& path, const std::vector<char>& code, const std::string& lowered);
+struct ScanJit {
+    int state = 1, cache = 0;
+    bool probed = false;
+    ScanShape shape{};
+    std::string shape_text, reason, key, compiler;
+    std::vector<std::pair<std::string, std::string>> sources;
+    double compile_ms = 0;
+    int vgprs = 0, scratch = 0, aot_vgprs = 0;
+    size_t lds = 0;
+    hipFunction_t fn = nullptr;
+    uint64_t launches = 0;
+};
 uint64_t seed_mix(uint64_t seed);
 struct SceneDev {
     bool committed;
diff --git a/rpt_amd/csrc/kernels.h b/rpt_amd/csrc/kernels.h
--- a/rpt_amd/csrc/kernels.h
+++ b/rpt_amd/csrc/kernels.h
@@ -1,7 +1,9 @@
 #pragma once
+#ifndef __HIPCC_RTC__
 #include <hip/hip_runtime_api.h>
 #include <stddef.h>
 #include <stdint.h>
+#endif
 #include "gpu_layout.h"
 
 namespace rptg {
@@ -38,7 +40,9 @@
     uint32_t* stream_scratch;
 };
 
-static_assert(offsetof(RenderArgs, sc) == 0, "RenderArgs must begin with the SceneView");
+static_assert(__builtin_offsetof(RenderArgs, sc) == 0, "RenderArgs must begin with the SceneView");
+
+#ifndef __HIPCC_RTC__
 
 struct KernelInfo {
     int vgprs, sgprs, lds, max_blocks_per_cu;
@@ -47,6 +51,7 @@
 hipError_t launch_render(const RenderArgs& a, int n_blocks, hipStream_t stream);
 hipError_t render_occupancy(bool medium, int bvh, int* blocks_per_cu, int detach = 0);
 size_t stream_scratch_bytes_per_block();
+__attribute__((weak)) hipError_t scan_render_info(bool medium, int* vgprs, int* scratch, size_t* lds);
 int bvh_mode(const SceneView& sc);
 hipError_t launch_buffer_add(uint32_t n_pixels, const double* d_batch, double* d_sum, double* d_sumsq, hipStream_t st);
 hipError_t launch_buffer_image(uint32_t w, uint32_t h, uint32_t radius, uint32_t n_batches, const double* d_sum, uint8_t* d_out,
@@ -181,4 +186,6 @@
 hipError_t launch_resolve_photon_f64(const rpt64::Args& a, const void* slab32, uint32_t n_chunks32, double scale_over_total, bool accumulate,
                                      double* d_out, hipStream_t stream);
 __attribute__((weak)) hipError_t launch_features_f64(const rpt64::FeatureArgs64& a, hipStream_t stream);
+#endif
+
 }
diff --git a/rpt_amd/csrc/kernels.hip b/rpt_amd/csrc/kernels.hip
--- a/rpt_amd/csrc/kernels.hip
+++ b/rpt_amd/csrc/kernels.hip
@@ -173,17 +173,17 @@
                                                : (cs != CODE_MISS && code_object<MONO>(sc, cs, is) == uint32_t(L.twin_object));
     if (cs != CODE_MISS && ts >= dist * (1.f - 1e-3f) && twin) stage_light_add(sc, albedo_med, rd, medium, I, wi, n, mcol, mat, E);
 }
-template <bool MONO = false>
+template <bool MONO = false, class SHAPE = ScanShapeRt>
 RPT_DEV bool scan_light_visible(const SceneView& sc, const Light& L, V x, V wi, float dist, float& ts) {
     ts = dist * (1.f + 1e-3f);
     uint32_t cs = CODE_MISS;
     if (__float_as_uint(L.color.w) != 0u) {
         bool twin = false;
-        scan_prims<false, MONO, false, true>(sc, x, wi, ray_tmin(x), ts, cs, ~0ull, nullptr,
+        scan_prims<false, MONO, false, true, SHAPE>(sc, x, wi, ray_tmin(x), ts, cs, ~0ull, nullptr,
                                              ShadowTwin{L.twin_lo >> 28, L.twin_lo & 0x0FFFFFFFu, L.twin_hi - L.twin_lo}, &twin);
         return twin && ts >= dist * (1.f - 1e-3f);
     }
-    scan_prims<false, MONO>(sc, x, wi, ray_tmin(x), ts, cs);
+    scan_prims<false, MONO, false, false, SHAPE>(sc, x, wi, ray_tmin(x), ts, cs);
     const bool twin = (L.twin_lo <= L.twin_hi) ? (cs >= L.twin_lo && cs <= L.twin_hi)
                                                : (cs != CODE_MISS && code_object<MONO>(sc, cs, 0u) == uint32_t(L.twin_object));
     return cs != CODE_MISS && ts >= dist * (1.f - 1e-3f) && twin;
@@ -230,6 +230,7 @@
 #endif
     static_assert(DETACH == 0 || (MEDIUM && BVH == 1 && !GROUPS), "detached tree walks: per-mesh-tree kernels in a medium only");
     static_assert(DETACH == 0 || !MONO, "no detached tree walks in scenes with monomial surfaces");
+    using Shape = tt::conditional_t<BVH == 0 && !COUNT && !GROUPS && DETACH == 0 && !MONO, ScanShapeK, ScanShapeRt>;
     extern __shared__ uint32_t dyn_lds[];
     const SceneView& sc = a.sc;
     uint32_t* stk = BVH ? (dyn_lds + threadIdx.x) : nullptr;
@@ -1105,9 +1106,9 @@
         const float tmin = ray_tmin(ro);
         uint32_t code = CODE_MISS, inst = 0;
         if constexpr (MEDIUM && BVH == 0 && !MONO)
-            scan_primary<COUNT>(sc, ro, rd, tmin, t, code, COUNT ? a.counters + kCullCounters : nullptr);
+            scan_primary<COUNT, Shape>(sc, ro, rd, tmin, t, code, COUNT ? a.counters + kCullCounters : nullptr);
         else
-            closest_hit<BVH, COUNT, false, MONO>(sc, ro, rd, tmin, t, code, inst, stk, stride, c_nodes, c_btris);
+            closest_hit<BVH, COUNT, false, MONO, Shape>(sc, ro, rd, tmin, t, code, inst, stk, stride, c_nodes, c_btris);
         if (COUNT) c_rays++;
         SECTK(3);
         const bool hit = code != CODE_MISS;
@@ -1143,7 +1144,7 @@
                     SECTK(8);
                     if constexpr (BVH == 0) {
                         float ts;
-                        const bool visible = scan_light_visible<MONO>(sc, L, x, wi, dist, ts);
+                        const bool visible = scan_light_visible<MONO, Shape>(sc, L, x, wi, dist, ts);
                         if (COUNT) c_rays++;
                         SECTK(9);
                         if (visible) stage_light_add<true>(sc, albedo_med, rd, ev_medium, I, wi, n, mcol, mat, E);
@@ -1208,6 +1209,7 @@
     }
 }
 
+#ifndef __HIPCC_RTC__
 __global__ __launch_bounds__(256) void resolve_kernel(const RenderArgs a, double scale, double* __restrict__ out) {
     uint32_t p = blockIdx.x * 256u + threadIdx.x;
     if (p >= a.n_owned) return;
@@ -1618,6 +1620,16 @@
     if (m) return c ? launch_render_b<true, true>(a, b, n_blocks, stream) : launch_render_b<true, false>(a, b, n_blocks, stream);
     return c ? launch_render_b<false, true>(a, b, n_blocks, stream) : launch_render_b<false, false>(a, b, n_blocks, stream);
 }
+hipError_t scan_render_info(bool medium, int* vgprs, int* scratch, size_t* lds) {
+    hipFuncAttributes fa{};
+    const hipError_t e = medium ? hipFuncGetAttributes(&fa, (const void*)render_kernel<true, 0, false>)
+                                : hipFuncGetAttributes(&fa, (const void*)render_kernel<false, 0, false>);
+    if (e != hipSuccess) return e;
+    *vgprs = fa.numRegs;
+    *scratch = int(fa.localSizeBytes);
+    *lds = kStateBytes;
+    return hipSuccess;
+}
 size_t stream_scratch_bytes_per_block() { return size_t(kWaveScratchDwords) * 4u * 4u; }
 hipError_t render_occupancy(bool medium, int bvh, int* blocks_per_cu, int detach) {
 #ifdef RPT_EXPERIMENTS
@@ -1760,4 +1772,6 @@
     return hipGetLastError();
 }
 
-}
+#endif
+
+}
diff --git a/rpt_amd/csrc/rpt_capi.cpp b/rpt_amd/csrc/rpt_capi.cpp
--- a/rpt_amd/csrc/rpt_capi.cpp
+++ b/rpt_amd/csrc/rpt_capi.cpp
@@ -1,15 +1,23 @@
 #include <hip/hip_runtime_api.h>
 
+#include <dlfcn.h>
+#include <unistd.h>
+
 #include <algorithm>
+#include <atomic>
 #include <cfloat>
+#include <chrono>
 #include <cmath>
 #include <cstdio>
+#include <cstdlib>
 #include <cstring>
+#include <filesystem>
 #include <functional>
 #include <limits>
 #include <memory>
 #include <mutex>
 #include <string>
+#include <type_traits>
 #include <unordered_map>
 #include <vector>
 
@@ -55,6 +63,7 @@
     int64_t room_shell = 1;
     int64_t scan_specialise = 1;
     int64_t scan_cull = 1;
+    int64_t scan_jit = 1;
     int64_t shadow_scan = 1;
     int64_t photon_skip = 0;
     int64_t photon_block_lists = 1;
@@ -97,6 +106,7 @@
     else if (s == "scan_specialise") o.scan_specialise = value;
     else if (s == "scan_cull") o.scan_cull = value;
     else if (s == "shadow_scan") o.shadow_scan = value;
+    else if (s == "scan_jit") { if (value < 0 || value > 2) return fail(RPT_ERR_INVALID, "scan_jit must be 0, 1 or 2"); o.scan_jit = value; }
     else if (s == "photon_skip") o.photon_skip = value;
     else if (s == "photon_block_lists") o.photon_block_lists = value;
     else if (s == "photon_parts") o.photon_parts = value;
@@ -519,6 +529,7 @@
     std::vector<Light> light_records;
     bool twins_scanned = false;
     uint64_t stats[16] = {0};
+    rpti::ScanJit jit;
     void* photon = nullptr;
     rpt64::Scene view64{};
     double medium_color64[3] = {0, 0, 0}, medium_color_hi64[3] = {0, 0, 0};
@@ -624,6 +635,7 @@
     if (s->photon) rpti::photon_release(s->photon);
     s->photon = nullptr;
     s->committed = false;
+    s->jit = rpti::ScanJit{};
 }
 
 void rpt_scene_destroy(rpt_scene* s) {
@@ -2450,6 +2462,345 @@
     HIP_TRY(hipEventRecord(mine.done.get(), st));
     return RPT_OK;
 }
+extern "C++" {
+namespace rpti {
+bool scan_shape_of(const SceneView& v, ScanShape* out, std::string* why) {
+    if (why) why->clear();
+    const char* w = nullptr;
+    if (v.n_lparts) w = "a group is a light (GROUPS)";
+    else if (v.n_mono) w = "the scene has monomial surfaces (MONO)";
+    else if (v.scene_bvh || v.n_nodes) w = "the scene has a tree (BVH != 0)";
+    if (w) { if (why) *why = w; return false; }
+    *out = ScanShape{v.n_sph, v.n_cub, v.n_pln, v.n_aabb, v.n_rect_x, v.n_rect_y, v.n_rect_z, v.n_tri, v.has_shell ? 1u : 0u,
+                     v.scan_cull ? 1u : 0u, v.has_medium ? 1u : 0u, v.sph_yrot, v.cub_yrot};
+    return true;
+}
+std::string scan_shape_constants(const ScanShape& h) {
+    char b[256];
+    std::snprintf(b, sizeof b, "%u,%u,%u,%u,%u,%u,%u,%u,%u,%u,0x%llxull,0x%llxull", h.n_sph, h.n_cub, h.n_pln, h.n_aabb, h.n_rect_x, h.n_rect_y,
+                  h.n_rect_z, h.n_tri, h.has_shell, h.scan_cull, (unsigned long long)h.sph_yrot, (unsigned long long)h.cub_yrot);
+    return b;
+}
+std::string scan_shape_string(const ScanShape& h) { return scan_shape_constants(h) + (h.medium ? ";medium=1" : ";medium=0"); }
+std::string scan_jit_kernel_name(const ScanShape& h) {
+    return std::string("rptg::render_kernel<") + (h.medium ? "true" : "false") + ", 0, false, false, 0, false>";
+}
+std::string scan_jit_program(const ScanShape& h) {
+    return "#define RPT_SCAN_SHAPE " + scan_shape_constants(h) + "\n#include \"kernels.hip\"\n";
+}
+const std::vector<std::string>& scan_jit_options() {
+    static const std::vector<std::string> o = {"--offload-arch=gfx950", "-O3", "-std=c++17", "-fno-slp-vectorize"};
+    return o;
+}
+bool scan_jit_sources(const std::string& dir, std::vector<std::pair<std::string, std::string>>* out, std::string* why) {
+    out->clear();
+    std::vector<std::string> todo = {"kernels.hip"};
+    while (!todo.empty()) {
+        const std::string name = todo.back();
+        todo.pop_back();
+        bool have = false;
+        for (auto& f : *out) have = have || f.first == name;
+        if (have) continue;
+        FILE* f = std::fopen((dir + "/" + name).c_str(), "rb");
+        if (!f) { *why = "source not found: " + dir + "/" + name; return false; }
+        std::string text;
+        char buf[65536];
+        for (size_t n; (n = std::fread(buf, 1, sizeof buf, f)) > 0;) text.append(buf, n);
+        std::fclose(f);
+        for (size_t p = 0; (p = text.find("#include \"", p)) != std::string::npos;) {
+            p += 10;
+            const size_t e = text.find('"', p);
+            if (e == std::string::npos) break;
+            const std::string inc = text.substr(p, e - p);
+            if (inc.find('/') == std::string::npos) todo.push_back(inc);
+            p = e;
+        }
+        out->emplace_back(name, std::move(text));
+    }
+    return true;
+}
+std::string scan_jit_key(const std::string& program, const std::vector<std::pair<std::string, std::string>>& sources,
+                         const std::vector<std::string>& options, int rtc_major, int rtc_minor) {
+    uint64_t h0 = 0xCBF29CE484222325ULL, h1 = 0x84222325CBF29CE4ULL;
+    auto eat = [&](const std::string& s) {
+        const uint64_t n = s.size();
+        for (int i = 0; i < 8; i++) { h0 = (h0 ^ ((n >> (8 * i)) & 255u)) * 0x100000001B3ULL; h1 = (h1 ^ ((n >> (8 * i)) & 255u)) * 0x100000001B3ULL; }
+        for (unsigned char c : s) { h0 = (h0 ^ c) * 0x100000001B3ULL; h1 = (h1 ^ c) * 0x100000001B3ULL; h1 ^= h1 >> 29; }
+    };
+    eat(program);
+    for (auto& f : sources) { eat(f.first); eat(f.second); }
+    for (auto& o : options) eat(o);
+    eat("hiprtc " + std::to_string(rtc_major) + "." + std::to_string(rtc_minor));
+    char b[40];
+    std::snprintf(b, sizeof b, "%016llx%016llx", (unsigned long long)h0, (unsigned long long)h1);
+    return b;
+}
+bool scan_jit_resources(const std::vector<char>& code, int* vgprs, int* scratch) {
+    auto find = [&](const char* key, int* out) {
+        const size_t kl = std::strlen(key);
+        for (size_t i = 0; i + kl + 1 <= code.size(); i++) {
+            if (std::memcmp(code.data() + i, key, kl) != 0) continue;
+            const unsigned char* p = reinterpret_cast<const unsigned char*>(code.data()) + i + kl;
+            const size_t left = code.size() - i - kl;
+            if (left >= 1 && p[0] < 0x80) { *out = p[0]; return true; }
+            if (left >= 2 && p[0] == 0xCC) { *out = p[1]; return true; }
+            if (left >= 3 && p[0] == 0xCD) { *out = (p[1] << 8) | p[2]; return true; }
+            if (left >= 5 && p[0] == 0xCE) { *out = int((uint32_t(p[1]) << 24) | (p[2] << 16) | (p[3] << 8) | p[4]); return true; }
+        }
+        return false;
+    };
+    return find(".vgpr_count", vgprs) && find(".private_segment_fixed_size", scratch);
+}
+
+namespace {
+struct Hiprtc {
+    void* lib = nullptr;
+    std::string path;
+    int major = 0, minor = 0;
+    int (*version)(int*, int*) = nullptr;
+    int (*create)(void**, const char*, const char*, int, const char* const*, const char* const*) = nullptr;
+    int (*destroy)(void**) = nullptr;
+    int (*add_name)(void*, const char*) = nullptr;
+    int (*compile)(void*, int, const char* const*) = nullptr;
+    int (*lowered)(void*, const char*, const char**) = nullptr;
+    int (*log_size)(void*, size_t*) = nullptr;
+    int (*log)(void*, char*) = nullptr;
+    int (*code_size)(void*, size_t*) = nullptr;
+    int (*code)(void*, char*) = nullptr;
+};
+struct HipModules {
+    bool looked = false, ok = false;
+    hipError_t (*load_data)(hipModule_t*, const void*) = nullptr;
+    hipError_t (*get_function)(hipFunction_t*, hipModule_t, const char*) = nullptr;
+    hipError_t (*launch)(hipFunction_t, unsigned, unsigned, unsigned, unsigned, unsigned, unsigned, unsigned, hipStream_t, void**, void**) = nullptr;
+};
+struct JitObject {
+    std::vector<char> code;
+    std::string lowered;
+    int vgprs = 0, scratch = 0;
+    double compile_ms = 0;
+    std::string rejected;
+    std::unordered_map<int, hipFunction_t> fn;
+};
+std::mutex g_jit_mutex;
+std::unordered_map<std::string, Hiprtc> g_hiprtc;
+HipModules g_modules;
+std::unordered_map<std::string, JitObject> g_jit_objects;
+uint64_t g_jit_compiles = 0;
+
+const Hiprtc* hiprtc_open(std::string* why) {
+    const char* env = std::getenv("RPT_HIPRTC_LIB");
+    const std::vector<std::string> paths = env && *env ? std::vector<std::string>{env} : std::vector<std::string>{"/opt/rocm/lib/libhiprtc.so", "libhiprtc.so"};
+    for (const std::string& path : paths) {
+        auto it = g_hiprtc.find(path);
+        if (it != g_hiprtc.end()) { if (it->second.lib) return &it->second; continue; }
+        Hiprtc& h = g_hiprtc[path];
+        void* lib = dlopen(path.c_str(), RTLD_NOW | RTLD_LOCAL);
+        if (!lib) continue;
+        bool ok = true;
+        auto sym = [&](auto& fn, const char* name) { fn = reinterpret_cast<std::remove_reference_t<decltype(fn)>>(dlsym(lib, name)); ok = ok && fn; };
+        sym(h.version, "hiprtcVersion"); sym(h.create, "hiprtcCreateProgram"); sym(h.destroy, "hiprtcDestroyProgram");
+        sym(h.add_name, "hiprtcAddNameExpression"); sym(h.compile, "hiprtcCompileProgram"); sym(h.lowered, "hiprtcGetLoweredName");
+        sym(h.log_size, "hiprtcGetProgramLogSize"); sym(h.log, "hiprtcGetProgramLog"); sym(h.code_size, "hiprtcGetCodeSize");
+        sym(h.code, "hiprtcGetCode");
+        if (!ok || h.version(&h.major, &h.minor) != 0) { dlclose(lib); continue; }
+        h.lib = lib;
+        h.path = path;
+        return &h;
+    }
+    *why = "hiprtc not available (" + paths[0] + ")";
+    return nullptr;
+}
+const HipModules& hip_modules() {
+    HipModules& m = g_modules;
+    if (m.looked) return m;
+    m.looked = true;
+    Dl_info di{};
+    if (!dladdr(reinterpret_cast<void*>(&hipGetDeviceCount), &di) || !di.dli_fname) return m;
+    void* lib = dlopen(di.dli_fname, RTLD_NOW | RTLD_NOLOAD);
+    if (!lib) return m;
+    m.load_data = reinterpret_cast<decltype(m.load_data)>(dlsym(lib, "hipModuleLoadData"));
+    m.get_function = reinterpret_cast<decltype(m.get_function)>(dlsym(lib, "hipModuleGetFunction"));
+    m.launch = reinterpret_cast<decltype(m.launch)>(dlsym(lib, "hipModuleLaunchKernel"));
+    m.ok = m.load_data && m.get_function && m.launch;
+    return m;
+}
+std::string jit_source_dir() {
+    if (const char* env = std::getenv("RPT_JIT_SRC")) if (*env) return env;
+    Dl_info di{};
+    if (!dladdr(reinterpret_cast<void*>(&rpt_last_error), &di) || !di.dli_fname) return "";
+    const std::string lib = di.dli_fname;
+    const size_t slash = lib.rfind('/');
+    return (slash == std::string::npos ? std::string(".") : lib.substr(0, slash)) + "/csrc";
+}
+std::string jit_cache_dir() {
+    if (const char* env = std::getenv("RPT_JIT_CACHE")) if (*env) return env;
+    const char* home = std::getenv("HOME");
+    return home && *home ? std::string(home) + "/.cache/rpt_amd/jit" : std::string();
+}
+uint64_t fnv_bytes(const void* p, size_t n, uint64_t h = 0xCBF29CE484222325ULL) {
+    const unsigned char* b = static_cast<const unsigned char*>(p);
+    for (size_t i = 0; i < n; i++) h = (h ^ b[i]) * 0x100000001B3ULL;
+    return h;
+}
+}
+
+bool scan_jit_cache_read(const std::string& path, std::vector<char>* code, std::string* lowered, std::string* why) {
+    FILE* f = std::fopen(path.c_str(), "rb");
+    if (!f) { *why = "no cache file"; return false; }
+    char magic[8];
+    uint64_t hd[3] = {0, 0, 0};
+    bool ok = std::fread(magic, 1, 8, f) == 8 && std::memcmp(magic, "RPTJIT01", 8) == 0 && std::fread(hd, 8, 3, f) == 3 && hd[0] > 0 &&
+              hd[0] < (uint64_t(1) << 28) && hd[1] > 0 && hd[1] < 4096;
+    if (ok) {
+        lowered->resize(size_t(hd[1]));
+        code->resize(size_t(hd[0]));
+        ok = std::fread(&(*lowered)[0], 1, lowered->size(), f) == lowered->size() && std::fread(code->data(), 1, code->size(), f) == code->size() &&
+             fnv_bytes(code->data(), code->size(), fnv_bytes(lowered->data(), lowered->size())) == hd[2];
+    }
+    std::fclose(f);
+    if (!ok) *why = "cache file truncated or damaged";
+    return ok;
+}
+bool scan_jit_cache_write(const std::string& dir, const std::string& path, const std::vector<char>& code, const std::string& lowered) {
+    std::error_code ec;
+    std::filesystem::create_directories(dir, ec);
+    static std::atomic<unsigned> serial{0};
+    const std::string tmp = path + ".tmp." + std::to_string(uint64_t(getpid())) + "." + std::to_string(serial++);
+    FILE* f = std::fopen(tmp.c_str(), "wb");
+    if (!f) return false;
+    const uint64_t hd[3] = {code.size(), lowered.size(), fnv_bytes(code.data(), code.size(), fnv_bytes(lowered.data(), lowered.size()))};
+    bool ok = std::fwrite("RPTJIT01", 1, 8, f) == 8 && std::fwrite(hd, 8, 3, f) == 3 && std::fwrite(lowered.data(), 1, lowered.size(), f) == lowered.size() &&
+              std::fwrite(code.data(), 1, code.size(), f) == code.size();
+    ok = (std::fclose(f) == 0) && ok;
+    if (ok) ok = std::rename(tmp.c_str(), path.c_str()) == 0;
+    if (!ok) std::remove(tmp.c_str());
+    return ok;
+}
+bool scan_jit_compile(const ScanShape& shape, const std::vector<std::pair<std::string, std::string>>& sources, std::vector<char>* code,
+                      std::string* lowered, double* ms, std::string* why) {
+    std::string w;
+    const Hiprtc* rtc = hiprtc_open(&w);
+    if (!rtc) { *why = w; return false; }
+    const std::string program = scan_jit_program(shape), name = scan_jit_kernel_name(shape);
+    std::vector<const char*> texts, names, opts;
+    for (auto& f : sources) { names.push_back(f.first.c_str()); texts.push_back(f.second.c_str()); }
+    for (auto& o : scan_jit_options()) opts.push_back(o.c_str());
+    void* prog = nullptr;
+    if (rtc->create(&prog, program.c_str(), "rpt_scan_jit.hip", int(texts.size()), texts.data(), names.data()) != 0) { *why = "hiprtcCreateProgram failed"; return false; }
+    const auto t0 = std::chrono::steady_clock::now();
+    bool ok = rtc->add_name(prog, name.c_str()) == 0;
+    if (!ok) *why = "hiprtcAddNameExpression failed";
+    if (ok && rtc->compile(prog, int(opts.size()), opts.data()) != 0) {
+        ok = false;
+        size_t n = 0;
+        std::string log;
+        if (rtc->log_size(prog, &n) == 0 && n > 1) { log.resize(n); rtc->log(prog, &log[0]); }
+        *why = "compile error: " + log.substr(0, 600);
+    }
+    *ms = std::chrono::duration<double, std::milli>(std::chrono::steady_clock::now() - t0).count();
+    const char* low = nullptr;
+    size_t n = 0;
+    if (ok && (rtc->lowered(prog, name.c_str(), &low) != 0 || !low)) { ok = false; *why = "no lowered name for " + name; }
+    if (ok) *lowered = low;
+    if (ok && (rtc->code_size(prog, &n) != 0 || n == 0)) { ok = false; *why = "empty code object"; }
+    if (ok) { code->resize(n); if (rtc->code(prog, code->data()) != 0) { ok = false; *why = "hiprtcGetCode failed"; } }
+    rtc->destroy(&prog);
+    return ok;
+}
+}
+
+static hipFunction_t scan_jit_function(rpt_scene* s, const RenderArgs& a) {
+    using namespace rpti;
+    ScanJit& j = s->jit;
+    if (s->opt.scan_jit == 0 || a.counters) return nullptr;
+    if (j.fn) return j.fn;
+    if (j.state == RPT_SCAN_JIT_FALLBACK || j.state == RPT_SCAN_JIT_OUT_OF_SCOPE) return nullptr;
+    std::lock_guard<std::mutex> lock(g_jit_mutex);
+    auto give_up = [&](int state, const std::string& why) { j.state = state; j.reason = why; return nullptr; };
+    if (!j.probed) {
+        j.probed = true;
+        ScanShape shape;
+        std::string why;
+        if (!scan_shape_of(s->view, &shape, &why)) return give_up(RPT_SCAN_JIT_OUT_OF_SCOPE, why);
+        j.shape = shape;
+        j.shape_text = scan_shape_string(shape);
+        if (!scan_render_info) return give_up(RPT_SCAN_JIT_FALLBACK, "this build has no AOT twin to compare with");
+        if (!hip_modules().ok) return give_up(RPT_SCAN_JIT_FALLBACK, "the HIP runtime has no module entry points");
+        const Hiprtc* rtc = hiprtc_open(&why);
+        if (!rtc) return give_up(RPT_SCAN_JIT_FALLBACK, why);
+        if (!scan_jit_sources(jit_source_dir(), &j.sources, &why)) return give_up(RPT_SCAN_JIT_FALLBACK, why);
+        j.key = scan_jit_key(scan_jit_program(shape), j.sources, scan_jit_options(), rtc->major, rtc->minor);
+        j.compiler = "hiprtc " + std::to_string(rtc->major) + "." + std::to_string(rtc->minor) + " (" + rtc->path + ")";
+        int aot_scratch = 0;
+        if (scan_render_info(shape.medium != 0, &j.aot_vgprs, &aot_scratch, &j.lds) != hipSuccess || j.aot_vgprs <= 0)
+            return give_up(RPT_SCAN_JIT_FALLBACK, "the AOT twin's registers are unknown");
+    }
+    const int aot_vgprs = j.aot_vgprs;
+    auto it = g_jit_objects.find(j.key);
+    int cache = RPT_SCAN_JIT_CACHE_MEMORY;
+    const std::string dir = jit_cache_dir(), path = dir.empty() ? std::string() : dir + "/" + j.key + ".co";
+    std::string note;
+    if (it == g_jit_objects.end() && !path.empty()) {
+        JitObject o;
+        std::string why;
+        if (scan_jit_cache_read(path, &o.code, &o.lowered, &why) && scan_jit_resources(o.code, &o.vgprs, &o.scratch)) {
+            it = g_jit_objects.emplace(j.key, std::move(o)).first;
+            cache = RPT_SCAN_JIT_CACHE_DISK;
+        } else if (why != "no cache file") {
+            std::remove(path.c_str());
+            note = "cache file discarded (" + (why.empty() ? std::string("no resource note") : why) + "); ";
+        }
+    }
+    if (it == g_jit_objects.end()) {
+        const uint64_t samples = uint64_t(a.n_owned) * a.iterations;
+        if (s->opt.scan_jit == 1 && samples < (uint64_t(1) << 27)) {
+            j.state = RPT_SCAN_JIT_IDLE;
+            j.reason = note + "no cached code object, and the launch is below the compile threshold of 2^27 camera samples";
+            return nullptr;
+        }
+        JitObject o;
+        std::string why;
+        g_jit_compiles++;
+        if (!scan_jit_compile(j.shape, j.sources, &o.code, &o.lowered, &o.compile_ms, &why)) o.rejected = why;
+        else if (!scan_jit_resources(o.code, &o.vgprs, &o.scratch)) o.rejected = "no resource note in the code object";
+        else if (!path.empty()) (void)scan_jit_cache_write(dir, path, o.code, o.lowered);
+        it = g_jit_objects.emplace(j.key, std::move(o)).first;
+        cache = RPT_SCAN_JIT_CACHE_MISS;
+    }
+    JitObject& o = it->second;
+    j.cache = cache;
+    j.compile_ms = cache == RPT_SCAN_JIT_CACHE_MISS ? o.compile_ms : 0.0;
+    j.vgprs = o.vgprs;
+    j.scratch = o.scratch;
+    if (!o.rejected.empty()) return give_up(RPT_SCAN_JIT_FALLBACK, note + o.rejected);
+    if (o.vgprs > aot_vgprs)
+        return give_up(RPT_SCAN_JIT_FALLBACK, note + std::to_string(o.vgprs) + " VGPRs against the AOT kernel's " + std::to_string(aot_vgprs));
+    auto fn = o.fn.find(s->device);
+    if (fn == o.fn.end()) {
+        hipModule_t mod = nullptr;
+        hipFunction_t f = nullptr;
+        hipError_t e = hip_modules().load_data(&mod, o.code.data());
+        if (e == hipSuccess) e = hip_modules().get_function(&f, mod, o.lowered.c_str());
+        if (e != hipSuccess || !f) {
+            if (cache == RPT_SCAN_JIT_CACHE_DISK) { std::remove(path.c_str()); g_jit_objects.erase(it); }
+            return give_up(RPT_SCAN_JIT_FALLBACK, note + "load error: " + hipGetErrorString(e));
+        }
+        fn = o.fn.emplace(s->device, f).first;
+    }
+    j.fn = fn->second;
+    j.state = RPT_SCAN_JIT_ACTIVE;
+    j.reason = note + j.compiler;
+    return j.fn;
+}
+static hipError_t launch_render_jit(rpt_scene* s, hipFunction_t fn, const RenderArgs& a, int n_blocks, hipStream_t stream) {
+    size_t size = sizeof(RenderArgs);
+    void* extra[] = {HIP_LAUNCH_PARAM_BUFFER_POINTER, const_cast<RenderArgs*>(&a), HIP_LAUNCH_PARAM_BUFFER_SIZE, &size, HIP_LAUNCH_PARAM_END};
+    s->jit.launches++;
+    return rpti::hip_modules().launch(fn, unsigned(n_blocks), 1, 1, 256, 1, 1, unsigned(s->jit.lds), stream, nullptr, extra);
+}
+}
+
 static int run_render(rpt_scene* s, const rpt_render_params* prm, const RenderArgs& a_in, double* d_out, hipStream_t st) {
     RenderArgs a = a_in;
     int bpc = int(s->opt.blocks_per_cu);
@@ -2462,8 +2813,11 @@
         HIP_TRY(ls.d_stream.reserve(size_t(s->n_cus) * size_t(bpc) * stream_scratch_bytes_per_block()));
         a.stream_scratch = ls.d_stream.get<uint32_t>();
     }
+    const hipFunction_t jit = a.n_items ? scan_jit_function(s, a) : nullptr;
     return rpti::run_persistent(s, prm, a, d_out, st, bpc,
-                                [](const RenderArgs& ra, int nb, hipStream_t stream) { return launch_render(ra, nb, stream); }, true);
+                                [s, jit](const RenderArgs& ra, int nb, hipStream_t stream) {
+                                    return jit ? launch_render_jit(s, jit, ra, nb, stream) : launch_render(ra, nb, stream);
+                                }, true);
 }
 extern "C++" rpti::SceneDev rpti::scene_dev(rpt_scene* s) {
     int first = -1;
@@ -3363,6 +3717,44 @@
     out[2] = (bits_u(L.color.w) != 0u && bvh_mode(s->view) == 0) ? 1u : 0u;
     out[3] = uint32_t(L.twin_object);
     return RPT_OK;
+}
+int rpt_scan_jit_info(rpt_scene* s, int64_t out[8], char* text, uint64_t text_capacity) {
+    if (!s || !out) return fail(RPT_ERR_INVALID, "null argument");
+    if (!text && text_capacity) return fail(RPT_ERR_INVALID, "rpt_scan_jit_info: a capacity without a buffer");
+    if (!s->committed) return fail(RPT_ERR_STATE, "rpt_scene_commit must be called first");
+    const rpti::ScanJit& j = s->jit;
+    std::string shape = j.shape_text, reason = j.reason;
+    int state = j.state;
+    if (!j.probed) {
+        rpti::ScanShape h;
+        if (rpti::scan_shape_of(s->view, &h, &reason)) shape = rpti::scan_shape_string(h);
+        else state = RPT_SCAN_JIT_OUT_OF_SCOPE;
+    }
+    if (s->opt.scan_jit == 0) { state = RPT_SCAN_JIT_OFF; reason = "option scan_jit = 0"; }
+    out[0] = state;
+    out[1] = j.cache;
+    out[2] = int64_t(j.compile_ms * 1000.0);
+    out[3] = j.vgprs;
+    out[4] = j.scratch;
+    out[5] = int64_t(j.launches);
+    {
+        std::lock_guard<std::mutex> lock(rpti::g_jit_mutex);
+        out[6] = int64_t(rpti::g_jit_compiles);
+    }
+    out[7] = j.aot_vgprs;
+    if (text_capacity) {
+        const std::string t = shape + "\n" + reason;
+        const size_t n = std::min<size_t>(t.size(), size_t(text_capacity) - 1);
+        std::memcpy(text, t.data(), n);
+        text[n] = 0;
+    }
+    return RPT_OK;
+}
+int rpt_scan_jit_forget(void) {
+    std::lock_guard<std::mutex> lock(rpti::g_jit_mutex);
+    const int n = int(rpti::g_jit_objects.size());
+    rpti::g_jit_objects.clear();
+    return n;
 }
 int rpt_debug_distance_pair(float sigma_t, uint32_t k0, uint32_t n, float* out_new, float* out_guarded) {
     if (!out_new || !out_guarded) return fail(RPT_ERR_INVALID, "null argument");
```

Result: faster. 16250 Msamples/s, median of 6 (+7.3%).
